# manhtuando97/two-stage-gnn

Measured on AMD Instinct MI355X. Metric: graphs/sec fwd+bwd, DD batch=32 SAGE-3L h=128, higher is better.
Workload: dtype f32; 1 GPU; DD-shaped synthetic graphs (avg 269 nodes / 676 edges, F_in=89), batch=32 per GPU, GcnEncoderGraph (GraphSage 'base') 3 layers h=128, Nmax=1000, slot-BN, CE loss, clip 2.0 + Adam; 1 step(s) per hipGraph launch, seed = rank, 128 untimed settle steps before the warm-up; global_batch=32, parallelism=dp1, launch=hipGraph replay (one graph: forward + backward + bucket + optimiser), rows=8151, edges_directed=40970

## Files before the change

### include/tsgnn.h

```cpp
#ifndef TSGNN_H
#define TSGNN_H
#include <stdint.h>

typedef struct ihipStream_t* tsgnn_stream_t;

#ifdef __cplusplus
extern "C" {
#endif

#define TSGNN_ABI_VERSION 2
int tsgnn_abi_version(void);
const char* tsgnn_strerror(int code);
const char* tsgnn_last_kernel(void);


int tsgnn_scan_workspace_ints(int64_t n, int64_t* ws_ints);
int tsgnn_exclusive_scan_i32(const int* in, int64_t n, int* out, int* ws, tsgnn_stream_t stream);

int tsgnn_row_maps(const int* graph_ptr, int B, int64_t n_rows, int* row_graph, int* row_slot,
                   tsgnn_stream_t stream);

int tsgnn_dense_adj_count(const float* adj, int B, int nmax, const int* graph_ptr, const int* row_graph,
                          int64_t n_rows, int* row_cnt, tsgnn_stream_t stream);
int tsgnn_dense_adj_fill(const float* adj, int B, int nmax, const int* graph_ptr, const int* row_graph,
                         int64_t n_rows, const int* rowptr, int* col, float* val, tsgnn_stream_t stream);

int tsgnn_coo_count(const int64_t* key, int64_t E, int64_t n_rows, int* cnt, int* bad_flag,
                    tsgnn_stream_t stream);
int tsgnn_coo_fill(const int64_t* key, const int64_t* other, int64_t E, int64_t n_rows, const int* rowptr,
                   int* cursor, int* col, int* eid, tsgnn_stream_t stream);


int tsgnn_ingest_layout(int B, int nmax, int64_t row_cap, int ell_w, int64_t tail_cap, int64_t* off);
int tsgnn_host_collate_tu(const int64_t* ds_graph_ptr, const int64_t* ds_rowptr, const int64_t* ds_col, const int64_t* ds_node_label,
                          const int64_t* ds_graph_label, const int64_t* ids, int B, int nmax, int64_t row_cap, int ell_w,
                          int64_t tail_cap, int32_t* staging, int64_t* out);
int tsgnn_onehot_rows_f32(const int* label, int64_t n_rows, int64_t total_rows, int F, float* x, int64_t ldx, tsgnn_stream_t stream);

int tsgnn_ingest_upload_f32(int32_t* dev, const int32_t* host, int64_t words, const int* node_label_dev, int64_t n_rows, int64_t total_rows,
                            int F, float* x, int64_t ldx, tsgnn_stream_t stream);
int tsgnn_ingest_compact_layout(int B, int nmax, int64_t row_cap, int64_t edge_cap, int64_t tail_cap, int64_t* off);
int tsgnn_host_collate_compact(const int64_t* ds_graph_ptr, const int64_t* ds_rowptr, const int64_t* ds_col, const int64_t* ds_node_label,
                               const int64_t* ds_graph_label, const int64_t* ids, int B, int nmax, int64_t row_cap, int64_t edge_cap,
                               int ell_w, int64_t tail_cap, int32_t* staging, int64_t* out);
int tsgnn_ingest_pull_expand_f32(const int32_t* host, int32_t* mirror, int B, int nmax, int64_t row_cap, int64_t edge_cap, int ell_w,
                                 int64_t tail_cap, int32_t* row_graph, int32_t* row_slot, int32_t* ell, int32_t* tail_ptr, int32_t* ell_slots, int32_t* tail_slots, int F, float* x,
                                 int64_t ldx, tsgnn_stream_t stream);
int tsgnn_ingest_pull_expand_ack_f32(const int32_t* host, int32_t* mirror, int B, int nmax, int64_t row_cap, int64_t edge_cap, int ell_w,
                                     int64_t tail_cap, int32_t* row_graph, int32_t* row_slot, int32_t* ell, int32_t* tail_ptr, int32_t* ell_slots, int32_t* tail_slots, int F,
                                     float* x, int64_t ldx, int64_t* host_ack, tsgnn_stream_t stream);
int tsgnn_ingest_pull_f32(const int32_t* host, int32_t* mirror, int B, int nmax, int64_t row_cap, int64_t edge_cap, int64_t tail_cap,
                          tsgnn_stream_t stream);
int tsgnn_ingest_expand_ack_f32(int32_t* mirror, int B, int nmax, int64_t row_cap, int64_t edge_cap, int ell_w, int64_t tail_cap,
                                int32_t* row_graph, int32_t* row_slot, int32_t* ell, int32_t* tail_ptr, int32_t* ell_slots, int32_t* tail_slots, int F, float* x, int64_t ldx,
                                int64_t* host_ack, tsgnn_stream_t stream);
int tsgnn_ingest_arm_pull_rider(const int32_t* host, int32_t* mirror, int B, int nmax, int64_t row_cap, int64_t edge_cap, int64_t tail_cap);
int tsgnn_ingest_arm_pull_rider_parts(const int32_t* host, int32_t* mirror, int B, int nmax, int64_t row_cap, int64_t edge_cap, int64_t tail_cap,
                                      int parts, int skip);
int tsgnn_ingest_arm_expand_rider(int32_t* mirror, int B, int nmax, int64_t row_cap, int64_t edge_cap, int ell_w, int64_t tail_cap,
                                  int32_t* row_graph, int32_t* row_slot, int32_t* ell, int32_t* tail_ptr, int32_t* ell_slots, int32_t* tail_slots, int F, float* x, int64_t ldx,
                                  int64_t* host_ack);
int tsgnn_ingest_flush_pull_rider(tsgnn_stream_t stream);
int tsgnn_ingest_disarm_riders(void);
typedef struct tsgnn_collate_pool tsgnn_collate_pool;
int tsgnn_collate_pool_create(int nthreads, tsgnn_collate_pool** pool);
int tsgnn_collate_pool_submit(tsgnn_collate_pool* pool, const int64_t* ds_graph_ptr, const int64_t* ds_rowptr, const int64_t* ds_col,
                              const int64_t* ds_node_label, const int64_t* ds_graph_label, const int64_t* ids, int B, int nmax,
                              int64_t row_cap, int64_t edge_cap, int ell_w, int64_t tail_cap, int32_t* staging, int64_t* out,
                              void* after_event, int64_t* ticket);
int tsgnn_collate_pool_submit_ack(tsgnn_collate_pool* pool, const int64_t* ds_graph_ptr, const int64_t* ds_rowptr, const int64_t* ds_col,
                                  const int64_t* ds_node_label, const int64_t* ds_graph_label, const int64_t* ids, int B, int nmax,
                                  int64_t row_cap, int64_t edge_cap, int ell_w, int64_t tail_cap, int32_t* staging, int64_t* out,
                                  const int64_t* host_ack, int64_t ack_target, int seq, int64_t* ticket);
int tsgnn_collate_pool_wait(tsgnn_collate_pool* pool, int64_t ticket);
int tsgnn_collate_pool_destroy(tsgnn_collate_pool* pool);

int tsgnn_csr_transpose(const int* rowptr, const int* col, const float* val, int64_t n_rows, int64_t n_cols,
                        int64_t nnz, int* rowptr_t, int* col_t, float* val_t, int* src_e, int* cnt_ws,
                        int* scan_ws, tsgnn_stream_t stream);


int tsgnn_csr_spmm_f32(const int* rowptr, const int* col, const float* val, const float* self_w,
                       const float* x, int64_t ldx, float* y, int64_t ldy, int64_t n_rows, int feat,
                       float self_scalar, int relu_in, int accumulate, tsgnn_stream_t stream);

int tsgnn_csr_to_ell(const int* rowptr, const int* col, int64_t n_rows, int W, int* ell, int* tail_cnt, tsgnn_stream_t stream);
int tsgnn_csr_tail_fill(const int* rowptr, const int* col, const int* tail_ptr, int64_t n_rows, int W, int* tail_col,
                        tsgnn_stream_t stream);
int tsgnn_ell_spmm_f32(const int* ell, int W, const float* x, int64_t ldx, float* y, int64_t ldy, int64_t n_rows, int feat,
                       float self_scalar, tsgnn_stream_t stream);

int tsgnn_gcn_norm_f32(const int* rowptr, const int* col, const float* val, int64_t n_rows, float self_fill,
                       float* dinv, float* val_out, float* self_w, tsgnn_stream_t stream);

int tsgnn_sddmm_rows_f32(const int* rowptr, const int* col, const float* dy, int64_t lddy, const float* x, int64_t ldx,
                         int64_t n_rows, int feat, float* dval, float* dself, tsgnn_stream_t stream);


int tsgnn_gemm_f32(const float* A, int64_t sam, int64_t sak, const float* B, int64_t sbk, int64_t sbn, float* C,
                   int64_t scm, int64_t scn, int M, int N, int K, int batch, int64_t stride_a, int64_t stride_b,
                   int64_t stride_c, const int* seg_ptr, int ragged, int max_seg, float alpha, int accumulate,
                   tsgnn_stream_t stream);
int tsgnn_gemm_splitk_plan(int M, int N, int K, int* ksplit, int64_t* ws_floats);
int tsgnn_gemm_splitk_f32(const float* A, int64_t sam, int64_t sak, const float* B, int64_t sbk, int64_t sbn,
                          float* C, int M, int N, int K, int ksplit, float* ws, int accumulate,
                          tsgnn_stream_t stream);
int tsgnn_linear_wgrad_plan(int64_t rows, int K_in, int N, int64_t ldz, int64_t lddu, int* nslab, int64_t* rows_per_slab,
                            int64_t* ws_floats);
int tsgnn_linear_wgrad_f32(const float* z, int64_t ldz, const float* du, int64_t lddu, int64_t rows, int K_in, int N, int nslab,
                           int64_t rows_per_slab, int64_t bias_only_rows, float* ws, float* dw, float* db, tsgnn_stream_t stream);
int tsgnn_wgrad_reduce_sets_blocks(const int64_t* desc);
int tsgnn_wgrad_reduce_sets_f32(const int64_t* desc, float* normparts, float* step_state, tsgnn_stream_t stream);
int tsgnn_wgrad_reduce_multi_f32(const float* ws0, int nslab0, int K0, int N0, float* dw0, float* db0, const float* ws1, int nslab1,
                                 int K1, int N1, float* dw1, float* db1, const float* ws2, int nslab2, int K2, int N2, float* dw2,
                                 float* db2, const float* ws3, int nslab3, int K3, int N3, float* dw3, float* db3,
                                 float* normparts, float* step_state, tsgnn_stream_t stream);
int tsgnn_wgrad_blocks_plan(int64_t rows, int K_in, int N, int64_t ldz, int64_t lddu, int* nslab, int64_t* rows_per_slab,
                            int64_t* ws_floats);
int tsgnn_wgrad_blocks_f32(const float* z, int64_t ldz, const float* du, int64_t lddu, int64_t rows, int K_in, int N, int nslab,
                           int64_t rows_per_slab, float* ws, float* dw, int64_t lddw, tsgnn_stream_t stream);
int tsgnn_wgrad_blocks_oi_f32(const float* z, int64_t ldz, const float* du, int64_t lddu, int64_t rows, int K_in, int N, int nslab,
                              int64_t rows_per_slab, float* ws, float* dw_oi, int64_t lddw, float* db, tsgnn_stream_t stream);
int tsgnn_ragged_tn_f32(const float* s_mat, int64_t lds_, const float* x, int64_t ldx, int K, int N, const int* slab_row_ptr,
                        int nslab, const int* seg_slab_ptr, int nseg, float* ws, float* out, tsgnn_stream_t stream);
int tsgnn_ragged_tn_direct_supported(int K, int64_t max_rows);
int tsgnn_ragged_tn_direct_f32(const float* s_mat, int64_t lds_, int K, const int* graph_ptr, int B, const float* x0, int64_t ldx0,
                               int N0, float* out0, const float* x1, int64_t ldx1, int N1, float* out1, tsgnn_stream_t stream);
int tsgnn_ragged_tn_direct_ro_f32(const float* s_mat, int64_t lds_, int K, const int* graph_ptr, int B, const float* x0, int64_t ldx0,
                                  int N0, float* out0, const float* x1, int64_t ldx1, int N1, float* out1, float* ro_out,
                                  int64_t ro_ldo, int* ro_arg, int nmax, int64_t n_real, int ghost_zero, tsgnn_stream_t stream);
int tsgnn_wgrad_narrow_plan(int64_t rows, int K_in, int N, int64_t* ws_floats);
int tsgnn_wgrad_narrow_f32(const float* z, int64_t ldz, const float* du, int64_t lddu, int64_t rows, int K_in, int N, float* ws,
                           float* dwb, tsgnn_stream_t stream);
int tsgnn_colsum_f32(const float* x, int64_t ld, int64_t rows, int F, float* out, float* ws, int accumulate,
                     tsgnn_stream_t stream);

int tsgnn_linear_l2norm_f32(const float* z, int64_t ldz, const float* w, int64_t ldw, const float* bias, float* v,
                            int64_t ldv, float* rinv, int64_t rows, int K, int N, int normalize,
                            tsgnn_stream_t stream);
int tsgnn_rowgemm_supported(const float* a, int64_t lda, const float* b, int64_t ldb, const float* c, int64_t ldc, int K, int N,
                            int trans_b);
int tsgnn_rowgemm_f32(const float* a, int64_t lda, const float* b, int64_t ldb, int trans_b, const float* bias, float* c,
                      int64_t ldc, float* rinv, int64_t rows, int K, int N, int normalize, int64_t fill_rows,
                      tsgnn_stream_t stream);
int tsgnn_panel_blocks(int64_t rows, int panel_units);
int tsgnn_gather_rowgemm_f32(const int* ell, int ell_w, const int* tail_ptr, const int* tail_col, const float* x, int64_t ldx, const float* b, int64_t ldb, int trans_b,
                             const float* bias, float* c, int64_t ldc, float* rinv, float* zout, int64_t ldz, int64_t rows, int K,
                             int N, int normalize, int64_t fill_rows, tsgnn_stream_t stream);
int tsgnn_gather_rowgemm_st_f32(const int* ell, int ell_w, const int* tail_ptr, const int* tail_col, const float* x, int64_t ldx, const float* b, int64_t ldb, const float* bias,
                                float* c, int64_t ldc, float* rinv, float* zout, int64_t ldz, int64_t rows, int K, int N,
                                int64_t fill_rows, const int* row_slot, unsigned long long* sums, float* ghost, int panel_units,
                                const int64_t* pack_desc, tsgnn_stream_t stream);
int tsgnn_sage_layer_fwd_bn_f32(const int* ell, int ell_w, const int* tail_ptr, const int* tail_col, const float* x, int64_t ldx, const float* w, int64_t ldw, const float* bias,
                                float* v, int64_t ldv, float* rinv, float* zout, int64_t ldz, int64_t rows, int K, int64_t fill_rows,
                                const int* graph_ptr, const int* slot_count, int B, int nslots, int n_ghost, unsigned long long* packed,
                                unsigned long long* packed_out, const int* row_graph, const unsigned long long* sums_in,
                                const float* ghost_in, float* mean_out, float* rstd_out, const int* row_slot,
                                unsigned long long* sums_out, float* ghost_out, const int* ro_map, int ro_map_ch, int panel_units,
                                const float* w_img, tsgnn_stream_t stream);
int tsgnn_sage_layer_fwd_bn_plan(int64_t rows, int64_t fill_rows, int B, int nslots, int panel_units, int* ro_ch, int* n_gemm,
                                 int* n_full);
int tsgnn_sage_layer_fwd_f32(const int* ell, int ell_w, const int* tail_ptr, const int* tail_col, const float* x, int64_t ldx, const float* w, int64_t ldw, const float* bias,
                             float* v, int64_t ldv, float* rinv, float* zout, int64_t ldz, int64_t rows, int K, int64_t fill_rows,
                             const int* graph_ptr, int B, int nslots, int n_ghost, unsigned long long* packed, tsgnn_stream_t stream);
int tsgnn_sage_layer_fwd_ro_f32(const int* ell, int ell_w, const int* tail_ptr, const int* tail_col, const float* x, int64_t ldx, const float* w, int64_t ldw, const float* bias,
                                float* v, int64_t ldv, float* rinv, float* zout, int64_t ldz, int64_t rows, int K, int64_t fill_rows,
                                const int* graph_ptr, int B, int nslots, int n_ghost, unsigned long long* packed,
                                unsigned long long* packed_out, const int* row_graph, tsgnn_stream_t stream);
int tsgnn_sage_layer_bwd_f32(const int* ell, int ell_w, const int* tail_ptr, const int* tail_col, const float* du, int64_t lddu, const float* w, int64_t ldw, float* dxs,
                             int64_t lddxs, const float* z, int64_t ldz, int64_t rows, int nslab, int64_t rows_per_slab,
                             int64_t bias_only_rows, float* ws, int panel_units, const float* w_img, tsgnn_stream_t stream);
int tsgnn_l2norm_bwd_f32(const float* v, int64_t ldv, const float* dv, int64_t lddv, const float* rinv, float* du,
                         int64_t lddu, int64_t rows, int F, tsgnn_stream_t stream);


int tsgnn_bn_slots_fwd_f32(const int* graph_ptr, const int* slot_count, const int* row_slot, int B, int nmax,
                           int64_t n_real, int n_ghost, const float* v, int64_t ldv, int F, int relu, int bn,
                           float* mean, float* rstd, float* y, int64_t ldy, tsgnn_stream_t stream);
int tsgnn_bn_slots_bwd_f32(const int* graph_ptr, const int* slot_count, const int* row_slot, int B, int nmax,
                           int64_t n_real, int n_ghost, const float* v, int64_t ldv, const float* dy, int64_t lddy, int F,
                           int relu, int bn, const float* mean, const float* rstd, float* m1, float* m2, float* dv,
                           int64_t lddv, tsgnn_stream_t stream);

int tsgnn_row_ln_fwd_f32(const float* v, int64_t ldv, int64_t rows, int F, int relu, float* mean, float* rstd, float* y, int64_t ldy,
                         tsgnn_stream_t stream);
int tsgnn_row_ln_bwd_f32(const float* v, int64_t ldv, const float* dy, int64_t lddy, int64_t rows, int F, int relu, const float* mean,
                         const float* rstd, float* dv, int64_t lddv, tsgnn_stream_t stream);

int tsgnn_row_post_bwd_f32(const int* row_graph, int B, int64_t n_real, int64_t rows, const float* v, int64_t ldv, const float* dxs,
                           int64_t lddxs, const float* dout, int64_t ldo, const int* arg, int F, int relu, int ln, const float* mean,
                           const float* rstd, const float* rinv, float* du, int64_t lddu, tsgnn_stream_t stream);

int tsgnn_row_post_nodes_bwd_f32(int64_t n_real, int64_t rows, const float* v, int64_t ldv, const float* dxs, int64_t lddxs,
                                 const float* dnode, int64_t lddn, int ghost_zero, int F, int relu, int ln, const float* mean,
                                 const float* rstd, const float* rinv, float* du, int64_t lddu, tsgnn_stream_t stream);

int tsgnn_readout_max_ws_words(int B, int nmax, int F);
int tsgnn_readout_max_fwd_f32(const int* graph_ptr, const int* slot_count, int B, int nmax, int64_t n_real, int n_ghost,
                              const float* x, int64_t ldx, int F, int relu, unsigned long long* packed_ws, float* out,
                              int64_t ldo, int* arg, tsgnn_stream_t stream);
int tsgnn_readout_max_bwd_f32(const float* dout, int64_t ldo, const int* arg, int B, int F, const float* x, int64_t ldx_in,
                              int relu, int64_t n_real, float* dx, int64_t ldx, tsgnn_stream_t stream);
int tsgnn_readout_max_bwd_rows_f32(const float* dout, int64_t ldo, const int* arg, const int* row_graph, int F, int64_t rows,
                                   int64_t rows_total, const float* add, int64_t ldadd, float* dx, int64_t ldx, tsgnn_stream_t stream);

int tsgnn_pack_rows_f32(const float* src, int nmax, int F, const int* row_graph, const int* row_slot, int64_t n_real,
                        float* dst, int64_t ld, tsgnn_stream_t stream);
int tsgnn_unpack_rows_f32(const int* graph_ptr, int B, int nmax, int64_t n_real, int n_ghost, const float* src, int64_t ld,
                          int F, float fill, float* dst, tsgnn_stream_t stream);
int tsgnn_unpack_rows_bwd_ghost_f32(const int* graph_ptr, int B, int nmax, int64_t n_real, const float* ddst, int F,
                                    float* dsrc, int64_t ld, tsgnn_stream_t stream);


int tsgnn_softmax_ce_f32(const float* logits, int64_t ld, const int64_t* label, int B, int C, float* loss, float* dlogits,
                         tsgnn_stream_t stream);
int tsgnn_adam_from_partials_f32(float* param, const float* grad, float* m, float* v, int64_t n, float lr, float beta1, float beta2,
                                 float eps, float weight_decay, float max_norm, float* state, const float* parts, int nparts,
                                 const float* poison, tsgnn_stream_t stream);
int tsgnn_clip_adam_step_f32(float* param, const float* grad, float* m, float* v, int64_t n, float lr, float beta1,
                             float beta2, float eps, float weight_decay, float max_norm, float grad_scale, float* state,
                             float* ws, const float* poison, tsgnn_stream_t stream);


int tsgnn_dense_stack_supported(int B, int K, int nstack, int L, int fin0, int hidden, int last0, int last1);
int tsgnn_dense_stack_fwd_f32(const int64_t* desc, tsgnn_stream_t stream);
int tsgnn_dense_stack_bwd_f32(const int64_t* desc, tsgnn_stream_t stream);
int tsgnn_dense_stack_max_resident(void);
int tsgnn_dense_stack_barrier_selftest(unsigned* sync, float* err, int expect, tsgnn_stream_t stream);


int tsgnn_node_scores_f32(const float* x, int64_t ldx, int64_t rows, int H, int Fh, const float* a, int64_t lda, float* s,
                          tsgnn_stream_t stream);
int tsgnn_node_scores2_f32(const float* x, int64_t ldx, int64_t rows, int H, int Fh, const float* a1, int64_t lda1, float* s1,
                           const float* a2, int64_t lda2, float* s2, tsgnn_stream_t stream);
int tsgnn_edge_softmax_fwd_f32(const int* rowptr, const int* col, int64_t rows, int H, const float* s_grp, const float* s_oth,
                               int mod, float slope, float* alpha, tsgnn_stream_t stream);
int tsgnn_edge_softmax_bwd_f32(const int* rowptr, const int* col, int64_t rows, int H, const float* s_grp, const float* s_oth,
                               int mod, float slope, const float* alpha, const float* dalpha, float* dt, float* ds_grp,
                               tsgnn_stream_t stream);
int tsgnn_edge_permute_f32(const float* src, const int* perm, int64_t n, int H, int scatter, float* dst, tsgnn_stream_t stream);
int tsgnn_csr_row_sum_f32(const int* rowptr, const float* val, int64_t rows, int H, float* out, tsgnn_stream_t stream);
int tsgnn_csr_row_sum_perm_f32(const int* rowptr, const float* val, const int* eperm, int64_t rows, int H, float* out,
                               tsgnn_stream_t stream);
int tsgnn_csr_spmm_heads_f32(const int* rowptr, const int* col, const float* alpha, int H, int Fh, const float* x, int64_t ldx,
                             int mod, float* y, int64_t ldy, int64_t rows, tsgnn_stream_t stream);
int tsgnn_csr_spmm_heads_epi_f32(const int* rowptr, const int* col, const float* alpha, int H, int Fh, const float* x, int64_t ldx,
                                 int mod, float* y, int64_t ldy, int64_t rows, const float* w1, const float* a1, int64_t lda1,
                                 const float* w2, const float* a2, int64_t lda2, const float* u, int64_t ldu, const float* uw,
                                 int rows_per_seg, const int* row_seg, float uscale, const int* eperm, tsgnn_stream_t stream);
int tsgnn_csr_sddmm_heads_f32(const int* rowptr, const int* col, int H, int Fh, const float* dy, int64_t lddy, const float* x,
                              int64_t ldx, int mod, float* dalpha, int64_t rows, tsgnn_stream_t stream);
int tsgnn_segment_wsum_f32(const float* x, int64_t ldx, const float* w, int H, int Fh, const int* seg_ptr, int nseg, int64_t rows,
                           int64_t max_seg, float scale, int mean, float* ws, float* out, int64_t ldo, tsgnn_stream_t stream);
int tsgnn_segment_wsum2_f32(const float* x, int64_t ldx, const float* w1, const float* w2, int H, int Fh, const int* seg_ptr, int nseg,
                            int64_t rows, int64_t max_seg, float scale, float* ws, float* out1, float* out2, int64_t ldo,
                            tsgnn_stream_t stream);
int tsgnn_gather_wsum_f32(const float* x, int64_t ldx, const int* idx, const float* w, const int* seg_ptr, int nseg, int C, float scale,
                          float* out, int64_t ldo, tsgnn_stream_t stream);
int tsgnn_broadcast_add_f32(float* y, int64_t ldy, int64_t rows, int H, int Fh, const float* w, const float* a, int64_t lda,
                            const float* u, int64_t ldu, int rows_per_seg, float scale, tsgnn_stream_t stream);
int tsgnn_pack_heads_max(void);
int tsgnn_pack_heads_f32(const float* w0, const float* w1, const float* w2, const float* w3, const float* w4, const float* w5,
                         const float* w6, const float* w7, const float* a0, const float* a1, const float* a2, const float* a3,
                         const float* a4, const float* a5, const float* a6, const float* a7, int H, int Fin, int Fo, float* W, float* A,
                         tsgnn_stream_t stream);
int tsgnn_unpack_heads_f32(const float* dW, const float* dA0, const float* dA1, int H, int Fin, int Fo, float* gw, float* ga,
                           tsgnn_stream_t stream);

int tsgnn_gat_fused_supported(int H, int Fh);
int tsgnn_gat_attn_fwd_f32(const float* hp, int64_t ldh, const int* rowptr, const int* col, const int* rp_t, const int* col_t,
                           int64_t rows, int H, int Fh, float slope, const int* row_graph, int nmax, const int* iso_idx,
                           const float* iso_w, const int* iso_ptr, float uscale, int mean_heads, int apply_elu, float drop_p,
                           uint64_t seed, const unsigned long long* drop_ctr, float* stat, float* y, int64_t ldy, tsgnn_stream_t stream);
int tsgnn_gat_bwd_parts(int B);
int tsgnn_gat_attn_bwd_f32(const float* hp, int64_t ldh, const float* y, int64_t ldy, const float* dy, int64_t lddy, const int* rp_t,
                           const int* col_t, int64_t rows, int H, int Fh, float slope, int mean_heads, int apply_elu,
                           const int* graph_ptr, int B, const int* iso_idx, const float* iso_w, const int* iso_ptr,
                           const float* iso_row, int iso_row_ld, float uscale, float drop_p, uint64_t seed,
                           const unsigned long long* drop_ctr, const float* stat, float* dhp, int Ns, float* t1, float* t2, float* S,
                           float* dupart, tsgnn_stream_t stream);
int tsgnn_gat_attn_bwd_ro_f32(const float* hp, int64_t ldh, const float* y, int64_t ldy, const float* dy, int64_t lddy, const int* rp_t,
                              const int* col_t, int64_t rows, int H, int Fh, float slope, int mean_heads, int apply_elu,
                              const int* graph_ptr, int B, const int* iso_idx, const float* iso_w, const int* iso_ptr,
                              const float* iso_row, int iso_row_ld, float uscale, float drop_p, uint64_t seed,
                              const unsigned long long* drop_ctr, const float* stat, float* dhp, int Ns, float* t1, float* t2, float* S,
                              float* dupart, const float* ro_dout, int64_t ro_ldo, const int* ro_arg, const int* row_graph,
                              tsgnn_stream_t stream);
int tsgnn_gat_dropout_mult_f32(float drop_p, uint64_t seed, const unsigned long long* drop_ctr, int64_t i0, int64_t ni, int64_t j0,
                               int64_t nj, int H, float* out, tsgnn_stream_t stream);
int tsgnn_gat_score_rowsum_f32(const int* rowptr, const int* col, const int* eperm, const float* t1, const float* t2, const float* S,
                               int64_t rows, int H, float* dhp, int64_t ldh, int C, const float* dupart, int B, const int* iso_idx,
                               const float* iso_w, const int* iso_ptr, float uscale, tsgnn_stream_t stream);
int tsgnn_gat_pack_desc_words(void);
int tsgnn_gat_pack_f32(const int64_t* desc, tsgnn_stream_t stream);
int tsgnn_gat_unpack_f32(const int64_t* desc, tsgnn_stream_t stream);
int tsgnn_elu_heads_fwd_f32(const float* x, int64_t rows, int H, int Fh, int mean_heads, int apply_elu, float* y, tsgnn_stream_t stream);
int tsgnn_elu_heads_bwd_f32(const float* x, const float* dy, int64_t rows, int H, int Fh, int mean_heads, int apply_elu, float* dx,
                            tsgnn_stream_t stream);


int tsgnn_mlp3_supported(int B, int D0, int D1, int D2, int C);
int tsgnn_mlp3_fwd_f32(const float* x, int64_t ldx, const float* w1, const float* b1, const float* keep, float keep_scale, const float* w2,
                       const float* b2, const float* w3, const float* b3, int B, int D0, int D1, int D2, int C, float* a1, float* a2,
                       float* logp, tsgnn_stream_t stream);
int tsgnn_mlp3_fwd_drop_f32(const float* x, int64_t ldx, const float* w1, const float* b1, float p, uint64_t seed,
                            unsigned long long* state, unsigned long long* used, const float* w2, const float* b2, const float* w3,
                            const float* b3, int B, int D0, int D1, int D2, int C, float* a1, float* a2, float* logp,
                            tsgnn_stream_t stream);
int tsgnn_mlp3_dropout_mask_f32(float p, uint64_t seed, uint64_t counter, int B, int D1, float* out, tsgnn_stream_t stream);
int tsgnn_mlp3_bwd_f32(const float* x, int64_t ldx, const float* w1, const float* w2, const float* w3, const float* a1,
                       const float* a2, const float* logp, const float* dlogp, float keep_scale, int B, int D0, int D1, int D2, int C,
                       float* dw1, float* db1, float* dw2, float* db2, float* dw3, float* db3, float* dx, int64_t lddx,
                       tsgnn_stream_t stream);
int tsgnn_mlp3_bwd2_f32(const float* x, int64_t ldx, const float* w1, const float* w2, const float* w3, const float* a1,
                        const float* a2, const float* logp, const float* dlogp, float keep_scale, int B, int D0, int D1, int D2, int C,
                        float* dw1, float* db1, float* dw2, float* db2, float* dw3, float* db3, float* dx, int64_t lddx, float* ws,
                        tsgnn_stream_t stream);
int tsgnn_mlp3_bwd2_nll_f32(const float* x, int64_t ldx, const float* w1, const float* w2, const float* w3, const float* a1,
                            const float* a2, const float* logp, const int64_t* label, float* loss, float keep_scale, int B, int D0,
                            int D1, int D2, int C, float* dw1, float* db1, float* dw2, float* db2, float* dw3, float* db3, float* dx,
                            int64_t lddx, float* ws, tsgnn_stream_t stream);

int tsgnn_mlp3_bwd2_norm_blocks(int D1, int D2);
int tsgnn_mlp3_bwd2_np_f32(const float* x, int64_t ldx, const float* w1, const float* w2, const float* w3, const float* a1,
                           const float* a2, const float* logp, const float* dlogp, const int64_t* label, float* loss, float keep_scale, int B,
                           int D0, int D1, int D2, int C, float* dw1, float* db1, float* dw2, float* db2, float* dw3, float* db3, float* dx,
                           int64_t lddx, float* ws, float* normparts, tsgnn_stream_t stream);

int tsgnn_mlp3_triplet_supported(int D0, int D1, int D2, int C);
int tsgnn_mlp3_triplet_fwd_f32(const float* x, int64_t ldx, const float* w1, const float* b1, float p, uint64_t seed,
                               unsigned long long* state, unsigned long long* used, const float* w2, const float* b2, const float* w3,
                               const float* b3, int D0, int D1, int D2, int C, float eps, float* a1, float* a2, float* embed, float* dist,
                               tsgnn_stream_t stream);
int tsgnn_mlp3_triplet_bwd_f32(const float* x, int64_t ldx, const float* w1, const float* w2, const float* w3, const float* a1,
                               const float* a2, const float* embed, const float* dist, float eps, float keep_scale, const float* g_dp,
                               const float* g_dn, const float* g_ea, const float* g_ep, const float* g_en, int D0, int D1, int D2, int C,
                               float* dw1, float* db1, float* dw2, float* db2, float* dw3, float* db3, float* dx, int64_t lddx,
                               tsgnn_stream_t stream);


int tsgnn_linkpred_tile_rows(void);
int tsgnn_linkpred_chunks(void);
int tsgnn_linkpred_loss_f32(const float* S, int64_t lds, int K, int64_t rows, const int* slab_row_ptr, const int* slab_graph,
                            int nslab, const int* graph_ptr, const int* rowptr, const int* col, const float* val,
                            const int* rowptr_t, const int* col_t, const float* val_t, float clamp, float inv_entries, float* dS,
                            int64_t ldd, float* ws, float* part, float* loss, tsgnn_stream_t stream);
int tsgnn_linkpred_loss_xy_f32(const float* X, int64_t ldx, const float* Y, int64_t ldy, int K, int64_t rows, const int* slab_row_ptr,
                               const int* slab_graph, int nslab, const int* graph_ptr, const int* rowptr, const int* col,
                               const float* val, float clamp, float inv_entries, int count_loss, float* dX, int64_t ldd, float* ws,
                               float* part, float* loss, tsgnn_stream_t stream);


int tsgnn_topk_max_segment(void);
int tsgnn_topk_segments_f32(const float* score, const int* graph_ptr, const int* k_ptr, int B, int max_seg, int* perm,
                            int* new_id, tsgnn_stream_t stream);
int tsgnn_gather_gate_fwd_f32(const float* x, int64_t ldx, const float* score, const int* perm, int64_t K, int F, int use_tanh,
                              float* out, int64_t ldo, tsgnn_stream_t stream);
int tsgnn_gather_gate_bwd_f32(const float* x, int64_t ldx, const float* score, const int* perm, int64_t K, int F, int use_tanh,
                              const float* dout, int64_t ldo, float* dx, int64_t lddx, float* dscore, tsgnn_stream_t stream);
int tsgnn_filter_edges_mark(const int* perm, int64_t K, int64_t N, const int64_t* src, const int64_t* dst, int64_t E,
                            int* new_id, int* flag, tsgnn_stream_t stream);
int tsgnn_filter_edges_compact(const int64_t* src, const int64_t* dst, int64_t E, const int* new_id, const int* flag,
                               const int* pos, int64_t* out_src, int64_t* out_dst, int64_t* kept_eid, tsgnn_stream_t stream);
int tsgnn_gcn_coef_f32(const int* rowptr, const int* col, int64_t n_rows, float* dinv, float* self_w, tsgnn_stream_t stream);
int tsgnn_gcn_propagate_f32(const int* rowptr, const int* col, const float* dinv, const float* self_w, const float* x,
                            int64_t ldx, int relu_in, const float* bias, const float* w_dot, const float* dot_bias, float* y,
                            int64_t ldy, float* t, int64_t n_rows, int feat, tsgnn_stream_t stream);
int tsgnn_gcn_propagate_re_f32(const int* rowptr, const int* rowend, const int* col, const float* dinv, const float* self_w,
                               const float* x, int64_t ldx, int relu_in, const float* bias, const float* w_dot, const float* dot_bias,
                               float* y, int64_t ldy, float* t, int64_t n_rows, int feat, tsgnn_stream_t stream);
int tsgnn_gcn_propagate_affine_f32(const int* rowptr, const int* rowend, const int* col, const float* dinv, const float* self_w,
                                   const float* x, int64_t ldx, float* agg, int64_t ldagg, int64_t n_rows, int feat, const float* w,
                                   int64_t ldw, const float* bias, float* y, int64_t ldy, int n_out, tsgnn_stream_t stream);
int tsgnn_propagate_mean_f32(const int* rowptr, const int* rowend, const int* col, int transpose, const float* x, int64_t ldx,
                             const float* xself, int64_t ldxs, float* y, int64_t ldy, int64_t n_rows, int feat, tsgnn_stream_t stream);
int tsgnn_sag_supported(int F);
int tsgnn_sag_pool_gather_f32(const float* y, int64_t ldy, const float* score, const int* perm, const int* new_id,
                              const int* rowptr, const int* col, int64_t K, int F, int relu_in, float* xp, int64_t ldo, int* cnt,
                              tsgnn_stream_t stream);
int tsgnn_sag_pool_graph_max_nodes(void);
int tsgnn_sag_pool_graph_f32(const float* y, int64_t ldy, const int* rowptr, const int* rowend, const int* col, const float* dinv,
                             const float* self_w, const float* w_s, const float* b_s, const int* graph_ptr, const int* graph_ptr_new,
                             int B, int max_seg, int F, float* score, int* perm, int* new_id, float* xp, int64_t ldo, int* cnt,
                             float* out, int64_t ldout, int* arg, int accumulate, int* rowptr_new, int* rowend_new, int* col_new,
                             float* dinv_new, float* self_w_new, float* agg_next, int64_t ldagg, tsgnn_stream_t stream);
int tsgnn_sag_readout_f32(const float* xp, int64_t ld, const int* graph_ptr, int B, int F, int accumulate, float* out, int64_t ldo,
                          int* arg, tsgnn_stream_t stream);
int tsgnn_csr_filter_fill(const int* rowptr, const int* col, const int* perm, const int* new_id, int64_t K, const int* rowptr_new,
                          int* col_new, float* dinv_new, float* self_w_new, tsgnn_stream_t stream);
int tsgnn_scan_short_i32(const int* in, int64_t n, int* out, tsgnn_stream_t stream);
int tsgnn_sag_pool_bwd_f32(const float* y, int64_t ldy, const float* score, const int* new_id, const int* row_graph_new,
                           const int* graph_ptr_new, const int* arg, const float* dxp, int64_t lddxp, const float* dread,
                           int64_t lddr, int64_t N, int F, int relu_in, float* dyb, int64_t lddy, float* dscore,
                           tsgnn_stream_t stream);
int tsgnn_sag_pool_graph_bwd_f32(const float* y, int64_t ldy, const float* score, const int* new_id, const int* graph_ptr,
                                 const int* graph_ptr_new, const int* arg, const float* dxp, int64_t lddxp, const float* dread,
                                 int64_t lddr, const int* rowptr, const int* rowend, const int* col, const float* dinv,
                                 const float* self_w, const float* w_s, int B, int max_seg, int F, float* du, int64_t lddu, float* part,
                                 float* dws, float* dbs, const float* dagg_next, int64_t lddagg, const int* rowptr_n,
                                 const int* rowend_n, const int* col_n, const float* dinv_n, const float* self_w_n,
                                 tsgnn_stream_t stream);
int tsgnn_sag_pool_graph_gc_f32(const float* y, int64_t ldy, const int* rowptr, const int* rowend, const int* col, const float* w_rel,
                                const float* w_root, const float* b, const int* graph_ptr, const int* graph_ptr_new, int B, int max_seg,
                                int F, float* score, int* perm, int* new_id, float* xp, int64_t ldo, int* cnt, float* out,
                                int64_t ldout, int* arg, int accumulate, int* rowptr_new, int* rowend_new, int* col_new,
                                tsgnn_stream_t stream);
int tsgnn_sag_pool_graph_gc_bwd_f32(const float* y, int64_t ldy, const float* score, const int* new_id, const int* graph_ptr,
                                    const int* graph_ptr_new, const int* arg, const float* dxp, int64_t lddxp, const float* dread,
                                    int64_t lddr, const int* rowptr, const int* rowend, const int* col, const float* w_rel,
                                    const float* w_root, int B, int max_seg, int F, float* du, int64_t lddu, float* part,
                                    tsgnn_stream_t stream);
int tsgnn_sag_du_reduce_f32(float* part, int nb, int F, float* dws, float* dbs, tsgnn_stream_t stream);
int tsgnn_linear_wgrad_du_f32(const float* z, int64_t ldz, const float* du, int64_t lddu, int64_t rows, int K_in, int N, int nslab,
                              int64_t rows_per_slab, float* ws, float* dw, float* db, float* part, int nb, int F_du, float* dws,
                              float* dbs, tsgnn_stream_t stream);
int tsgnn_sag_du_blocks(int64_t N, int F);
int tsgnn_sag_du_f32(const int* rowptr, const int* rowend, const int* col, const float* dinv, const float* self_w, const float* dscore, const float* y,
                     int64_t ldy, const float* w_s, float* dyb, int64_t lddy, int64_t N, int F, float* part, float* dws, float* dbs,
                     tsgnn_stream_t stream);
int tsgnn_relu_fwd_f32(const float* x, int64_t n, float* y, tsgnn_stream_t stream);
int tsgnn_relu_bwd_f32(const float* y, const float* dy, int64_t n, float* dx, tsgnn_stream_t stream);
int tsgnn_row_softmax_fwd_f32(const float* x, int64_t ldx, int64_t rows, int C, float* y, int64_t ldy, tsgnn_stream_t stream);
int tsgnn_row_softmax_bwd_f32(const float* y, int64_t ldy, const float* dy, int64_t lddy, int64_t rows, int C, float* dx,
                              int64_t lddx, tsgnn_stream_t stream);
int tsgnn_row_softmax_masked_fwd_f32(const float* x, int64_t ldx, int64_t rows, int C, float* y, int64_t ldy, int64_t zero_from,
                                     tsgnn_stream_t stream);
int tsgnn_row_softmax_masked_bwd_f32(const float* y, int64_t ldy, const float* dy, int64_t lddy, int64_t rows, int C, float* dx,
                                     int64_t lddx, int64_t zero_from, tsgnn_stream_t stream);
int tsgnn_row_softmax_ent_fwd_f32(const float* x, int64_t ldx, int64_t rows, int C, const float* mask, float eps, float* y, int64_t ldy,
                                  float* hpart, tsgnn_stream_t stream);
int tsgnn_row_softmax_ent_bwd_f32(const float* y, int64_t ldy, const float* ds, int64_t ldds, const float* mask, const float* g_ent,
                                  float g_scale, float eps, int64_t rows, int C, float* dx, int64_t lddx, tsgnn_stream_t stream);
int tsgnn_diffpool_link_fwd_f32(const float* adj, int64_t n_adj, const float* ao, const float* G, int B, int K, double* part, int nblk,
                                float* link, double* coef, tsgnn_stream_t stream);
int tsgnn_diffpool_link_bwd_f32(const float* g_link, const double* coef, const float* G, int B, int K, const float* adj, int64_t n_adj,
                                float* dG, float* dao, float* dadj, tsgnn_stream_t stream);


int tsgnn_slot_fused_supported(int B, int F);
int tsgnn_slot_bn_fwd_f32(const int* graph_ptr, const int* slot_count, int B, int nmax, int64_t n_real, int n_ghost,
                          const float* v, int64_t ldv, int F, int relu, float* mean, float* rstd, float* y, int64_t ldy,
                          unsigned long long* zero_ptr, int64_t zero_n, tsgnn_stream_t stream);
int tsgnn_slot_post_bwd_f32(const int* graph_ptr, const int* slot_count, int B, int nmax, int64_t n_real, int n_ghost,
                            const float* v, int64_t ldv, const float* dxs, int64_t lddxs, const float* dxs2, int64_t lddxs2,
                            const float* dout, int64_t ldo, const int* arg, int F, int relu, int bn, const float* mean,
                            const float* rstd, const float* rinv, float* du, int64_t lddu, tsgnn_stream_t stream);
int tsgnn_slot_post_wgrad_f32(const int* graph_ptr, const int* slot_count, int B, int nmax, int64_t n_real, int n_ghost,
                              const float* v, int64_t ldv, const float* dxs, int64_t lddxs, const float* dout, int64_t ldo,
                              const int* arg, int F, int relu, int bn, const float* mean, const float* rstd, const float* rinv,
                              const float* z, int64_t ldz, int K_in, float* ws, int nblocks, tsgnn_stream_t stream);
int tsgnn_readout_l2_bwd_f32(const int* graph_ptr, const int* row_graph, int B, int64_t n_real, int n_ghost_rows, const float* v,
                             int64_t ldv, const float* dout, int64_t ldo, const int* arg, int F, const float* rinv, float* du,
                             int64_t lddu, tsgnn_stream_t stream);
int tsgnn_readout_partial_f32(const int* graph_ptr, int B, int nmax, int64_t n_real, int n_ghost, const float* x, int64_t ldx, int F,
                              unsigned long long* packed, tsgnn_stream_t stream);
int tsgnn_readout_decode_layers_f32(const unsigned long long* packed, int B, int L, int Fh, int Fl, float* out, int64_t ldo, int* arg,
                                    tsgnn_stream_t stream);


int tsgnn_head2_fwd_f32(const float* out, int64_t ldo, const float* w1, const float* b1, const float* w2, const float* b2, int B, int P,
                        int E, int C, float* vec, float* y, tsgnn_stream_t stream);
int tsgnn_readout_head_fwd_f32(const unsigned long long* packed, int B, int L, int Fh, int Fl, const float* v_last, int64_t ldv,
                               const int* graph_ptr, int64_t n_real, int nslots, int n_ghost, float* out, int64_t ldo, int* arg,
                               const float* w1, const float* b1, const float* w2, const float* b2, int E, int C, float* vec, float* y,
                               tsgnn_stream_t stream);
int tsgnn_packed_head_fwd_f32(const unsigned long long* packed, int B, int L, int Fh, int Fl, float* out, int64_t ldo, int* arg,
                              const float* w1, const float* b1, const float* w2, const float* b2, int E, int C, float* vec, float* y,
                              tsgnn_stream_t stream);
int tsgnn_packed_head_fwd_z_f32(unsigned long long* packed, int B, int L, int Fh, int Fl, float* out, int64_t ldo, int* arg,
                                const float* w1, const float* b1, const float* w2, const float* b2, int E, int C, float* vec, float* y,
                                unsigned long long* clear, int64_t clear_n, tsgnn_stream_t stream);
int tsgnn_head2_bwd_f32(const float* out, int64_t ldo, const float* vec, const float* dy, const float* dvec, const float* w1,
                        const float* w2, int B, int P, int E, int C, float* dout, int64_t lddo, float* dw1, float* db1,
                        float* dw2, float* db2, float* normparts, tsgnn_stream_t stream);
int tsgnn_head2_fwd_ro_f32(float* out, int64_t ldo, const float* w1, const float* b1, const float* w2, const float* b2, int B, int P,
                           int E, int C, float* vec, float* y, const float* z, int64_t ldz, int N, int c0, int F, int* arg,
                           tsgnn_stream_t stream);
int tsgnn_head2_bwd_ro_f32(const float* out, int64_t ldo, const float* vec, const float* dy, const float* dvec, const float* w1,
                           const float* w2, int B, int P, int E, int C, float* dout, int64_t lddo, float* dw1, float* db1,
                           float* dw2, float* db2, float* normparts, const int* arg, int c0, int F, int N, float* dz, int64_t lddz,
                           const float* ce_y, const int64_t* ce_label, float* ce_loss, tsgnn_stream_t stream);
int tsgnn_head2_bwd_ce_f32(const float* out, int64_t ldo, const float* vec, const float* y, const int64_t* label, float* loss,
                           const float* dvec, const float* w1, const float* w2, int B, int P, int E, int C, float* dout, int64_t lddo,
                           float* dw1, float* db1, float* dw2, float* db2, float* normparts, tsgnn_stream_t stream);

int tsgnn_head2_bwd_du_f32(const float* out, int64_t ldo, const float* vec, const float* y, const int64_t* label, float* loss,
                           const float* dy, const float* dvec, const float* w1, const float* w2, int B, int P, int E, int C, float* dout,
                           int64_t lddo, float* dw1, float* db1, float* dw2, float* db2, float* normparts, const int* graph_ptr,
                           int64_t n_real, int n_ghost_rows, int max_nodes, const float* v, int64_t ldv, const float* rinv, const int* arg,
                           int seg_off, int F, float* du, int64_t lddu, tsgnn_stream_t stream);
int tsgnn_head2_bwd_du_map_f32(const float* out, int64_t ldo, const float* vec, const float* y, const int64_t* label, float* loss,
                               const float* dy, const float* dvec, const float* w1, const float* w2, int B, int P, int E, int C,
                               float* dout, int64_t lddo, float* dw1, float* db1, float* dw2, float* db2, float* normparts,
                               const int* graph_ptr, int64_t n_real, int n_ghost_rows, int max_nodes, const float* v, int64_t ldv,
                               const float* rinv, const int* arg, int seg_off, int F, float* du, int64_t lddu, const int* du_map,
                               int n_map, int du_chunk, tsgnn_stream_t stream);

int tsgnn_contract_dense_supported(int N, int K, int F);
int tsgnn_contract_dense_fwd_f32(const float* s, const float* z, const float* adj, int B, int N, int K, int F, float* xo, float* ao,
                                 float* t, tsgnn_stream_t stream);
int tsgnn_contract_dense_fwd_ro_f32(const float* s, const float* z, const float* adj, int B, int N, int K, int F, float* xo, float* ao,
                                    float* t, float* ro_out, int64_t ro_ldo, int* ro_arg, float* s_out, tsgnn_stream_t stream);
int tsgnn_contract_dense_bwd_f32(const float* s, const float* z, const float* adj, const float* t, const float* dxo, const float* dao,
                                 int B, int N, int K, int F, float* ds, float* dz, float* dadj, tsgnn_stream_t stream);
int tsgnn_contract_dense_bwd_ro_f32(const float* s, const float* z, const float* adj, const float* t, const float* dxo, const float* dao,
                                    int B, int N, int K, int F, float* ds, float* dz, float* dadj, const float* ro_dout, int64_t ro_ldo,
                                    const int* ro_arg, int softmax, tsgnn_stream_t stream);

int tsgnn_contract_rows_bwd_supported(int K, int F);
int tsgnn_contract_rows_bwd_f32(const float* S, int64_t ldS, const float* Z, int64_t ldZ, const float* AS, int64_t ldAS,
                                const float* dxo, const float* dao, const int* slab_row_ptr, const int* slab_graph, int nslab, int K,
                                int F, float* dZ, int64_t lddZ, float* dS, int64_t lddS, float* dAS, int64_t lddAS,
                                int64_t zero_from, int64_t zero_to, tsgnn_stream_t stream);
int tsgnn_contract_rows_bwd_ro_f32(const float* S, int64_t ldS, const float* Z, int64_t ldZ, const float* AS, int64_t ldAS,
                                   const float* dxo, const float* dao, const int* slab_row_ptr, const int* slab_graph, int nslab, int K,
                                   int F, float* dZ, int64_t lddZ, float* dS, int64_t lddS, float* dAS, int64_t lddAS,
                                   int64_t zero_from, int64_t zero_to, const float* ro_dout, int64_t ro_ldo, const int* ro_arg,
                                   tsgnn_stream_t stream);

int tsgnn_slot_bn_fwd_pair_f32(const int* graph_ptr, const int* slot_count, int B, int nmax, int64_t n_real, int n_ghost,
                               const float* v0, const float* v1, int64_t ldv, int F, int relu, float* mean0, float* mean1, float* rstd0,
                               float* rstd1, float* y0, float* y1, int64_t ldy, tsgnn_stream_t stream);
int tsgnn_slot_post_bwd_pair_f32(const int* graph_ptr, const int* slot_count, int B, int nmax, int64_t n_real, int n_ghost,
                                 const float* v0, const float* v1, int64_t ldv, const float* dxs0, const float* dxs1, int64_t lddxs,
                                 const float* dxs2_0, const float* dxs2_1, int64_t lddxs2, int F, int relu, int bn, const float* mean0,
                                 const float* mean1, const float* rstd0, const float* rstd1, const float* rinv0, const float* rinv1,
                                 float* du0, float* du1, int64_t lddu, tsgnn_stream_t stream);

int tsgnn_sage_multi_tn_words(void);
int tsgnn_sage_multi_g_words(void);
int tsgnn_sage_multi_f32(const int64_t* desc, tsgnn_stream_t stream);
int tsgnn_sage_multi_zero_f32(const int64_t* desc, float* zero0, int64_t n0, float* zero1, int64_t n1, tsgnn_stream_t stream);

int tsgnn_gat_bwd_products_f32(const float* x, int64_t ldx, const float* du, int64_t lddu, int64_t rows, int K_in, int N, const float* wp,
                               int64_t ldwp, float* dx, int64_t lddx, int nslab, int64_t rows_per_slab, float* ws, tsgnn_stream_t stream);
int tsgnn_linear_bwd_products_f32(const float* x, int64_t ldx, const float* dy, int64_t lddy, int64_t rows, int K_in, int N, const float* w,
                                  int64_t ldw, float* dx, int64_t lddx, int nslab, int64_t rows_per_slab, float* ws, tsgnn_stream_t stream);
int tsgnn_wgrad_blocks_slabs_f32(const float* z, int64_t ldz, const float* du, int64_t lddu, int64_t rows, int K_in, int N, int nslab,
                                 int64_t rows_per_slab, float* ws, tsgnn_stream_t stream);

int tsgnn_triplet_embed_fwd_f32(const float* r, int64_t ldr, const float* w, int64_t ldw, const float* b, int D, int E, float eps,
                                float* embed, float* dist, tsgnn_stream_t stream);
int tsgnn_triplet_embed_bwd_f32(const float* r, int64_t ldr, const float* w, int64_t ldw, int D, int E, float eps, const float* embed,
                                const float* dist, const float* d_dp, const float* d_dn, const float* d_ea, const float* d_ep,
                                const float* d_en, float* d_r, int64_t lddr, float* dw, int64_t lddw, float* db, tsgnn_stream_t stream);

int tsgnn_mlp2_triplet_supported(int D, int H, int E);
int tsgnn_mlp2_triplet_fwd_f32(const float* r, int64_t ldr, const float* w1, const float* b1, const float* w2, const float* b2, int D,
                               int H, int E, float eps, float* h, float* embed, float* dist, tsgnn_stream_t stream);
int tsgnn_mlp2_triplet_bwd_f32(const float* r, int64_t ldr, const float* w1, const float* w2, const float* h, const float* embed,
                               const float* dist, float eps, const float* g_dp, const float* g_dn, const float* g_ea, const float* g_ep,
                               const float* g_en, int D, int H, int E, float* dr, int64_t lddr, float* dw1, float* db1, float* dw2,
                               float* db2, tsgnn_stream_t stream);

int tsgnn_margin_rank_fwd_f32(const float* x1, const float* x2, const float* target, int64_t n, float margin, int mean, float* loss,
                              float* coef, tsgnn_stream_t stream);
int tsgnn_margin_rank_bwd_f32(const float* g, const float* coef, int64_t n, float* dx1, float* dx2, tsgnn_stream_t stream);

int tsgnn_sage_conv_supported(int K, int N);
int tsgnn_sage_conv_pack_f32(const int64_t* desc, tsgnn_stream_t stream);
int tsgnn_sage_conv_f32(const int* ell, int ell_w, const int* tail_ptr, const int* tail_col, const float* xg, int64_t ldxg, const float* xs,
                        int64_t ldxs, const float* dst_scale, const float* wl_pk, const float* wr_pk,
                        const float* bias, float* out, int64_t ldo, float* zout, int64_t ldz, float* rinv,
                        int64_t rows, int K, int N, int relu_out, int normalize, unsigned long long* ro_packed,
                        unsigned long long* ro_sums, const int* ro_row_graph, const int* ro_graph_ptr, const float* post_h, int64_t post_ldh,
                        const float* post_dread, int64_t post_lddr, const int* post_arg, const float* post_row_scale, float* out2,
                        int64_t ldo2, tsgnn_stream_t stream);
int tsgnn_sage_wgrad_pair_f32(const float* z, int64_t ldz, const float* x, int64_t ldx, const float* du, int64_t lddu, int64_t rows, int K,
                              int N, int nslab, int64_t rows_per_slab, float* ws_l, float* ws_r, tsgnn_stream_t stream);
int tsgnn_sage_relu_readout_bwd_f32(const float* h, int64_t ldh, const float* dxs, int64_t lddxs, const float* dread, int64_t lddr,
                                    const int* arg, const int* row_graph, const int* graph_ptr, int64_t rows, int F, int relu, float* du,
                                    int64_t lddu, const float* row_scale, float* dus, int64_t lddus, tsgnn_stream_t stream);
int tsgnn_sage_readout_decode_f32(unsigned long long* packed, unsigned long long* sums, const int* graph_ptr, int B, int L, int F, float* read,
                                  int64_t ldr, int* arg, tsgnn_stream_t stream);
int tsgnn_copy2d_multi_f32(const int64_t* desc, tsgnn_stream_t stream);

int tsgnn_gatconv_supported(int H, int Co);
int tsgnn_gatconv_fwd_f32(const float* hp, int64_t ldh, const int* rowptr, const int* col, int64_t rows, int H, int Co, float slope,
                          int mean_heads, int apply_elu, const float* bias, float* stat, float* y, int64_t ldy, tsgnn_stream_t stream);
int tsgnn_gatconv_bwd_rows_f32(const float* hp, int64_t ldh, const float* y, int64_t ldy, const float* dy, int64_t lddy, const int* rowptr,
                               const int* col, int64_t rows, int H, int Co, float slope, int mean_heads, int apply_elu, const float* stat,
                               float* dpre, int64_t lddp, float* dhp, int Ns, float* alpha, float* t1, float* t2, float* S,
                               tsgnn_stream_t stream);
int tsgnn_gatconv_pack_desc_words(void);
int tsgnn_gatconv_pack_f32(const int64_t* desc, tsgnn_stream_t stream);
int tsgnn_gatconv_unpack_f32(const int64_t* desc, tsgnn_stream_t stream);

int tsgnn_eigen_pool_fwd_f32(const float* z, int64_t ldz, int C, const int* graph_ptr0, int B, int nmax, int64_t n_rows0,
                             int ghost_mode, const int* graph_ptr1, const int* bptr, const int* members, const float* coef, int J,
                             int final_level, float* out, int64_t ldo, int64_t n_rows1, int n_ghost1, float* fsum, float* ro,
                             int64_t ldro, int* arg, tsgnn_stream_t stream);
int tsgnn_eigen_pool_bwd_f32(const float* dxp, int64_t lddxp, const float* fsum, const int* cluster_of, const int* row_graph,
                             const float* coef, int J, int C, const float* dro, int64_t lddro, const int* arg, int B, int nmax,
                             int64_t n_rows0, int ghost_mode, int final_level, float* dz, int64_t lddz, int64_t rows_total,
                             tsgnn_stream_t stream);
int tsgnn_eigen_pool_from_dense_f32(const float* P, int J, int B, int nmax, const int* row_graph, const int* row_slot,
                                    const int* graph_ptr1, int64_t n_rows, int final_level, int* cluster_of, float* coef, int64_t* key,
                                    int* bad, tsgnn_stream_t stream);

int tsgnn_knn_supported(int64_t dim, int k, int n_classes);
int tsgnn_knn_classify_f32(const float* train, int64_t ld_train, const int* train_class, int64_t n_train, const float* query,
                           int64_t ld_query, int64_t n_query, int64_t dim, int k, int n_classes, const int* query_class, int* confusion,
                           int* pred, int* nbr_index, float* nbr_dist, tsgnn_stream_t stream);

#ifdef __cplusplus
}
#endif
#endif
```

### two-stage-gnn_amd/csrc/layer_bwd.hip

```cpp
#include "common.h"
#include "../../include/tsgnn.h"
#include "rowgemm_body.h"
#include "tn_rows_body.h"
#include <cstdlib>

namespace {

template <bool PANELS_FIRST, bool UNITS = false, bool BIMG = false>
__global__ __launch_bounds__(256) void sage_layer_bwd_kernel(RowGemmArgs ga, TnArgs gt, unsigned n_tn, unsigned nslab, unsigned n_pan, int slab_delay) {
  extern __shared__ __attribute__((aligned(16))) float smem[];
  if (PANELS_FIRST) {
    if (blockIdx.x < n_pan) rowgemm_body<4, true, true, 1, false, false, false, UNITS, BIMG>(ga, smem, blockIdx.x);
    else {
      for (int i = 0; i < slab_delay; ++i) __builtin_amdgcn_s_sleep(16);
      const unsigned b = blockIdx.x - n_pan, by = b / nslab, sp = b % nslab;
      unsigned sl = sp;
      if ((nslab & 7u) == 0) sl = ((blockIdx.x & 7u) * (nslab >> 3)) + (sp >> 3);
      tn_rows_body<4, 4, 2>(gt, smem, sl, by, nslab);
    }
  } else {
    if (blockIdx.x < n_tn) tn_rows_body<4, 4, 2>(gt, smem, blockIdx.x % nslab, blockIdx.x / nslab, nslab);
    else rowgemm_body<4, true, true, 1, false, false, false, UNITS, BIMG>(ga, smem, blockIdx.x - n_tn);
  }
}

}

extern "C" {

int tsgnn_sage_layer_bwd_f32(const int* ell, int ell_w, const int* tail_ptr, const int* tail_col, const float* du, int64_t lddu, const float* w, int64_t ldw, float* dxs,
                             int64_t lddxs, const float* z, int64_t ldz, int64_t rows, int nslab, int64_t rows_per_slab,
                             int64_t bias_only_rows, float* ws, int panel_units, const float* w_img, tsgnn_stream_t stream) {
  if (!ell || !du || !w || !dxs || !z || !ws || rows <= 0 || nslab <= 0 || rows_per_slab <= 0 || bias_only_rows < 0) return TSGNN_EINVAL;
  if (ell_w != 4 && ell_w != 8 && ell_w != 16) return TSGNN_EUNSUPPORTED;
  const uintptr_t al = reinterpret_cast<uintptr_t>(ell) | reinterpret_cast<uintptr_t>(du) | reinterpret_cast<uintptr_t>(w) |
                       reinterpret_cast<uintptr_t>(dxs) | reinterpret_cast<uintptr_t>(z) | reinterpret_cast<uintptr_t>(w_img);
  if ((al & 15) || (lddu % 4) || (ldw % 4) || (lddxs % 4) || (ldz % 4) || lddu < 128 || ldw < 128 || lddxs < 128 || ldz < 128)
    return TSGNN_EUNSUPPORTED;
  if ((tail_ptr == nullptr) != (tail_col == nullptr)) return TSGNN_EINVAL;
  RowGemmArgs ga{du, lddu, w, ldw, nullptr, dxs, lddxs, nullptr, rows, 128, 128, 0, 0, ell, ell_w, nullptr, 0, tail_ptr, tail_col};
  ga.b_img = reinterpret_cast<const float4*>(w_img);
  TnArgs gt{z, ldz, du, lddu, rows, rows_per_slab, 128, 128, ws, nullptr, bias_only_rows};
  const int ncu = device_cu_count();
  const unsigned n_tn = 2u * (unsigned)nslab, n_pan = panel_split(rows, ncu, panel_units, &ga.n_full, &ga.unit);
  constexpr size_t lt = tn_rows_lds_bytes<4, 4>();
  const size_t la = w_img ? rowgemm_lds_bytes<4, true, true, 1, false, true>() : rowgemm_lds_bytes<4, true, true>();
  const size_t lds = la > lt ? la : lt;
  static const int panels_first = [] { const char* e = getenv("TSGNN_BWD_PANELS_FIRST"); return e ? atoi(e) : 1; }();
  static const int slab_delay_env = [] { const char* e = getenv("TSGNN_SLAB_DELAY"); return e ? atoi(e) : -1; }();
  const int slab_delay = slab_delay_env >= 0 ? slab_delay_env : ((int64_t)n_pan <= (int64_t)ncu ? 2 : 0);
  const bool units = ga.unit == 8 || ga.unit == 16;
  TSGNN_KNAME("sage_layer_bwd_kernel<%s,%s>", panels_first ? "true" : "false", units ? "true" : "false");
#define TSGNN_BWD_(PF_, UN_) \
  do {                       \
    if (w_img) sage_layer_bwd_kernel<PF_, UN_, true><<<n_tn + n_pan, 256, lds, stream>>>(ga, gt, n_tn, (unsigned)nslab, n_pan, slab_delay); \
    else sage_layer_bwd_kernel<PF_, UN_><<<n_tn + n_pan, 256, lds, stream>>>(ga, gt, n_tn, (unsigned)nslab, n_pan, slab_delay);            \
  } while (0)
  if (panels_first && units) TSGNN_BWD_(true, true);
  else if (panels_first) TSGNN_BWD_(true, false);
  else if (units) TSGNN_BWD_(false, true);
  else TSGNN_BWD_(false, false);
#undef TSGNN_BWD_
  TSGNN_CHECK_LAUNCH();
  return TSGNN_OK;
}

}
```

### two-stage-gnn_amd/csrc/layer_fwd.hip

```cpp
#include "common.h"
#include "../../include/tsgnn.h"
#include "rowgemm_body.h"
#include "readout_body.h"
#include "ingest_rider.h"

namespace {

template <bool RO>
__global__ __launch_bounds__(256) void sage_layer_fwd_kernel(RowGemmArgs ga, SlotArgs sa, unsigned n_gemm, unsigned ro_gx, int F4,
                                                             unsigned long long* __restrict__ packed, unsigned n_main, PullRider pr) {
  extern __shared__ __attribute__((aligned(16))) float smem[];
  if (blockIdx.x < n_gemm) {
    rowgemm_body<4, false, true, 1, RO>(ga, smem, blockIdx.x);
  } else if (blockIdx.x < n_main) {
    const unsigned r = blockIdx.x - n_gemm;
    readout_partial_body<32>(sa, ga.a, ga.lda, F4, packed, r % ro_gx, r / ro_gx, reinterpret_cast<unsigned long long*>(smem));
  } else {
    pull_rider_body(pr, blockIdx.x - n_main);
  }
}

template <bool RO, bool ST, bool UNITS = false, bool BIMG = false>
__global__ __launch_bounds__(256, 2) void sage_layer_fwd_bn_kernel(RowGemmArgs ga, SlotArgs sa, BnReadArgs bn, unsigned n_gemm, unsigned ro_gx,
                                                                int ro_ch, int F4, unsigned long long* __restrict__ packed, unsigned n_main,
                                                                PullRider pr, const int* __restrict__ ro_map) {
  extern __shared__ __attribute__((aligned(16))) float smem[];
  if (blockIdx.x < n_gemm) {
    rowgemm_body<4, false, true, 1, RO, true, ST, UNITS, BIMG>(ga, smem, blockIdx.x);
  } else if (blockIdx.x < n_main) {
    unsigned r = blockIdx.x - n_gemm;
    if (ro_map) r = (unsigned)ro_map[r];
    readout_partial_bn_body<32>(sa, bn, ga.a, ga.lda, F4, packed, r % ro_gx, r / ro_gx, ro_ch, reinterpret_cast<unsigned long long*>(smem));
  } else {
    pull_rider_body(pr, blockIdx.x - n_main);
  }
}

}

extern "C" {

int tsgnn_sage_layer_fwd_bn_plan(int64_t rows, int64_t fill_rows, int B, int nslots, int panel_units, int* ro_ch, int* n_gemm, int* n_full) {
  if (!ro_ch || !n_gemm || !n_full || rows <= 0 || B <= 0 || nslots <= 0) return TSGNN_EINVAL;
  const int ncu = device_cu_count();
  int unit_ = 16;
  const unsigned ng = panel_split(rows, ncu, panel_units, n_full, &unit_) + (fill_rows > 0 ? 1u : 0u);
  int ch = 64;
  while (ch < 256 && ng + (unsigned)((nslots + ch - 1) / ch) * (unsigned)B > 2u * (unsigned)ncu) ch *= 2;
  *ro_ch = ch; *n_gemm = (int)ng;
  return TSGNN_OK;
}

int tsgnn_sage_layer_fwd_bn_f32(const int* ell, int ell_w, const int* tail_ptr, const int* tail_col, const float* x, int64_t ldx, const float* w, int64_t ldw, const float* bias,
                                float* v, int64_t ldv, float* rinv, float* zout, int64_t ldz, int64_t rows, int K, int64_t fill_rows,
                                const int* graph_ptr, const int* slot_count, int B, int nslots, int n_ghost, unsigned long long* packed,
                                unsigned long long* packed_out, const int* row_graph, const unsigned long long* sums_in,
                                const float* ghost_in, float* mean_out, float* rstd_out, const int* row_slot,
                                unsigned long long* sums_out, float* ghost_out, const int* ro_map, int ro_map_ch, int panel_units,
                                const float* w_img, tsgnn_stream_t stream) {
  if (!ell || !x || !w || !v || !rinv || !graph_ptr || !slot_count || !packed || !sums_in || !ghost_in || !mean_out || !rstd_out ||
      rows <= 0 || fill_rows < 0 || K <= 0 || B <= 0 || nslots <= 0 || (n_ghost != 0 && n_ghost != nslots) || (packed_out && !row_graph) ||
      (row_slot && (!sums_out || !ghost_out)))
    return TSGNN_EINVAL;
  if (ell_w != 4 && ell_w != 8 && ell_w != 16) return TSGNN_EUNSUPPORTED;
  const uintptr_t al = reinterpret_cast<uintptr_t>(ell) | reinterpret_cast<uintptr_t>(x) | reinterpret_cast<uintptr_t>(w) |
                       reinterpret_cast<uintptr_t>(v) | reinterpret_cast<uintptr_t>(zout) | reinterpret_cast<uintptr_t>(bias) |
                       reinterpret_cast<uintptr_t>(sums_in) | reinterpret_cast<uintptr_t>(sums_out) | reinterpret_cast<uintptr_t>(w_img);
  if ((al & 15) || K != 128 || (ldx % 4) || (ldw % 4) || (ldv % 4) || (zout && (ldz % 4 || ldz < K)) || ldx < K || ldw < 128 || ldv < 128 ||
      nslots > BN_TAB || rows >= (1 << 20) || n_ghost == 0 || (packed_out && row_slot))
    return TSGNN_EUNSUPPORTED;
  if (packed_out && fill_rows <= 0) return TSGNN_EUNSUPPORTED;
  if ((tail_ptr == nullptr) != (tail_col == nullptr)) return TSGNN_EINVAL;
  RowGemmArgs ga{x, ldx, w, ldw, bias, v, ldv, rinv, rows, K, 128, 1, fill_rows, ell, ell_w, zout, ldz, tail_ptr, tail_col,
                 packed_out, graph_ptr, row_graph, B, nslots, n_ghost};
  ga.st_row_slot = row_slot; ga.st_sums = sums_out; ga.st_ghost = ghost_out;
  ga.b_img = reinterpret_cast<const float4*>(w_img);
  ga.bn_sums = sums_in; ga.bn_ghost = ghost_in; ga.bn_slot_count = slot_count; ga.bn_B = B; ga.bn_nslots = nslots; ga.bn_F = K;
  SlotArgs sa{graph_ptr, slot_count, B, nslots, rows, n_ghost};
  BnReadArgs bn{sums_in, ghost_in, K, mean_out, rstd_out};
  const int ncu = device_cu_count();
  const unsigned n_gemm = panel_split(rows, ncu, panel_units, &ga.n_full, &ga.unit) + (fill_rows > 0 ? 1u : 0u);
  int ro_ch = 64;
  while (ro_ch < 256 && n_gemm + (unsigned)((nslots + ro_ch - 1) / ro_ch) * (unsigned)B > 2u * (unsigned)ncu) ro_ch *= 2;
  const unsigned ro_gx = (unsigned)((nslots + ro_ch - 1) / ro_ch);
  if (ro_map && ro_map_ch != ro_ch) ro_map = nullptr;
  size_t lds = w_img ? rowgemm_lds_bytes<4, false, true, 1, true, true>() : rowgemm_lds_bytes<4, false, true, 1, true>();
  const size_t lro = 8 * 128 * sizeof(unsigned long long) + 256 * sizeof(float2);
  if (lds < lro) lds = lro;
  const unsigned n_main = n_gemm + ro_gx * (unsigned)B;
  const PullRider pr = take_pull_rider();
  const bool units = ga.unit == 8 || ga.unit == 16;
#define TSGNN_FWD_BN_(RO_, ST_, UN_, IM_) \
  sage_layer_fwd_bn_kernel<RO_, ST_, UN_, IM_><<<n_main + pr.blocks, 256, lds, stream>>>(ga, sa, bn, n_gemm, ro_gx, ro_ch, K / 4, packed, n_main, pr, ro_map)
#define TSGNN_FWD_BN(RO_, ST_)                                                                  \
  do {                                                                                          \
    if (units) { if (w_img) TSGNN_FWD_BN_(RO_, ST_, true, true); else TSGNN_FWD_BN_(RO_, ST_, true, false); }   \
    else { if (w_img) TSGNN_FWD_BN_(RO_, ST_, false, true); else TSGNN_FWD_BN_(RO_, ST_, false, false); }       \
  } while (0)
  if (packed_out) {
    TSGNN_KNAME("sage_layer_fwd_bn_kernel<true,false,%s>", units ? "true" : "false");
    TSGNN_FWD_BN(true, false);
  } else if (row_slot) {
    TSGNN_KNAME("sage_layer_fwd_bn_kernel<false,true,%s>", units ? "true" : "false");
    TSGNN_FWD_BN(false, true);
  } else {
    TSGNN_KNAME("sage_layer_fwd_bn_kernel<false,false,%s>", units ? "true" : "false");
    TSGNN_FWD_BN(false, false);
  }
#undef TSGNN_FWD_BN
#undef TSGNN_FWD_BN_
  TSGNN_CHECK_LAUNCH();
  return TSGNN_OK;
}

int tsgnn_sage_layer_fwd_ro_f32(const int* ell, int ell_w, const int* tail_ptr, const int* tail_col, const float* x, int64_t ldx, const float* w, int64_t ldw, const float* bias,
                                float* v, int64_t ldv, float* rinv, float* zout, int64_t ldz, int64_t rows, int K, int64_t fill_rows,
                                const int* graph_ptr, int B, int nslots, int n_ghost, unsigned long long* packed,
                                unsigned long long* packed_out, const int* row_graph, tsgnn_stream_t stream) {
  if (!ell || !x || !w || !v || !rinv || !graph_ptr || !packed || rows <= 0 || fill_rows < 0 || K <= 0 || B <= 0 || nslots <= 0 ||
      (n_ghost != 0 && n_ghost != nslots) || (packed_out && !row_graph))
    return TSGNN_EINVAL;
  if (ell_w != 4 && ell_w != 8 && ell_w != 16) return TSGNN_EUNSUPPORTED;
  const uintptr_t al = reinterpret_cast<uintptr_t>(ell) | reinterpret_cast<uintptr_t>(x) | reinterpret_cast<uintptr_t>(w) |
                       reinterpret_cast<uintptr_t>(v) | reinterpret_cast<uintptr_t>(zout) | reinterpret_cast<uintptr_t>(bias);
  if ((al & 15) || K != 128 || (ldx % 4) || (ldw % 4) || (ldv % 4) || (zout && (ldz % 4 || ldz < K)) || ldx < K || ldw < 128 || ldv < 128)
    return TSGNN_EUNSUPPORTED;
  if ((tail_ptr == nullptr) != (tail_col == nullptr)) return TSGNN_EINVAL;
  if (packed_out && n_ghost && fill_rows <= 0) return TSGNN_EUNSUPPORTED;
  RowGemmArgs ga{x, ldx, w, ldw, bias, v, ldv, rinv, rows, K, 128, 1, fill_rows, ell, ell_w, zout, ldz, tail_ptr, tail_col,
                 packed_out, graph_ptr, row_graph, B, nslots, n_ghost};
  SlotArgs sa{graph_ptr, nullptr, B, nslots, rows, n_ghost};
  const unsigned n_gemm = (unsigned)ceil_div64(rows, 32) + (fill_rows > 0 ? 1u : 0u);
  const unsigned ro_gx = (unsigned)((nslots + 63) / 64);
  size_t lds = rowgemm_lds_bytes<4, false, true>();
  if (lds < 8 * 128 * sizeof(unsigned long long)) lds = 8 * 128 * sizeof(unsigned long long);
  const unsigned n_main = n_gemm + ro_gx * (unsigned)B;
  const PullRider pr = take_pull_rider();
  if (packed_out) {
    TSGNN_KNAME("sage_layer_fwd_kernel<true>");
    sage_layer_fwd_kernel<true><<<n_main + pr.blocks, 256, lds, stream>>>(ga, sa, n_gemm, ro_gx, K / 4, packed, n_main, pr);
  } else {
    TSGNN_KNAME("sage_layer_fwd_kernel<false>");
    sage_layer_fwd_kernel<false><<<n_main + pr.blocks, 256, lds, stream>>>(ga, sa, n_gemm, ro_gx, K / 4, packed, n_main, pr);
  }
  TSGNN_CHECK_LAUNCH();
  return TSGNN_OK;
}

int tsgnn_sage_layer_fwd_f32(const int* ell, int ell_w, const int* tail_ptr, const int* tail_col, const float* x, int64_t ldx, const float* w, int64_t ldw, const float* bias,
                             float* v, int64_t ldv, float* rinv, float* zout, int64_t ldz, int64_t rows, int K, int64_t fill_rows,
                             const int* graph_ptr, int B, int nslots, int n_ghost, unsigned long long* packed, tsgnn_stream_t stream) {
  return tsgnn_sage_layer_fwd_ro_f32(ell, ell_w, tail_ptr, tail_col, x, ldx, w, ldw, bias, v, ldv, rinv, zout, ldz, rows, K, fill_rows,
                                     graph_ptr, B, nslots, n_ghost, packed, nullptr, nullptr, stream);
}

}
```

### two-stage-gnn_amd/csrc/rowgemm.hip

```cpp
#include "common.h"
#include "../../include/tsgnn.h"

#include <cstdlib>
#include "rowgemm_body.h"
#include "ingest_rider.h"
#include "pack_body.h"
#include "rowgemm_big_body.h"

namespace {

inline unsigned ks2_max_blocks() {
  static const unsigned n = [] { const char* e = getenv("TSGNN_KS2_MAX_BLOCKS"); return e ? (unsigned)atoi(e) : (unsigned)device_cu_count(); }();
  return n;
}
inline bool rowgemm_ks2_enabled() {
  static const bool on = [] { const char* e = getenv("TSGNN_ROWGEMM_KS2"); return !(e && e[0] == '0'); }();
  return on;
}

template <int NT, bool TRANS_B, bool GATHER>
__global__ __launch_bounds__(256) void rowgemm_kernel(RowGemmArgs g) {
  extern __shared__ __attribute__((aligned(16))) float smem[];
  rowgemm_body<NT, TRANS_B, GATHER>(g, smem, blockIdx.x);
}

template <int NT, bool TRANS_B>
__global__ __launch_bounds__(512) void rowgemm_gather_ks2_kernel(RowGemmArgs g) {
  extern __shared__ __attribute__((aligned(16))) float smem[];
  rowgemm_body<NT, TRANS_B, true, 2>(g, smem, blockIdx.x);
}

__device__ __forceinline__ void st_passengers(const PackRider& pk, const PullRider& pr, unsigned b) {
  if (b < pk.blocks) pack_rider_body(pk, b);
  else pull_rider_body(pr, b - pk.blocks);
}
template <bool UNITS>
__global__ __launch_bounds__(256) void rowgemm_gather_st_kernel(RowGemmArgs g, PullRider pr, unsigned nblk, PackRider pk) {
  extern __shared__ __attribute__((aligned(16))) float smem[];
  if (blockIdx.x >= nblk) { st_passengers(pk, pr, blockIdx.x - nblk); return; }
  rowgemm_body<4, false, true, 1, false, false, true, UNITS>(g, smem, blockIdx.x);
}
__global__ __launch_bounds__(512) void rowgemm_gather_ks2_st_kernel(RowGemmArgs g, PullRider pr, unsigned nblk, PackRider pk) {
  extern __shared__ __attribute__((aligned(16))) float smem[];
  if (blockIdx.x >= nblk) { st_passengers(pk, pr, blockIdx.x - nblk); return; }
  rowgemm_body<4, false, true, 2, false, false, true>(g, smem, blockIdx.x);
}

template <int NT, bool TRANS_B>
__global__ __launch_bounds__(256) void rowgemm_colsplit_kernel(RowGemmArgs g) {
  extern __shared__ __attribute__((aligned(16))) float smem[];
  const int n0 = (int)blockIdx.y * 32 * NT;
  g.N = min(32 * NT, g.N - n0);
  g.c += n0;
  if (g.bias) g.bias += n0;
  g.b += TRANS_B ? (int64_t)n0 * g.ldb : (int64_t)n0;
  g.rinv = nullptr;
  if (!TRANS_B && g.N <= 32) rowgemm_body<1, TRANS_B, false>(g, smem, blockIdx.x);
  else rowgemm_body<NT, TRANS_B, false>(g, smem, blockIdx.x);
}

inline bool rowgemm_colsplit_enabled() {
  static const bool on = [] { const char* e = getenv("TSGNN_ROWGEMM_COLSPLIT"); return !(e && e[0] == '0'); }();
  return on;
}

inline unsigned colsplit_max_panels() {
  static const unsigned n = [] {
    const char* e = getenv("TSGNN_ROWGEMM_COLSPLIT_PANELS");
    return e ? (unsigned)atoi(e) : 0xFFFFFFFFu;
  }();
  return n;
}

inline int64_t rowgemm_big_min_rows() {
  static const int64_t n = [] {
    const char* e = getenv("TSGNN_ROWGEMM_BIG_ROWS");
    return e ? (int64_t)atoll(e) : (int64_t)49152;
  }();
  return n;
}

inline int64_t rowgemm_big_wide_min_rows() {
  static const int64_t n = [] {
    const char* e = getenv("TSGNN_ROWGEMM_BIG_WIDE_ROWS");
    return e ? (int64_t)atoll(e) : (int64_t)2048;
  }();
  return n;
}

template <int U, bool TRANS_B>
void launch_big(const RowGemmArgs& g, hipStream_t s) {
  constexpr size_t lds = rowgemm_big_lds_bytes<U, TRANS_B>();
  static const int bpc = [] {
    if (lds > 64 * 1024)
      (void)hipFuncSetAttribute(reinterpret_cast<const void*>(rowgemm_big_kernel<U, TRANS_B>), hipFuncAttributeMaxDynamicSharedMemorySize, (int)lds);
    int n = 0;
    if (hipOccupancyMaxActiveBlocksPerMultiprocessor(&n, reinterpret_cast<const void*>(rowgemm_big_kernel<U, TRANS_B>), 256, lds) != hipSuccess || n < 1) n = 1;
    return n;
  }();
  const unsigned npanels = (unsigned)ceil_div64(g.rows, 32);
  const unsigned ny = (unsigned)((g.N + 127) / 128);
  const unsigned heavy = (unsigned)(g.N / 128 + ((g.N % 128) > 32 ? 1 : 0));
  unsigned grid = (unsigned)device_cu_count() * (unsigned)bpc / (heavy ? heavy : 1u);
  if (grid > npanels) grid = npanels;
  if (grid == 0) grid = 1;
  if (ny > 1) {
    const unsigned per = (npanels + grid - 1) / grid;
    grid = (npanels + per - 1) / per;
  }
  TSGNN_KNAME("rowgemm_big_kernel<%d,%s>", U, TRANS_B ? "true" : "false");
  rowgemm_big_kernel<U, TRANS_B><<<dim3(grid, ny), 256, lds, s>>>(g, npanels);
}

template <bool TRANS_B>
bool try_big(const RowGemmArgs& g, hipStream_t s) {
  const bool wide = g.N > 128;
  const int64_t mn = wide ? rowgemm_big_wide_min_rows() : rowgemm_big_min_rows();
  if (mn <= 0 || g.rows < mn || g.N > 384 || g.K > 128 || (TRANS_B && (g.K % 4)) || (g.N % 4)) return false;
  if (g.N > 128 && (g.normalize || g.fill_rows > 0 || g.rinv)) return false;
  if (g.K <= 96) launch_big<12, TRANS_B>(g, s);
  else launch_big<16, TRANS_B>(g, s);
  return true;
}

template <bool TRANS_B>
bool try_colsplit(const RowGemmArgs& g, hipStream_t s) {
  const unsigned nblk = (unsigned)ceil_div64(g.rows, 32);
  if (g.normalize || g.fill_rows > 0 || g.N <= 128 || (g.N % 4) || nblk == 0 || nblk > colsplit_max_panels() ||
      !rowgemm_colsplit_enabled())
    return false;
  const size_t lds = rowgemm_lds_bytes<4, TRANS_B, false>();
  TSGNN_KNAME("rowgemm_colsplit_kernel<4,%s>", TRANS_B ? "true" : "false");
  rowgemm_colsplit_kernel<4, TRANS_B><<<dim3(nblk, (unsigned)((g.N + 127) / 128)), 256, lds, s>>>(g);
  return true;
}

template <int NT, bool TRANS_B, bool GATHER>
void launch_rowgemm(const RowGemmArgs& g, hipStream_t s) {
  const unsigned nblk = (unsigned)(ceil_div64(g.rows, 32) + (g.fill_rows > 0 ? 1 : 0));
  if constexpr (GATHER && NT <= 4) {
    if (g.K > KC && nblk <= ks2_max_blocks() && rowgemm_ks2_enabled()) {
      constexpr size_t lds2 = rowgemm_lds_bytes<NT, TRANS_B, true, 2>();
      static bool attr = false;
      if (!attr && lds2 > 64 * 1024) {
        (void)hipFuncSetAttribute(reinterpret_cast<const void*>(rowgemm_gather_ks2_kernel<NT, TRANS_B>),
                                  hipFuncAttributeMaxDynamicSharedMemorySize, (int)lds2);
        attr = true;
      }
      TSGNN_KNAME("rowgemm_gather_ks2_kernel<%d,%s>", NT, TRANS_B ? "true" : "false");
      rowgemm_gather_ks2_kernel<NT, TRANS_B><<<nblk, 512, lds2, s>>>(g);
      return;
    }
  }
  const size_t lds = rowgemm_lds_bytes<NT, TRANS_B, GATHER>();
  TSGNN_KNAME("rowgemm_kernel<%d,%s,%s>", NT, TRANS_B ? "true" : "false", GATHER ? "true" : "false");
  rowgemm_kernel<NT, TRANS_B, GATHER><<<nblk, 256, lds, s>>>(g);
}

template <bool TRANS_B, bool GATHER>
void dispatch_rowgemm(const RowGemmArgs& g, hipStream_t s) {
  switch ((g.N + 31) / 32) {
    case 1: launch_rowgemm<1, TRANS_B, GATHER>(g, s); break;
    case 2: launch_rowgemm<2, TRANS_B, GATHER>(g, s); break;
    case 3: launch_rowgemm<3, TRANS_B, GATHER>(g, s); break;
    case 4: launch_rowgemm<4, TRANS_B, GATHER>(g, s); break;
    default:
      if constexpr (!GATHER) {
        switch ((g.N + 31) / 32) {
          case 5: launch_rowgemm<5, TRANS_B, false>(g, s); break;
          case 6: launch_rowgemm<6, TRANS_B, false>(g, s); break;
          case 7: launch_rowgemm<7, TRANS_B, false>(g, s); break;
          default: launch_rowgemm<8, TRANS_B, false>(g, s); break;
        }
      }
      break;
  }
}

}

extern "C" {

int tsgnn_rowgemm_supported(const float* a, int64_t lda, const float* b, int64_t ldb, const float* c, int64_t ldc, int K, int N,
                            int trans_b) {
  const bool al = ((reinterpret_cast<uintptr_t>(a) | reinterpret_cast<uintptr_t>(b)) & 15) == 0;
  if (!al || (lda % 4) || (ldb % 4) || N > 384 || N <= 0 || K <= 0) return 0;
  if (lda < ((K + 3) / 4) * 4) return 0;
  if (!trans_b && (N % 4)) return 0;
  if (trans_b && (K % 4)) return 0;
  (void)c; (void)ldc;
  return 1;
}

int tsgnn_rowgemm_f32(const float* a, int64_t lda, const float* b, int64_t ldb, int trans_b, const float* bias, float* c,
                      int64_t ldc, float* rinv, int64_t rows, int K, int N, int normalize, int64_t fill_rows,
                      tsgnn_stream_t stream) {
  if (!a || !b || !c || rows < 0 || fill_rows < 0 || K <= 0 || N <= 0 || lda < K || ldc < N) return TSGNN_EINVAL;
  if (!tsgnn_rowgemm_supported(a, lda, b, ldb, c, ldc, K, N, trans_b)) return TSGNN_EUNSUPPORTED;
  if (fill_rows > 0 && ((N % 4) || (ldc % 4) || (reinterpret_cast<uintptr_t>(c) & 15) ||
                        (bias && (reinterpret_cast<uintptr_t>(bias) & 15))))
    return TSGNN_EUNSUPPORTED;
  if (rows == 0 && fill_rows == 0) return TSGNN_OK;
  RowGemmArgs g{a, lda, b, ldb, bias, c, ldc, rinv, rows, K, N, normalize, fill_rows, nullptr, 0, nullptr, 0};
  if (trans_b) {
    if (!try_big<true>(g, stream) && !try_colsplit<true>(g, stream)) {
      if (N > 256) return TSGNN_EUNSUPPORTED;
      dispatch_rowgemm<true, false>(g, stream);
    }
  } else {
    if (!try_big<false>(g, stream) && !try_colsplit<false>(g, stream)) {
      if (N > 256) return TSGNN_EUNSUPPORTED;
      dispatch_rowgemm<false, false>(g, stream);
    }
  }
  TSGNN_CHECK_LAUNCH();
  return TSGNN_OK;
}

int tsgnn_gather_rowgemm_st_f32(const int* ell, int ell_w, const int* tail_ptr, const int* tail_col, const float* x, int64_t ldx, const float* b, int64_t ldb, const float* bias,
                                float* c, int64_t ldc, float* rinv, float* zout, int64_t ldz, int64_t rows, int K, int N,
                                int64_t fill_rows, const int* row_slot, unsigned long long* sums, float* ghost, int panel_units,
                                const int64_t* pack_desc, tsgnn_stream_t stream) {
  if (!ell || !x || !b || !c || !row_slot || !sums || !ghost || rows <= 0 || fill_rows < 0 || K <= 0 || N <= 0 || ldx < K || ldc < N)
    return TSGNN_EINVAL;
  if (ell_w != 4 && ell_w != 8 && ell_w != 16) return TSGNN_EUNSUPPORTED;
  if (!tsgnn_rowgemm_supported(x, ldx, b, ldb, c, ldc, K, N, 0) || N > 128 || N <= 96 || K > 128 || (reinterpret_cast<uintptr_t>(ell) & 15) ||
      (reinterpret_cast<uintptr_t>(sums) & 15))
    return TSGNN_EUNSUPPORTED;
  if (zout && ((ldz % 4) || ldz < K || (reinterpret_cast<uintptr_t>(zout) & 15))) return TSGNN_EUNSUPPORTED;
  if ((N % 4) || (ldc % 4) || (reinterpret_cast<uintptr_t>(c) & 15) || (bias && (reinterpret_cast<uintptr_t>(bias) & 15))) return TSGNN_EUNSUPPORTED;
  PackRider pk{};
  if (pack_desc) {
    if (reinterpret_cast<uintptr_t>(pack_desc) & 7) return TSGNN_EINVAL;
    const int nsets = (int)pack_desc[0];
    if (nsets <= 0 || nsets > PACK_RIDER_SETS) return TSGNN_EINVAL;
    for (int t = 0; t < nsets; ++t) {
      const int rc = pack_set_from_desc(pack_desc + 1 + 6 * t, pk.s[t]);
      if (rc != TSGNN_OK) return rc;
    }
    pk.blocks = (unsigned)nsets;
  }
  if ((tail_ptr == nullptr) != (tail_col == nullptr)) return TSGNN_EINVAL;
  RowGemmArgs g{x, ldx, b, ldb, bias, c, ldc, rinv, rows, K, N, 1, fill_rows, ell, ell_w, zout, ldz, tail_ptr, tail_col};
  g.st_row_slot = row_slot; g.st_sums = sums; g.st_ghost = ghost;
  unsigned nblk = (unsigned)(ceil_div64(rows, 32) + (fill_rows > 0 ? 1 : 0));
  const bool ks2 = K > KC && nblk <= ks2_max_blocks() && rowgemm_ks2_enabled();
  if (!ks2)
    nblk = panel_split(rows, device_cu_count(), panel_units, &g.n_full, &g.unit) + (fill_rows > 0 ? 1u : 0u);
  if (ks2) {
    constexpr size_t lds2 = rowgemm_lds_bytes<4, false, true, 2>();
    static bool attr = false;
    if (!attr && lds2 > 64 * 1024) {
      (void)hipFuncSetAttribute(reinterpret_cast<const void*>(rowgemm_gather_ks2_st_kernel), hipFuncAttributeMaxDynamicSharedMemorySize, (int)lds2);
      attr = true;
    }
    const PullRider pr = take_pull_rider(512);
    pk.blocks *= PACK_SET_ENTRIES / 512;
    TSGNN_KNAME("rowgemm_gather_ks2_st_kernel");
    rowgemm_gather_ks2_st_kernel<<<nblk + pk.blocks + pr.blocks, 512, lds2, stream>>>(g, pr, nblk, pk);
  } else {
    const PullRider pr = take_pull_rider(256);
    pk.blocks *= PACK_SET_ENTRIES / 256;
    TSGNN_KNAME("rowgemm_gather_st_kernel<%s>", (g.unit == 8 || g.unit == 16) ? "true" : "false");
    if (g.unit == 8 || g.unit == 16) rowgemm_gather_st_kernel<true><<<nblk + pk.blocks + pr.blocks, 256, rowgemm_lds_bytes<4, false, true>(), stream>>>(g, pr, nblk, pk);
    else rowgemm_gather_st_kernel<false><<<nblk + pk.blocks + pr.blocks, 256, rowgemm_lds_bytes<4, false, true>(), stream>>>(g, pr, nblk, pk);
  }
  TSGNN_CHECK_LAUNCH();
  return TSGNN_OK;
}

int tsgnn_panel_blocks(int64_t rows, int panel_units) {
  if (rows <= 0) return 0;
  int nf = 0, un = 16;
  return (int)panel_split(rows, device_cu_count(), panel_units, &nf, &un);
}

int tsgnn_gather_rowgemm_f32(const int* ell, int ell_w, const int* tail_ptr, const int* tail_col, const float* x, int64_t ldx, const float* b, int64_t ldb, int trans_b,
                             const float* bias, float* c, int64_t ldc, float* rinv, float* zout, int64_t ldz, int64_t rows, int K,
                             int N, int normalize, int64_t fill_rows, tsgnn_stream_t stream) {
  if (!ell || !x || !b || !c || rows < 0 || fill_rows < 0 || K <= 0 || N <= 0 || ldx < K || ldc < N) return TSGNN_EINVAL;
  if (ell_w != 4 && ell_w != 8 && ell_w != 16) return TSGNN_EUNSUPPORTED;
  if (!tsgnn_rowgemm_supported(x, ldx, b, ldb, c, ldc, K, N, trans_b) || N > 128 || K > 128 || (reinterpret_cast<uintptr_t>(ell) & 15))
    return TSGNN_EUNSUPPORTED;
  if (zout && ((ldz % 4) || ldz < K || (reinterpret_cast<uintptr_t>(zout) & 15))) return TSGNN_EUNSUPPORTED;
  if (fill_rows > 0 && ((N % 4) || (ldc % 4) || (reinterpret_cast<uintptr_t>(c) & 15) ||
                        (bias && (reinterpret_cast<uintptr_t>(bias) & 15))))
    return TSGNN_EUNSUPPORTED;
  if (rows == 0 && fill_rows == 0) return TSGNN_OK;
  if ((tail_ptr == nullptr) != (tail_col == nullptr)) return TSGNN_EINVAL;
  RowGemmArgs g{x, ldx, b, ldb, bias, c, ldc, rinv, rows, K, N, normalize, fill_rows, ell, ell_w, zout, ldz, tail_ptr, tail_col};
  if (trans_b) dispatch_rowgemm<true, true>(g, stream);
  else dispatch_rowgemm<false, true>(g, stream);
  TSGNN_CHECK_LAUNCH();
  return TSGNN_OK;
}

}
```

### two-stage-gnn_amd/csrc/rowgemm_body.h

```cpp
#pragma once
#include "common.h"
#include <type_traits>
#include <cstdlib>

namespace {


typedef float f32x16 __attribute__((ext_vector_type(16)));
constexpr int KC = 32;
constexpr int LDA_S = KC + 4;
constexpr float NORM_EPS = 1e-12f;

struct RowGemmArgs {
  const float* a; int64_t lda;
  const float* b; int64_t ldb;
  const float* bias;
  float* c; int64_t ldc;
  float* rinv;
  int64_t rows; int K; int N;
  int normalize;
  int64_t fill_rows;
  const int* ell; int ell_w;
  float* zout; int64_t ldz;
  const int* tail_ptr; const int* tail_col;
  unsigned long long* ro_packed;
  const int* ro_graph_ptr; const int* ro_row_graph;
  int ro_B, ro_nslots, ro_nghost;
  const int* st_row_slot; unsigned long long* st_sums; float* st_ghost;
  const unsigned long long* bn_sums; const float* bn_ghost; const int* bn_slot_count; int bn_B, bn_nslots, bn_F;
  int n_full;
  int unit;
  const float4* b_img;
};

inline int panel_unit_rows(int64_t rows, int ncu) {
  static const int forced = [] { const char* e = getenv("TSGNN_PANEL_UNIT"); const int v = e ? atoi(e) : 0; return (v == 8 || v == 16) ? v : 0; }();
  if (forced) return forced;
  return ((rows + 31) / 32 - ncu) <= ncu / 16 ? 8 : 16;
}
inline unsigned panel_split(int64_t rows, int ncu, int panel_units, int* n_full, int* unit) {
  const int64_t P = (rows + 31) / 32;
  *n_full = 0; *unit = 32;
  if (!panel_units || ncu < 8) return (unsigned)P;
  if (P <= ncu || P - ncu > ncu / 2) return (unsigned)P;
  const int nf = ncu & ~7;
  *n_full = nf;
  const int u = *unit = panel_unit_rows(rows, ncu);
  return (unsigned)nf + (unsigned)((rows - 32 * (int64_t)nf + u - 1) / u);
}

constexpr int BN_TAB = 1024;
constexpr float BN_FWD_EPS = 1e-5f;
constexpr double BN_FIX = 1099511627776.0;

__device__ __forceinline__ unsigned long long rg_pack_max(float val, unsigned r) {
  return ((unsigned long long)f32_ordered(val) << 32) | (unsigned long long)(0xFFFFFFFFu - r);
}

__device__ __forceinline__ float4 ldg4(const float* p) { return *reinterpret_cast<const float4*>(p); }

constexpr int GN = 8;
constexpr int LDA_F = 128;

template <int NT, bool TRANS_B, bool GATHER, int KS = 1, bool READOUT = false, bool BNIN = false, bool STATS = false, bool UNITS = false,
          bool BIMG = false>
__device__ __forceinline__ void rowgemm_body(const RowGemmArgs& g, float* smem_all, unsigned bid) {
  static_assert(KS == 1 || (KS == 2 && GATHER && NT <= 4), "the split-K variant is built for the gather kernel, widths <= 128");
  static_assert(!READOUT || (NT <= 4 && KS == 1), "the readout epilogue is built for one column tile per wave");
  static_assert(!BNIN || (GATHER && KS == 1), "batch-norm on the fly lives in the gather prologue of the one-group kernel");
  static_assert(!STATS || NT <= 4, "the statistics epilogue is built for one column tile per wave");
  static_assert(!BIMG || (GATHER && KS == 1 && NT == 4), "the image variant is built for the one-group gather kernel at K = N = 128");
  constexpr int NP = 32 * NT;
  constexpr int TPW = (NT + 3) / 4;
  constexpr int BV = NT;
  constexpr int A_FLOATS = GATHER ? 0 : 32 * LDA_S;
  constexpr int B_FLOATS = TRANS_B ? NP * LDA_S : KC * NP;
  constexpr int STAGE = A_FLOATS + B_FLOATS;
  const int tid_all = threadIdx.x;
  const int grp = KS == 2 ? (tid_all >> 8) : 0;
  const int tid = KS == 2 ? (tid_all & 255) : tid_all, lane = tid & 63, wid = tid >> 6;
  const int i = lane & 31, h = lane >> 5;
  const int Kc = KS == 1 ? g.K : ((g.K + 2 * KC - 1) / (2 * KC)) * KC;
  const int kb = grp * Kc;
  const int Kv = KS == 1 ? g.K : min(g.K - kb, Kc);
  constexpr int GRP = BIMG ? 256 : (KS == 2 && 2 * STAGE < 4096 + 256) ? 4096 + 256 : 2 * STAGE;
  float* smem = smem_all + grp * GRP;
  float* Apanel = smem_all + KS * GRP + (KS == 2 ? 0 : 256);
  float* scratch = KS == 2 ? smem_all + GRP + 4096 : smem_all + GRP;
  const unsigned npanels = (unsigned)((g.rows + 31) / 32);
  int64_t m0, rows_hi;
  if constexpr (UNITS) {
    const int un = g.unit == 8 ? 8 : 16;
    const unsigned nfull = (unsigned)g.n_full, nhalf = (unsigned)((g.rows - 32 * (int64_t)nfull + un - 1) / un);
    if (bid < nfull) { m0 = (int64_t)xcd_remap(bid, nfull) * 32; rows_hi = m0 + 32; }
    else if (bid < nfull + nhalf) { m0 = 32 * (int64_t)nfull + un * (int64_t)xcd_remap(bid - nfull, nhalf); rows_hi = min(m0 + un, g.rows); }
    else { m0 = (int64_t)npanels * 32; rows_hi = m0; }
  } else {
    m0 = (bid < npanels ? (int64_t)xcd_remap(bid, npanels) : (int64_t)bid) * 32;
    rows_hi = g.rows;
  }
  TR(0);
  if (m0 >= g.rows) {
    if (KS == 2 && grp == 1) return;
    float* fred = smem_all;
    const int N4 = g.N / 4, rpp = 256 / N4;
    const int c4 = tid % N4, rsub = tid / N4;
    float4 bv = make_float4(0.f, 0.f, 0.f, 0.f);
    if (g.bias && rsub < rpp) bv = ldg4(g.bias + 4 * c4);
    float ss = rsub == 0 ? (bv.x * bv.x + bv.y * bv.y) + (bv.z * bv.z + bv.w * bv.w) : 0.f;
    ss = wave_sum(ss);
    if (lane == 0) fred[wid] = ss;
    __syncthreads();
    float sc = 1.f;
    if (g.normalize) sc = fminf(__builtin_amdgcn_rsqf((fred[0] + fred[1]) + (fred[2] + fred[3])), 1.0f / NORM_EPS);
    const float4 out = make_float4(bv.x * sc, bv.y * sc, bv.z * sc, bv.w * sc);
    if constexpr (STATS) {
      if (g.st_ghost && wid == 0) {
        const float a = fmaxf(out.x, 0.f), b = fmaxf(out.y, 0.f), c = fmaxf(out.z, 0.f), d = fmaxf(out.w, 0.f);
        float g1 = rsub == 0 ? (a + b) + (c + d) : 0.f, g2 = rsub == 0 ? (a * a + b * b) + (c * c + d * d) : 0.f;
        g1 = wave_sum(g1); g2 = wave_sum(g2);
        if (lane == 0) { g.st_ghost[0] = g1; g.st_ghost[1] = g2; }
      }
    }
    if (rsub < rpp) {
      for (int64_t r = rsub; r < g.fill_rows; r += rpp) {
        *reinterpret_cast<float4*>(g.c + (g.rows + r) * g.ldc + 4 * c4) = out;
        if (g.rinv && c4 == 0) g.rinv[g.rows + r] = sc;
      }
      if constexpr (READOUT) {
        if (g.ro_packed && g.ro_nghost) {
          for (int b = rsub; b < g.ro_B; b += rpp) {
            const int sz = g.ro_graph_ptr[b + 1] - g.ro_graph_ptr[b];
            if (sz < g.ro_nslots && sz < g.fill_rows) {
              const unsigned row = (unsigned)(g.rows + sz);
              unsigned long long* dst = g.ro_packed + (int64_t)b * g.N + 4 * c4;
              atomicMax(dst + 0, rg_pack_max(out.x, row)); atomicMax(dst + 1, rg_pack_max(out.y, row));
              atomicMax(dst + 2, rg_pack_max(out.z, row)); atomicMax(dst + 3, rg_pack_max(out.w, row));
            }
          }
        }
      }
    }
    return;
  }
  int ro_gf = 0, ro_gl = 0;
  if constexpr (READOUT) {
    if (g.ro_packed) {
      ro_gf = g.ro_row_graph[m0];
      ro_gl = g.ro_row_graph[min(m0 + 31, rows_hi - 1)];
    }
  }

  const int am = tid >> 3, ak4 = tid & 7;
  const bool a_row_ok = (m0 + am) < rows_hi;
  const float* ap = g.a + ((a_row_ok && !GATHER) ? (m0 + am) : 0) * g.lda + 4 * ak4 + (GATHER ? 0 : kb);
  const float* bp[BV];
  int b_k[BV];
  int b_lds[BV];
  bool b_nok[BV];
#pragma unroll
  for (int q = 0; q < BV; ++q) {
    const int idx = q * 256 + tid;
    if (!TRANS_B) {
      const int k = idx / (NP / 4), n4 = idx % (NP / 4);
      b_nok[q] = 4 * n4 < g.N;
      bp[q] = g.b + (int64_t)(k + kb) * g.ldb + (b_nok[q] ? 4 * n4 : 0);
      b_k[q] = k;
      b_lds[q] = k * NP + 4 * n4;
    } else {
      const int n = idx / (KC / 4), k4 = idx % (KC / 4);
      b_nok[q] = n < g.N;
      bp[q] = g.b + (int64_t)(b_nok[q] ? n : 0) * g.ldb + 4 * k4 + kb;
      b_k[q] = 4 * k4;
      b_lds[q] = n * LDA_S + 4 * k4;
    }
  }
  struct Staged {
    float4 ra;
    float4 rb[BV];
    int a_valid;
    unsigned b_valid;
    bool plain;
  };
  const bool panel_full = (m0 + 32) <= rows_hi && g.N == NP;
  auto fetch = [&](Staged& s, int k0) {
    s.plain = panel_full && (k0 + KC) <= Kv;
    s.a_valid = 0;
    s.b_valid = 0;
    if (GATHER) {
#pragma unroll
      for (int q = 0; q < BV; ++q) {
        const bool kok = (k0 + b_k[q]) < Kv;
        if (!TRANS_B) s.rb[q] = ldg4(kok ? bp[q] + (int64_t)k0 * g.ldb : bp[q] - (int64_t)b_k[q] * g.ldb);
        else s.rb[q] = ldg4(kok ? bp[q] + k0 : bp[q] - b_k[q]);
        s.b_valid |= (kok && b_nok[q]) ? (1u << q) : 0u;
      }
      s.plain = false;
      return;
    }
    if (s.plain) {
      s.ra = ldg4(ap + k0);
#pragma unroll
      for (int q = 0; q < BV; ++q) s.rb[q] = ldg4(TRANS_B ? bp[q] + k0 : bp[q] + (int64_t)k0 * g.ldb);
      return;
    }
    const int gk = k0 + 4 * ak4;
    const bool ok = a_row_ok && gk < Kv;
    s.a_valid = ok ? min(4, Kv - gk) : 0;
    s.ra = ldg4(gk < Kv ? ap + k0 : ap - 4 * ak4);
#pragma unroll
    for (int q = 0; q < BV; ++q) {
      const bool kok = (k0 + b_k[q]) < Kv;
      if (!TRANS_B) s.rb[q] = ldg4(kok ? bp[q] + (int64_t)k0 * g.ldb : bp[q] - (int64_t)b_k[q] * g.ldb);
      else s.rb[q] = ldg4(kok ? bp[q] + k0 : bp[q] - b_k[q]);
      s.b_valid |= (kok && b_nok[q]) ? (1u << q) : 0u;
    }
  };
  auto commit = [&](const Staged& s, float* st) {
    if (GATHER) {
#pragma unroll
      for (int q = 0; q < BV; ++q)
        *reinterpret_cast<float4*>(st + A_FLOATS + b_lds[q]) = ((s.b_valid >> q) & 1u) ? s.rb[q] : make_float4(0.f, 0.f, 0.f, 0.f);
      return;
    }
    if (s.plain) {
      *reinterpret_cast<float4*>(st + am * LDA_S + 4 * ak4) = s.ra;
#pragma unroll
      for (int q = 0; q < BV; ++q) *reinterpret_cast<float4*>(st + A_FLOATS + b_lds[q]) = s.rb[q];
      return;
    }
    float4 va = s.ra;
    if (s.a_valid < 4) va.w = 0.f;
    if (s.a_valid < 3) va.z = 0.f;
    if (s.a_valid < 2) va.y = 0.f;
    if (s.a_valid < 1) va.x = 0.f;
    *reinterpret_cast<float4*>(st + am * LDA_S + 4 * ak4) = va;
#pragma unroll
    for (int q = 0; q < BV; ++q)
      *reinterpret_cast<float4*>(st + A_FLOATS + b_lds[q]) = ((s.b_valid >> q) & 1u) ? s.rb[q] : make_float4(0.f, 0.f, 0.f, 0.f);
  };
  auto frags = [&](const float* st, int k0, float (&af)[KC / 2], float (&bf)[TPW][KC / 2]) {
    const float* As = GATHER ? Apanel : st;
    constexpr int lda_s = GATHER ? LDA_F : LDA_S;
    const int kq = GATHER ? (kb + k0) >> 2 : 0;
    const float* Bs = st + A_FLOATS;
#pragma unroll
    for (int u = 0; u < KC / 8; ++u) {
      const float4 v = GATHER ? *reinterpret_cast<const float4*>(As + i * lda_s + 4 * ((kq + 2 * u + h) ^ (i & 7)))
                              : *reinterpret_cast<const float4*>(As + i * lda_s + 8 * u + 4 * h);
      af[4 * u] = v.x; af[4 * u + 1] = v.y; af[4 * u + 2] = v.z; af[4 * u + 3] = v.w;
    }
    if constexpr (BIMG) return;
#pragma unroll
    for (int t = 0; t < TPW; ++t) {
      const int tile = wid + 4 * t;
      if (4 * (t + 1) <= NT || tile < NT) {
#pragma unroll
        for (int u = 0; u < KC / 8; ++u) {
          if (!TRANS_B) {
#pragma unroll
            for (int c = 0; c < 4; ++c) bf[t][4 * u + c] = Bs[(8 * u + 4 * h + c) * NP + tile * 32 + i];
          } else {
            const float4 v = *reinterpret_cast<const float4*>(Bs + (tile * 32 + i) * LDA_S + 8 * u + 4 * h);
            bf[t][4 * u] = v.x; bf[t][4 * u + 1] = v.y; bf[t][4 * u + 2] = v.z; bf[t][4 * u + 3] = v.w;
          }
        }
      } else {
#pragma unroll
        for (int j = 0; j < KC / 2; ++j) bf[t][j] = 0.f;
      }
    }
  };

  f32x16 acc[TPW];
#pragma unroll
  for (int t = 0; t < TPW; ++t)
#pragma unroll
    for (int r = 0; r < 16; ++r) acc[t][r] = 0.f;

  constexpr int NS = (NT <= 4 && !GATHER) ? 4 : 2;
  Staged st[NS];
  constexpr int NPASS = 4 / KS;
  int ids[NPASS][GN];
  if (GATHER) {
    const int rsub = tid_all >> 5;
#pragma unroll
    for (int p = 0; p < NPASS; ++p) {
      const int64_t row = m0 + 8 * KS * p + rsub;
#pragma unroll
      for (int q = 0; q < GN / 4; ++q) {
        int4 v = make_int4(-1, -1, -1, -1);
        if (row < rows_hi && 4 * q < g.ell_w) v = *reinterpret_cast<const int4*>(g.ell + row * g.ell_w + 4 * q);
        ids[p][4 * q] = v.x; ids[p][4 * q + 1] = v.y; ids[p][4 * q + 2] = v.z; ids[p][4 * q + 3] = v.w;
      }
    }
  }
  constexpr int BN_PT = BN_TAB / 256;
  float2* bn_tab = reinterpret_cast<float2*>(Apanel + 32 * LDA_F);
  ulonglong2 bn_s[BNIN ? BN_PT : 1];
  int bn_have[BNIN ? BN_PT : 1];
  float bn_g1 = 0.f, bn_g2 = 0.f;
  if constexpr (BNIN) {
#pragma unroll
    for (int q = 0; q < BN_PT; ++q) {
      const int n = min(tid_all + 256 * q, g.bn_nslots - 1);
      bn_s[q] = *reinterpret_cast<const ulonglong2*>(g.bn_sums + 2 * n);
      bn_have[q] = g.bn_slot_count[n];
    }
    bn_g1 = g.bn_ghost[0]; bn_g2 = g.bn_ghost[1];
  }
  int st_slot = -1;
  if constexpr (STATS) {
    if (g.st_sums && wid == 0 && grp == 0 && lane < 32 && (m0 + lane) < rows_hi) st_slot = g.st_row_slot[m0 + lane];
  }
  if constexpr (!BIMG) {
#pragma unroll
    for (int c = 0; c < NS; ++c)
      if (c == 0 || c * KC < Kc) fetch(st[c], c * KC);
  }
  float bq[BIMG ? 4 * KC / 2 : 1];
  auto img_fetch = [&](int u0) {
    const float4* img = g.b_img + (wid * 16 + u0) * 64 + lane;
#pragma unroll
    for (int u = 0; u < 8; ++u) {
      const float4 v = img[u * 64];
      bq[4 * (u0 + u)] = v.x; bq[4 * (u0 + u) + 1] = v.y; bq[4 * (u0 + u) + 2] = v.z; bq[4 * (u0 + u) + 3] = v.w;
    }
  };
  if (GATHER) {
    const int c4 = tid_all & 31, rsub = tid_all >> 5;
    const bool colok = 4 * c4 < g.K;
    if constexpr (BNIN) {
      const double inv_cnt = 1.0 / ((double)g.bn_B * (double)g.bn_F);
#pragma unroll
      for (int q = 0; q < BN_PT; ++q) {
        const int n = tid_all + 256 * q;
        if (n < g.bn_nslots) {
          const float2 ms = bn_stats_from_sums(bn_s[q].x, bn_s[q].y, bn_have[q], bn_g1, bn_g2, g.bn_B, inv_cnt, BN_FWD_EPS);
          bn_tab[n] = make_float2(ms.y, ms.x * ms.y);
        }
      }
    }
    float4 nbv[NPASS][GN];
#pragma unroll
    for (int p = 0; p < NPASS; ++p)
#pragma unroll
      for (int k = 0; k < GN; ++k) {
        nbv[p][k] = make_float4(0.f, 0.f, 0.f, 0.f);
        if (colok && ids[p][k] >= 0) nbv[p][k] = ldg4(g.a + (int64_t)(BNIN ? (ids[p][k] & 0xFFFFF) : ids[p][k]) * g.lda + 4 * c4);
      }
    if constexpr (BIMG) {
      __builtin_amdgcn_sched_barrier(0);
      img_fetch(0);
      __builtin_amdgcn_sched_barrier(0);
    }
    if constexpr (BNIN) {
      __syncthreads();
#pragma unroll
      for (int p = 0; p < NPASS; ++p)
#pragma unroll
        for (int k = 0; k < GN; ++k) {
          if (ids[p][k] >= 0) {
            const float2 rm = bn_tab[ids[p][k] >> 20];
            float4& t = nbv[p][k];
            t.x = fmaf(fmaxf(t.x, 0.f), rm.x, -rm.y); t.y = fmaf(fmaxf(t.y, 0.f), rm.x, -rm.y);
            t.z = fmaf(fmaxf(t.z, 0.f), rm.x, -rm.y); t.w = fmaf(fmaxf(t.w, 0.f), rm.x, -rm.y);
          }
        }
    }
#pragma unroll
    for (int p = 0; p < NPASS; ++p) {
      const int64_t row = m0 + 8 * KS * p + rsub;
      float4 va = nbv[p][0];
#pragma unroll
      for (int k = 1; k < GN; ++k) { va.x += nbv[p][k].x; va.y += nbv[p][k].y; va.z += nbv[p][k].z; va.w += nbv[p][k].w; }
      bool table_full = g.ell_w <= GN && ids[p][GN - 1] >= 0;
      if (colok && g.ell_w > GN && ids[p][GN - 1] >= 0) {
        static_assert(GN == 8, "the second half of a 16-wide table");
        const int4 e0 = *reinterpret_cast<const int4*>(g.ell + row * g.ell_w + 8), e1 = *reinterpret_cast<const int4*>(g.ell + row * g.ell_w + 12);
        const int js[8] = {e0.x, e0.y, e0.z, e0.w, e1.x, e1.y, e1.z, e1.w};
        table_full = js[7] >= 0;
        float4 t[8];
#pragma unroll
        for (int k = 0; k < 8; ++k) t[k] = ldg4(g.a + (int64_t)(js[k] >= 0 ? (BNIN ? (js[k] & 0xFFFFF) : js[k]) : 0) * g.lda + 4 * c4);
#pragma unroll
        for (int k = 0; k < 8; ++k) {
          if (js[k] >= 0) {
            if constexpr (BNIN) {
              const float2 rm = bn_tab[js[k] >> 20];
              t[k].x = fmaf(fmaxf(t[k].x, 0.f), rm.x, -rm.y); t[k].y = fmaf(fmaxf(t[k].y, 0.f), rm.x, -rm.y);
              t[k].z = fmaf(fmaxf(t[k].z, 0.f), rm.x, -rm.y); t[k].w = fmaf(fmaxf(t[k].w, 0.f), rm.x, -rm.y);
            }
            va.x += t[k].x; va.y += t[k].y; va.z += t[k].z; va.w += t[k].w;
          }
        }
      }
      if (colok && g.tail_ptr && row < rows_hi && table_full) {
        for (int e = g.tail_ptr[row]; e < g.tail_ptr[row + 1]; ++e) {
          const int j = g.tail_col[e];
          float4 t = ldg4(g.a + (int64_t)(BNIN ? (j & 0xFFFFF) : j) * g.lda + 4 * c4);
          if constexpr (BNIN) {
            const float2 rm = bn_tab[j >> 20];
            t.x = fmaf(fmaxf(t.x, 0.f), rm.x, -rm.y); t.y = fmaf(fmaxf(t.y, 0.f), rm.x, -rm.y);
            t.z = fmaf(fmaxf(t.z, 0.f), rm.x, -rm.y); t.w = fmaf(fmaxf(t.w, 0.f), rm.x, -rm.y);
          }
          va.x += t.x; va.y += t.y; va.z += t.z; va.w += t.w;
        }
      }
      {
        const int pr = 8 * KS * p + rsub;
        *reinterpret_cast<float4*>(Apanel + pr * LDA_F + 4 * (c4 ^ (pr & 7))) = va;
      }
      if (g.zout && colok && row < rows_hi) st_out(reinterpret_cast<float4*>(g.zout + row * g.ldz + 4 * c4), va);
    }
    if constexpr (BIMG) {
      __builtin_amdgcn_sched_barrier(0);
      img_fetch(8);
      __builtin_amdgcn_sched_barrier(0);
    }
  }
  float bias_v[TPW];
#pragma unroll
  for (int t = 0; t < TPW; ++t) {
    const int cn = (wid + 4 * t) * 32 + i;
    bias_v[t] = (g.bias && (wid + 4 * t) < NT && cn < g.N) ? g.bias[cn] : 0.f;
  }
  TR(1);
  if constexpr (!BIMG) {
    commit(st[0], smem);
    if (KC < Kc) commit(st[1], smem + STAGE);
  }
  __syncthreads();
  TR(2);
  float fa[2][KC / 2], fb[2][TPW][KC / 2];
  frags(smem, 0, fa[0], fb[0]);
  if constexpr (BIMG) {
#pragma unroll
    for (int c = 0; c < 4; ++c) {
      if (c < 3) frags(smem, (c + 1) * KC, fa[(c + 1) & 1], fb[0]);
      __builtin_amdgcn_sched_barrier(0);
#pragma unroll
      for (int j = 0; j < KC / 2; ++j) acc[0] = __builtin_amdgcn_mfma_f32_32x32x2f32(fa[c & 1][j], bq[16 * c + j], acc[0], 0, 0, 0);
      __builtin_amdgcn_sched_barrier(0);
      TR(3 + 2 * c);
      TR(4 + 2 * c);
    }
  }
  if (NS == 2 && !BIMG) {
    if (2 * KC < Kc) fetch(st[0], 2 * KC);
    if (3 * KC < Kc) fetch(st[1], 3 * KC);
  }
  auto body = [&](auto ci_, int c) {
    constexpr int CI = decltype(ci_)::value;
    constexpr int P = CI & 1;
    const int k0 = c * KC;
    if (k0 + KC < Kc) frags(smem + (P ^ 1) * STAGE, k0 + KC, fa[P ^ 1], fb[P ^ 1]);
    if (NS == 4 && c >= 0 && k0 + 4 * KC < Kc) fetch(st[CI % NS], k0 + 4 * KC);
    __builtin_amdgcn_sched_barrier(0);
#pragma unroll
    for (int j = 0; j < 8; ++j) acc[0] = __builtin_amdgcn_mfma_f32_32x32x2f32(fa[P][j], fb[P][0][j], acc[0], 0, 0, 0);
    __builtin_amdgcn_sched_barrier(0);
    if (k0 + 2 * KC < Kc) commit(st[(CI + 2) % NS], smem + P * STAGE);
    if (NS == 2 && k0 + 4 * KC < Kc) fetch(st[CI % NS], k0 + 4 * KC);
    __builtin_amdgcn_sched_barrier(0);
#pragma unroll
    for (int j = 8; j < KC / 2; ++j) acc[0] = __builtin_amdgcn_mfma_f32_32x32x2f32(fa[P][j], fb[P][0][j], acc[0], 0, 0, 0);
#pragma unroll
    for (int t = 1; t < TPW; ++t) {
      if (4 * (t + 1) <= NT || (wid + 4 * t) < NT) {
#pragma unroll
        for (int j = 0; j < KC / 2; ++j) acc[t] = __builtin_amdgcn_mfma_f32_32x32x2f32(fa[P][j], fb[P][t][j], acc[t], 0, 0, 0);
      }
    }
    TR(3 + 2 * min(c, 3));
    if (Kc > 2 * KC) __syncthreads();
    TR(4 + 2 * min(c, 3));
  };
  for (int c = 0; !BIMG && c * KC < Kc; c += 4) {
    body(std::integral_constant<int, 0>{}, c);
    if ((c + 1) * KC < Kc) body(std::integral_constant<int, 1>{}, c + 1);
    if ((c + 2) * KC < Kc) body(std::integral_constant<int, 2>{}, c + 2);
    if ((c + 3) * KC < Kc) body(std::integral_constant<int, 3>{}, c + 3);
  }
  if (KS == 2) {
    float* xch = smem_all + GRP;
    if (grp == 1) {
#pragma unroll
      for (int r = 0; r < 16; ++r) xch[(wid * 16 + r) * 64 + lane] = acc[0][r];
    }
    __syncthreads();
    TR(7);
    if (grp == 1) { TR_END(); return; }
#pragma unroll
    for (int r = 0; r < 16; ++r) acc[0][r] += xch[(wid * 16 + r) * 64 + lane];
    TR(8);
  }

  float scale[16];
#pragma unroll
  for (int r = 0; r < 16; ++r) scale[r] = 1.f;
  if (g.bias || g.normalize) {
    float ss[16];
    float q1[STATS ? 16 : 1], q2[STATS ? 16 : 1];
#pragma unroll
    for (int r = 0; r < 16; ++r) ss[r] = 0.f;
#pragma unroll
    for (int t = 0; t < TPW; ++t) {
      const int tile = wid + 4 * t;
      const int cn = tile * 32 + i;
      const bool okc = tile < NT && cn < g.N;
      const float bv = bias_v[t];
#pragma unroll
      for (int r = 0; r < 16; ++r) {
        const float v = okc ? acc[t][r] + bv : 0.f;
        acc[t][r] = v;
        ss[r] = fmaf(v, v, ss[r]);
        if constexpr (STATS) { const float rl = fmaxf(v, 0.f); q1[r] = rl; q2[r] = rl * rl; }
      }
    }
    if (g.normalize) {
      float* red = scratch;
      float* inv = red + 128 + wid * 32;
      float* redq = smem_all;
      if constexpr (STATS) { if (Kc <= 2 * KC) __syncthreads(); }
      float tot = row16_sum_transpose(ss);
      tot += __shfl_xor(tot, 16, 64);
      float t1 = 0.f, t2 = 0.f;
      if constexpr (STATS) {
        t1 = row16_sum_transpose(q1); t2 = row16_sum_transpose(q2);
        t1 += __shfl_xor(t1, 16, 64); t2 += __shfl_xor(t2, 16, 64);
      }
      TR(11);
      if ((lane & 16) == 0) {
        const int r = lane & 15, row = (r & 3) + 8 * (r >> 2) + 4 * h;
        red[row * 4 + wid] = tot;
        if constexpr (STATS) { redq[row * 4 + wid] = t1; redq[128 + row * 4 + wid] = t2; }
      }
      __syncthreads();
      TR(12);
      if (lane < 32) {
        const float4 p = *reinterpret_cast<const float4*>(red + lane * 4);
        const float rs = fminf(__builtin_amdgcn_rsqf((p.x + p.y) + (p.z + p.w)), 1.0f / NORM_EPS);
        inv[lane] = rs;
        if (g.rinv && wid == 0 && (m0 + lane) < rows_hi) g.rinv[m0 + lane] = rs;
        if constexpr (STATS) {
          if (g.st_sums && wid == 0 && st_slot >= 0) {
            const float4 a = *reinterpret_cast<const float4*>(redq + lane * 4), b = *reinterpret_cast<const float4*>(redq + 128 + lane * 4);
            const float s1 = ((a.x + a.y) + (a.z + a.w)) * rs, s2 = ((b.x + b.y) + (b.z + b.w)) * (rs * rs);
            atomicAdd(g.st_sums + 2 * st_slot, (unsigned long long)__double2ll_rn((double)s1 * BN_FIX));
            atomicAdd(g.st_sums + 2 * st_slot + 1, (unsigned long long)__double2ll_rn((double)s2 * BN_FIX));
          }
        }
      }
      __syncthreads();
#pragma unroll
      for (int q = 0; q < 4; ++q) {
        const float4 v = *reinterpret_cast<const float4*>(inv + 8 * q + 4 * h);
        scale[4 * q] = v.x; scale[4 * q + 1] = v.y; scale[4 * q + 2] = v.z; scale[4 * q + 3] = v.w;
      }
    }
  }
  const bool full = panel_full;
#pragma unroll
  for (int t = 0; t < TPW; ++t) {
    const int tile = wid + 4 * t;
    if (tile < NT) {
      const int cn = tile * 32 + i;
      float* cp = g.c + (m0 + 4 * h) * g.ldc + cn;
      if (full) {
#pragma unroll
        for (int r = 0; r < 16; ++r) st_out(cp + (int64_t)((r & 3) + 8 * (r >> 2)) * g.ldc, acc[t][r] * scale[r]);
      } else {
#pragma unroll
        for (int r = 0; r < 16; ++r) {
          const int64_t gm = m0 + (r & 3) + 8 * (r >> 2) + 4 * h;
          if (gm < rows_hi && cn < g.N) cp[(int64_t)((r & 3) + 8 * (r >> 2)) * g.ldc] = acc[t][r] * scale[r];
        }
      }
    }
  }
  if constexpr (READOUT) {
    if (g.ro_packed) {
      const int cn = wid * 32 + i;
      const int64_t last = min(m0 + 31, rows_hi - 1);
      for (int b = ro_gf; b <= ro_gl; ++b) {
        int64_t lo = m0, hi = last + 1;
        if (ro_gf != ro_gl) { lo = max(lo, (int64_t)g.ro_graph_ptr[b]); hi = min(hi, (int64_t)g.ro_graph_ptr[b + 1]); }
        unsigned long long best = 0ull;
#pragma unroll
        for (int r = 0; r < 16; ++r) {
          const int64_t gm = m0 + (r & 3) + 8 * (r >> 2) + 4 * h;
          if (gm >= lo && gm < hi) {
            const unsigned long long p = rg_pack_max(acc[0][r] * scale[r], (unsigned)gm);
            best = p > best ? p : best;
          }
        }
        const unsigned olo = __shfl_xor((unsigned)(best & 0xFFFFFFFFull), 32, 64), ohi = __shfl_xor((unsigned)(best >> 32), 32, 64);
        const unsigned long long other = ((unsigned long long)ohi << 32) | olo;
        best = other > best ? other : best;
        if (h == 0 && best && cn < g.N) atomicMax(&g.ro_packed[(int64_t)b * g.N + cn], best);
      }
    }
  }
  TR(13);
  TR_END();
}


template <int NT, bool TRANS_B, bool GATHER, int KS = 1, bool BNIN = false, bool BIMG = false>
constexpr size_t rowgemm_lds_bytes() {
  constexpr int NP = 32 * NT;
  constexpr int STAGE2 = BIMG ? 256 : 2 * ((GATHER ? 0 : 32 * LDA_S) + (TRANS_B ? NP * LDA_S : KC * NP));
  constexpr int GRP = (KS == 2 && STAGE2 < 4096 + 256) ? 4096 + 256 : STAGE2;
  return sizeof(float) * (KS * GRP + (KS == 2 ? 0 : 128 + 4 * 32) + (GATHER ? 32 * LDA_F : 0) + (BNIN ? 2 * BN_TAB : 0));
}

}
```

### two-stage-gnn_amd/graph.py

```python
import numpy as np
import torch

from . import _native as nat


def _i32(n, device):
    return torch.empty(int(n), dtype=torch.int32, device=device)


def _scan_ws(n, device):
    need = np.zeros(1, dtype=np.int64)
    nat.call_nostream("scan_workspace_ints", int(n), need.ctypes.data)
    return _i32(need[0], device)


def exclusive_scan(counts):
    n = counts.numel()
    out = _i32(n + 1, counts.device)
    nat.call("exclusive_scan_i32", counts, n, out, _scan_ws(n, counts.device))
    return out


class GraphBatch:
    def __init__(self):
        self.B = 0
        self.nmax = 0
        self.n_rows = 0
        self.n_ghost = 0
        self.layout = "packed"
        self.sizes = None
        self.graph_ptr = None
        self.row_graph = None
        self.row_slot = None
        self.slot_count = None
        self.rowptr = None
        self.col = None
        self.val = None
        self.nnz = 0
        self.symmetric = False
        self._t = None
        self.device = None
        self.panel_units = True

    @property
    def total_rows(self):
        return self.n_rows + self.n_ghost

    def _set_sizes(self, sizes, nmax, device, ghosts=True):
        sizes = np.asarray(sizes, dtype=np.int64).reshape(-1)
        if sizes.size == 0 or (sizes < 0).any() or (sizes > nmax).any():
            raise ValueError("graph sizes must lie in [0, nmax]")
        self.B = int(sizes.size)
        self.nmax = int(nmax)
        self.sizes = sizes
        self.n_rows = int(sizes.sum())
        self.n_ghost = self.nmax if ghosts else 0
        gp = np.zeros(self.B + 1, dtype=np.int32)
        np.cumsum(sizes, out=gp[1:])
        hist = np.bincount(sizes, minlength=self.nmax + 1)
        slot_count = (self.B - np.cumsum(hist)[: self.nmax]).astype(np.int32)
        self.device = device
        self.graph_ptr = torch.from_numpy(gp).to(device, non_blocking=True)
        self.slot_count = torch.from_numpy(slot_count).to(device, non_blocking=True)
        self.row_graph = _i32(max(self.n_rows, 1), device)
        self.row_slot = _i32(max(self.n_rows, 1), device)
        nat.call("row_maps", self.graph_ptr, self.B, self.n_rows, self.row_graph, self.row_slot)

    @classmethod
    def from_dense_ghost1(cls, adj, sizes, assume_symmetric=False):
        sizes = np.asarray(sizes, dtype=np.int64).reshape(-1)
        nmax = adj.size(1)
        if (sizes > nmax).any() or (sizes < 0).any():
            raise ValueError("graph sizes must lie in [0, nmax]")
        has_ghost = sizes < nmax
        g = cls.from_dense(adj, sizes + has_ghost, layout="packed", assume_symmetric=assume_symmetric, ghosts=False)
        mult = np.ones(g.n_rows, dtype=np.float32)
        ends = np.cumsum(sizes + has_ghost) - 1
        mult[ends[has_ghost]] = (nmax - sizes[has_ghost]).astype(np.float32)
        g.row_mult = torch.from_numpy(mult).to(adj.device)
        g.real_sizes = sizes
        return g

    @classmethod
    def from_dense(cls, adj, sizes=None, layout="packed", assume_symmetric=False, ghosts=None):
        if adj.dim() != 3 or adj.size(1) != adj.size(2):
            raise ValueError("adj must be [B,N,N]")
        adj = adj.contiguous().float()
        B, nmax = adj.size(0), adj.size(1)
        g = cls()
        g.layout = layout
        if layout == "padded":
            sizes = np.full(B, nmax, dtype=np.int64)
        elif sizes is None:
            raise ValueError("packed layout needs the per-graph node counts")
        g._set_sizes(sizes, nmax, adj.device, ghosts=(layout != "padded") if ghosts is None else bool(ghosts))
        if g.B != B:
            raise ValueError("len(sizes) != batch size of adj")
        R = g.n_rows
        cnt = torch.zeros(g.total_rows, dtype=torch.int32, device=adj.device)
        nat.call("dense_adj_count", adj, B, nmax, g.graph_ptr, g.row_graph, R, cnt)
        g.rowptr = exclusive_scan(cnt)
        g.nnz = int(g.rowptr[-1].item())
        g.col = _i32(max(g.nnz, 1), adj.device)
        g.val = torch.empty(max(g.nnz, 1), dtype=torch.float32, device=adj.device)
        nat.call("dense_adj_fill", adj, B, nmax, g.graph_ptr, g.row_graph, R, g.rowptr, g.col, g.val)
        g.symmetric = bool(assume_symmetric)
        return g

    @classmethod
    def from_edge_index(cls, edge_index, num_nodes, sizes=None, nmax=None, assume_symmetric=False, ghosts=False):
        g = cls()
        g.layout = "packed"
        dev = edge_index.device
        num_nodes = int(num_nodes)
        if sizes is None:
            sizes = np.array([num_nodes], dtype=np.int64)
        sizes = np.asarray(sizes, dtype=np.int64)
        if int(sizes.sum()) != num_nodes:
            raise ValueError("sizes must sum to num_nodes")
        g._set_sizes(sizes, int(nmax) if nmax is not None else int(max(1, sizes.max())), dev, ghosts=ghosts)
        ei = edge_index.contiguous()
        E = int(ei.size(1))
        R = num_nodes
        cnt = torch.zeros(g.total_rows, dtype=torch.int32, device=dev)
        bad = torch.zeros(1, dtype=torch.int32, device=dev)
        key, other = ei[1], ei[0]
        nat.call("coo_count", key, E, R, cnt, bad)
        g.rowptr = exclusive_scan(cnt)
        g.nnz = E
        g.col = _i32(max(E, 1), dev)
        g.eid = _i32(max(E, 1), dev)
        nat.call("coo_fill", key, other, E, R, g.rowptr, _i32(max(R, 1), dev), g.col, g.eid)
        if int(bad.item()) != 0:
            raise IndexError("edge_index contains node ids outside [0, num_nodes)")
        g.val = None
        g.symmetric = bool(assume_symmetric)
        return g

    _uniform_cache = {}

    @classmethod
    def uniform(cls, B, K, device):
        key = (int(B), int(K), str(device))
        g = cls._uniform_cache.get(key)
        if g is None:
            g = cls._uniform_cache[key] = cls.structure_only(np.full(int(B), int(K), dtype=np.int64), int(K), device, ghosts=False)
        return g

    @classmethod
    def structure_only(cls, sizes, nmax, device, ghosts=True):
        g = cls()
        g.layout = "packed" if ghosts else "padded"
        g._set_sizes(sizes, nmax, device, ghosts=ghosts)
        g.rowptr = torch.zeros(g.total_rows + 1, dtype=torch.int32, device=device)
        g.col = _i32(1, device)
        g.symmetric = True
        return g

    @classmethod
    def from_csr(cls, rowptr, col, val, sizes, nmax, assume_symmetric=True):
        g = cls()
        g._set_sizes(sizes, nmax, rowptr.device)
        if rowptr.numel() != g.total_rows + 1:
            raise ValueError("rowptr must have n_rows + nmax + 1 entries (empty ghost rows included)")
        g.rowptr, g.col, g.val = rowptr, col, val
        g.nnz = int(col.numel())
        g.symmetric = bool(assume_symmetric)
        return g

    def row_slabs(self, rows_per_slab=64):
        cache = getattr(self, "_slabs", None)
        if cache is None or cache[3] != rows_per_slab:
            starts, seg = [], [0]
            off = 0
            for n in self.sizes:
                n = int(n)
                starts.extend(range(off, off + n, rows_per_slab))
                seg.append(len(starts))
                off += n
            srp = np.asarray(starts + [off], dtype=np.int32)
            cache = self._slabs = (torch.from_numpy(srp).to(self.device),
                                   torch.from_numpy(np.asarray(seg, dtype=np.int32)).to(self.device), len(starts), rows_per_slab)
        return cache[0], cache[1], cache[2]

    def ell(self):
        if self.val is not None:
            return None
        if getattr(self, "_ell", None) is None:
            R = self.total_rows
            deg = self.rowptr[1:] - self.rowptr[:-1]
            maxdeg = int(deg.max().item()) if R > 0 else 0
            W = 4 if maxdeg <= 4 else (8 if maxdeg <= 8 else 16)
            ell = _i32(max(R * W, 1), self.device)
            tail_cnt = torch.zeros(R, dtype=torch.int32, device=self.device) if maxdeg > W else None
            nat.call("csr_to_ell", self.rowptr, self.col, R, W, ell, tail_cnt)
            tail = None
            if tail_cnt is not None:
                tail_ptr = exclusive_scan(tail_cnt)
                tail_col = _i32(max(int(tail_ptr[-1].item()), 1), self.device)
                nat.call("csr_tail_fill", self.rowptr, self.col, tail_ptr, R, W, tail_col)
                tail = (tail_ptr, tail_col)
            self._ell = (ell, W, tail)
        return self._ell

    def ell_slots(self):
        if getattr(self, "_ell_slots", None) is None:
            e = self.ell()
            if e is None or self.total_rows >= (1 << 20) or self.nmax > 1024 or self.row_slot is None:
                self._ell_slots = False
            else:
                ell, W, tail = e
                slot_of = self.row_slot.to(torch.int64)

                def pack(ids32, n):
                    ids = ids32[:n].to(torch.int64)
                    ok = (ids >= 0) & (ids < self.n_rows)
                    packed = torch.where(ok, (slot_of[ids.clamp(0, max(self.n_rows - 1, 0))] << 20) | ids, torch.full_like(ids, -1))
                    out = _i32(max(ids32.numel(), 1), self.device)
                    out[:n] = packed.to(torch.int32)
                    return out
                table = pack(ell, self.total_rows * W)
                tcol = pack(tail[1], int(tail[0][-1].item())) if tail is not None else None
                self._ell_slots = (table, tcol)
        return self._ell_slots if self._ell_slots is not False else None

    def du_map(self, other_blocks):
        if self.sizes is None or getattr(self, "ghost_slots_fixed", None) is not None:
            return None, (-1 if self.B <= 64 else 0), 64
        cache = self.__dict__.setdefault("_du_maps", {})
        key = int(other_blocks)
        if key not in cache:
            sizes = np.asarray(self.sizes, dtype=np.int64)
            ncu = torch.cuda.get_device_properties(self.device).multi_processor_count
            chunk = 64
            if key + int(np.maximum(1, -(-sizes // 64)).sum()) > ncu:
                chunk = 128
            if int(sizes.max()) > 255 * chunk or self.B >= (1 << 22):
                cache[key] = (None, 0, 64)
            else:
                ent = [(b << 8) | c for b in range(self.B) for c in range(max(1, -(-int(sizes[b]) // chunk)))]
                cache[key] = (torch.from_numpy(np.asarray(ent, dtype=np.int32)).to(self.device), len(ent), chunk)
        return cache[key]

    def readout_map(self, nslots, fill_rows):
        if self.sizes is None:
            return None, 0
        key = (int(nslots), int(fill_rows))
        cache = self.__dict__.setdefault("_ro_maps", {})
        if key not in cache:
            ch = np.zeros(1, dtype=np.int32)
            ng = np.zeros(1, dtype=np.int32)
            nf = np.zeros(1, dtype=np.int32)
            nat.call_nostream("sage_layer_fwd_bn_plan", int(self.n_rows), int(fill_rows), int(self.B), int(nslots), int(self.panel_units),
                              ch.ctypes.data, ng.ctypes.data, nf.ctypes.data)
            ch, ng, nf = int(ch[0]), int(ng[0]), int(nf[0])
            chunks = -(-int(nslots) // ch)
            npan = nf or -(-self.n_rows // 32)
            q, r = divmod(npan, 8)
            start = np.zeros(9, dtype=np.int64)
            for x in range(8):
                start[x + 1] = start[x] + (q + 1 if x < r else q)
            gp = np.concatenate([[0], np.cumsum(np.asarray(self.sizes, dtype=np.int64))])
            mid_panel = ((gp[:-1] + gp[1:]) // 2) // 32
            xcd_of_graph = np.clip(np.searchsorted(start, mid_panel, side="right") - 1, 0, 7)
            want = [[] for _ in range(8)]
            for b in range(self.B):
                for c in range(chunks):
                    want[int(xcd_of_graph[b])].append(b * chunks + c)
            items = self.B * chunks
            slots = [[k for k in range(items) if (ng + k) % 8 == x] for x in range(8)]
            ro = np.full(items, -1, dtype=np.int32)
            left = []
            for x in range(8):
                n = min(len(want[x]), len(slots[x]))
                ro[slots[x][:n]] = want[x][:n]
                left += want[x][n:]
                slots[x] = slots[x][n:]
            free = [k for x in range(8) for k in slots[x]]
            ro[free] = left
            assert (np.sort(ro) == np.arange(items)).all()
            cache[key] = (torch.from_numpy(ro).to(self.device), ch)
        return cache[key]

    def bn_workspace(self, B, L, Fh, Fl, nslots):
        key = (B, L, Fh, Fl, nslots)
        ws = getattr(self, "_bn_ws", None)
        if ws is None or ws["key"] != key:
            words = (L - 1) * 2 * nslots
            from . import message_passing as mp
            ws = {"key": key, "sums": mp.register_clear_on_error(torch.zeros(max(words, 2), dtype=torch.int64, device=self.device)),
                  "ghost": mp.register_clear_on_error(torch.zeros(max(2 * (L - 1), 2), dtype=torch.float32, device=self.device)),
                  "packed": mp.register_clear_on_error(torch.zeros(B * ((L - 1) * Fh + Fl) + Fl, dtype=torch.int64, device=self.device)),
                  "dirty": False}
            self._bn_ws = ws
        return ws

    def _ensure_transpose(self):
        if self._t is None:
            R1 = self.total_rows
            dev = self.device
            rowptr_t = _i32(R1 + 1, dev)
            col_t = _i32(max(self.nnz, 1), dev)
            val_t = torch.empty(max(self.nnz, 1), dtype=torch.float32, device=dev) if self.val is not None else None
            src_e = _i32(max(self.nnz, 1), dev)
            nat.call("csr_transpose", self.rowptr, self.col, self.val, R1, R1, self.nnz, rowptr_t, col_t, val_t,
                     src_e, _i32(max(R1, 1), dev), _scan_ws(R1, dev))
            self._t = (rowptr_t, col_t, val_t)
            self.src_e_t = src_e
        return self._t

    def transpose_map(self):
        rp, col, _ = self._ensure_transpose()
        return rp, col, self.src_e_t

    def transposed(self, val="graph"):
        if isinstance(val, str):
            val = self.val
        if self.symmetric:
            return self.rowptr, self.col, val
        t = self._ensure_transpose()
        if val is self.val:
            return t
        return t[0], t[1], (val[self.src_e_t.long()] if val is not None else None)

    def new_features(self, feat, zero=False):
        f = torch.zeros if zero else torch.empty
        return f(self.total_rows, feat, dtype=torch.float32, device=self.device)
```

### two-stage-gnn_amd/sage_stack.py

```python
import numpy as np
import torch

from . import _native as nat
from . import message_passing as mp


def eligible(g, convs, bn, x):
    if not bn or g.B > 128 or len(convs) < 2:
        return False
    hid = convs[0].output_dim
    for i, c in enumerate(convs):
        if c.add_self or not c.normalize_embedding or c.dropout > 0.001:
            return False
        if c.output_dim % 4 or c.output_dim > 128:
            return False
        if i < len(convs) - 1 and c.output_dim != hid:
            return False
    return x.dim() == 2 and x.size(1) % 4 == 0 and x.is_cuda and x.stride(0) % 4 == 0


def _aggregate_raw(g, x, transposed=False, rows=None):
    n = g.total_rows if rows is None else rows
    if g.val is None and mp.ell_ok(x) and g.total_rows <= mp.ELL_MAX_ROWS and (not transposed or g.symmetric):
        return mp.spmm_ell(g, x, rows=n)
    rp, col, val = g.transposed() if transposed else (g.rowptr, g.col, g.val)
    return mp.spmm_raw(rp, col, val, x, n)


import os

FUSED_TAIL = os.environ.get("TSGNN_FUSED_TAIL", "1") != "0"
MERGED_FWD = os.environ.get("TSGNN_MERGED_FWD", "1") != "0"
MERGED_BWD = os.environ.get("TSGNN_MERGED_BWD", "1") != "0"
GATHER_MAX_ROWS = int(os.environ.get("TSGNN_GATHER_MAX_ROWS", 65536))
GATHER_FUSED = os.environ.get("TSGNN_GATHER_FUSED", "1") != "0"
EPILOGUE_READOUT = os.environ.get("TSGNN_EPILOGUE_READOUT", "1") != "0"
LAST_LAYER_ROWS = os.environ.get("TSGNN_LAST_LAYER_ROWS", "1") != "0"
RO_MAP = os.environ.get("TSGNN_RO_MAP", "1") != "0"
FUSED_BN = os.environ.get("TSGNN_FUSED_BN", "1") != "0"
SLOT_WGRAD = os.environ.get("TSGNN_SLOT_WGRAD", "0") != "0"
HEAD_DU = os.environ.get("TSGNN_HEAD_DU", "1") != "0"


DU_MAP = os.environ.get("TSGNN_DU_MAP", "1") != "0"
SLABS_BESIDE = os.environ.get("TSGNN_SLABS_BESIDE", "1") != "0"
NSLAB_MAX = int(os.environ.get("TSGNN_NSLAB_MAX", "0"))
_ncu = {}


def _cu_count(dev):
    n = _ncu.get(dev)
    if n is None:
        n = _ncu[dev] = torch.cuda.get_device_properties(dev).multi_processor_count
    return n


def _slabs_beside_panels(nslab, rps, need, rows, K, N, dev, panel_units):
    if not SLABS_BESIDE or nslab <= 0:
        return nslab, rps, need
    if NSLAB_MAX and nslab > NSLAB_MAX:
        rps = (-(-rows // NSLAB_MAX) + 7) // 8 * 8
        nslab = -(-rows // rps)
        need = nslab * (K + 1) * N
    ncu = _cu_count(dev)
    npan = int(nat.lib().tsgnn_panel_blocks(int(rows), int(panel_units)))
    if npan <= ncu or 2 * nslab + npan <= 2 * ncu:
        return nslab, rps, need
    cap = max(32, (2 * ncu - npan) // 2)
    rps = -(-rows // cap)
    rps = (rps + 7) // 8 * 8
    nslab = -(-rows // rps)
    return nslab, rps, nslab * (K + 1) * N


def _gather_ok(g, x):
    if not GATHER_FUSED or g.val is not None or not mp.ell_ok(x) or g.total_rows > GATHER_MAX_ROWS:
        return False
    return True


def _flush_readout(g, B, sn, sg, pending):
    if pending is not None:
        y, pk = pending
        nat.call("readout_partial_f32", g.graph_ptr, B, sn, g.n_rows, sg, y, y.stride(0), y.size(1), pk)


_PER_GRAPH = [False]

_IMG_FLOATS = 16384
_IMG_LAYERS = 4


class per_graph_stats:
    def __init__(self, on=True):
        self.on = bool(on)

    def __enter__(self):
        self.prev = _PER_GRAPH[0]
        _PER_GRAPH[0] = self.on

    def __exit__(self, *exc):
        _PER_GRAPH[0] = self.prev
        return False


class _SageStack(torch.autograd.Function):

    @staticmethod
    def forward(ctx, x0, g, has_bias, n_head, nodes, *params):
        head = params[len(params) - n_head:] if n_head else None
        params = params[:len(params) - n_head] if n_head else params
        L = len(params) // 2
        Ws = [params[2 * l].contiguous() for l in range(L)]
        bs = [params[2 * l + 1] if has_bias else None for l in range(L)]
        dev = x0.device
        R, B = g.total_rows, g.B
        Fh, Fl = Ws[0].size(1), Ws[-1].size(1)
        total = B * ((L - 1) * Fh + Fl)
        packed = torch.empty(total + Fl, dtype=torch.int64, device=dev) if not nodes else None
        cat = torch.empty(R, (L - 1) * Fh + Fl, dtype=torch.float32, device=dev) if nodes else None
        x = mp._check(x0, R)
        gs = g.n_ghost
        if g.n_ghost > 0 and x.stride(0) % 4 == 0 and all(
                Ws[l].size(1) % 4 == 0 and Ws[l].data_ptr() % 16 == 0 and (bs[l] is None or bs[l].data_ptr() % 16 == 0)
                for l in range(L)):
            fixed = getattr(g, "ghost_slots_fixed", None)
            gs = min(g.nmax, (int(fixed) if fixed is not None else int(g.sizes.max()) + 1))
        if nodes == 1:
            gs = g.n_ghost
        sn, sg = (gs, gs) if g.n_ghost else (g.nmax, 0)
        saved = []
        off = 0
        pending_ro = None
        keep = []
        last_ro_done = False
        bnf = None
        per_graph = ctx.per_graph = bool(_PER_GRAPH[0])
        if per_graph and head is not None:
            raise NotImplementedError("per-graph statistics: the readout and the node-feature form of the stack only")
        if (FUSED_BN and not per_graph and head is not None and not nodes and L >= 2 and g.n_ghost == g.nmax and sn == sg and sn <= 1024
                and Fh == 128 and Fl == 128 and Ws[0].size(0) <= 128 and x.size(1) % 4 == 0 and MERGED_FWD and EPILOGUE_READOUT
                and _gather_ok(g, x) and all(Ws[l].size(0) == 128 and Ws[l].stride(0) % 4 == 0 for l in range(1, L))
                and all(Ws[l].data_ptr() % 16 == 0 and (bs[l] is None or bs[l].data_ptr() % 16 == 0) for l in range(L))
                and mp.rowgemm_ok(x, x.stride(0), Ws[0], Ws[0].stride(0), Ws[0].size(0), Fh, False)
                and head[0].size(0) <= 128 and (L - 1) * Fh + Fl <= 2048 and g.row_graph is not None):
            ell_s = g.ell_slots()
            if ell_s is not None:
                bnf = g.bn_workspace(B, L, Fh, Fl, sn)
                if bnf["dirty"]:
                    bnf["sums"].zero_(); bnf["ghost"].zero_(); bnf["packed"].zero_()
                bnf["dirty"] = True
                packed = bnf["packed"]
        ctx.w_img = ctx.pack_desc = None
        if bnf is not None:
            ell, ell_w, tail = g.ell()
            tp, tc = tail if tail is not None else (None, None)
            ell_s, tc_s = ell_s
            sums, ghost = bnf["sums"], bnf["ghost"]
            ro_map, ro_ch = g.readout_map(sn, gs) if RO_MAP else (None, 0)
            w_img = pack_desc = None
            if 1 <= L - 1 <= _IMG_LAYERS:
                w_img = torch.empty(2 * (L - 1), _IMG_FLOATS, dtype=torch.float32, device=dev)
                pack_desc = np.empty(1 + 12 * (L - 1), dtype=np.int64)
                pack_desc[0] = 2 * (L - 1)
                for l in range(1, L):
                    for kn in (1, 0):
                        t = 2 * (l - 1) + (1 - kn)
                        pack_desc[1 + 6 * t:7 + 6 * t] = (Ws[l].data_ptr(), Ws[l].stride(0), 128, 128, kn, w_img[t].data_ptr())
                bnf["pack_desc"] = pack_desc
            ctx.w_img, ctx.pack_desc = w_img, pack_desc
            for l in range(L):
                K, N = Ws[l].size(0), Ws[l].size(1)
                v = torch.empty(R, N, dtype=torch.float32, device=dev)
                rinv = torch.empty(R, dtype=torch.float32, device=dev)
                z = torch.empty(R, x.size(1) if l == 0 else Fh, dtype=torch.float32, device=dev)
                s_out = sums[l * 2 * sn:(l + 1) * 2 * sn] if l < L - 1 else None
                g_out = ghost[2 * l:2 * l + 2] if l < L - 1 else None
                if l == 0:
                    nat.call("gather_rowgemm_st_f32", ell, ell_w, tp, tc, x, x.stride(0), Ws[0], Ws[0].stride(0), bs[0], v, v.stride(0), rinv, z,
                             z.stride(0), g.n_rows, K, N, gs, g.row_slot, s_out, g_out, int(g.panel_units),
                             pack_desc.ctypes.data if pack_desc is not None else None)
                    mean = rstd = None
                else:
                    pm, pr_ = saved[l - 1][3], saved[l - 1][4]
                    last = l == L - 1
                    nat.call("sage_layer_fwd_bn_f32", ell_s, ell_w, tp, tc_s, saved[l - 1][1], saved[l - 1][1].stride(0), Ws[l], Ws[l].stride(0), bs[l],
                             v, v.stride(0), rinv, z, z.stride(0), g.n_rows, K, gs, g.graph_ptr, g.slot_count, B, sn, sg,
                             packed[(l - 1) * B * Fh:(l - 1) * B * Fh + B * Fh],
                             packed[l * B * Fh:l * B * Fh + (B + 1) * N] if last else None, g.row_graph,
                             sums[(l - 1) * 2 * sn:l * 2 * sn], ghost[2 * (l - 1):2 * l], pm, pr_,
                             None if last else g.row_slot, s_out, g_out, ro_map, ro_ch, int(g.panel_units),
                             w_img[2 * (l - 1)] if w_img is not None else None)
                if l < L - 1:
                    mean = torch.empty(g.nmax, dtype=torch.float32, device=dev)
                    rstd = torch.empty(g.nmax, dtype=torch.float32, device=dev)
                else:
                    mean = rstd = None
                saved.append((z, v, rinv, mean, rstd, True))
            last_ro_done = True
        for l in (range(L) if bnf is None else ()):
            K, N = Ws[l].size(0), Ws[l].size(1)
            if nodes and l == L - 1:
                v = cat[:, (L - 1) * Fh:]
            else:
                v = torch.empty(R, N, dtype=torch.float32, device=dev)
            rinv = torch.empty(R, dtype=torch.float32, device=dev)
            lean = (g.n_ghost > 0 and x.stride(0) % 4 == 0 and N % 4 == 0 and Ws[l].data_ptr() % 16 == 0
                    and (bs[l] is None or bs[l].data_ptr() % 16 == 0))
            fused = lean and N <= 128 and _gather_ok(g, x) and mp.rowgemm_ok(x, x.stride(0), Ws[l], Ws[l].stride(0), K, N, False)
            if (fused and MERGED_FWD and pending_ro is not None and K == 128 and N == 128 and x.size(1) == 128
                    and Ws[l].stride(0) % 4 == 0):
                ell, ell_w, tail = g.ell()
                tp, tc = tail if tail is not None else (None, None)
                z = torch.empty(R, x.size(1), dtype=torch.float32, device=dev)
                if EPILOGUE_READOUT and l == L - 1 and not nodes and l > 0 and (not g.n_ghost or gs > 0):
                    nat.call("sage_layer_fwd_ro_f32", ell, ell_w, tp, tc, x, x.stride(0), Ws[l], Ws[l].stride(0), bs[l], v, v.stride(0),
                             rinv, z, z.stride(0), g.n_rows, K, gs, g.graph_ptr, B, sn, sg, pending_ro[1],
                             packed[off:off + (B + 1) * N], g.row_graph)
                    last_ro_done = True
                else:
                    nat.call("sage_layer_fwd_f32", ell, ell_w, tp, tc, x, x.stride(0), Ws[l], Ws[l].stride(0), bs[l], v, v.stride(0), rinv,
                             z, z.stride(0), g.n_rows, K, gs, g.graph_ptr, B, sn, sg, pending_ro[1])
                pending_ro = None
            elif fused:
                _flush_readout(g, B, sn, sg, pending_ro)
                pending_ro = None
                ell, ell_w, tail = g.ell()
                tp, tc = tail if tail is not None else (None, None)
                z = torch.empty(R, x.size(1), dtype=torch.float32, device=dev)
                nat.call("gather_rowgemm_f32", ell, ell_w, tp, tc, x, x.stride(0), Ws[l], Ws[l].stride(0), 0, bs[l], v, v.stride(0), rinv,
                         z, z.stride(0), g.n_rows, K, N, 1, gs)
            else:
                _flush_readout(g, B, sn, sg, pending_ro)
                pending_ro = None
                z = _aggregate_raw(g, x, rows=g.n_rows if lean else None)
                if lean and mp.rowgemm_ok(z, z.stride(0), Ws[l], Ws[l].stride(0), K, N, False):
                    nat.call("rowgemm_f32", z, z.stride(0), Ws[l], Ws[l].stride(0), 0, bs[l], v, v.stride(0), rinv, g.n_rows, K, N, 1,
                             gs)
                elif mp.rowgemm_ok(z, z.stride(0), Ws[l], Ws[l].stride(0), K, N, False):
                    if lean:
                        z[g.n_rows:].zero_()
                        lean = False
                    nat.call("rowgemm_f32", z, z.stride(0), Ws[l], Ws[l].stride(0), 0, bs[l], v, v.stride(0), rinv, R, K, N, 1, 0)
                else:
                    if lean:
                        z[g.n_rows:].zero_()
                        lean = False
                    nat.call("linear_l2norm_f32", z, z.stride(0), Ws[l], Ws[l].stride(0), bs[l], v, v.stride(0), rinv, R, K, N, 1)
            pk = packed[off:off + B * N] if not nodes else None
            if l < L - 1 and per_graph:
                mean = torch.empty(R, dtype=torch.float32, device=dev)
                rstd = torch.empty(R, dtype=torch.float32, device=dev)
                y = torch.empty_like(v) if not nodes else cat[:, l * Fh:(l + 1) * Fh]
                if l == 0 and not nodes:
                    packed[:total].zero_()
                nat.call("row_ln_fwd_f32", v, v.stride(0), g.n_rows + sg, N, 1, mean, rstd, y, y.stride(0))
                if not nodes:
                    pending_ro = (y, pk)
                keep.append(y)
                x = y
            elif l < L - 1:
                mean = torch.empty(g.nmax, dtype=torch.float32, device=dev)
                rstd = torch.empty(g.nmax, dtype=torch.float32, device=dev)
                y = torch.empty_like(v) if not nodes else cat[:, l * Fh:(l + 1) * Fh]
                nat.call("slot_bn_fwd_f32", g.graph_ptr, g.slot_count, B, sn, g.n_rows, sg, v, v.stride(0), N, 1,
                         mean, rstd, y, y.stride(0), packed if (l == 0 and not nodes) else None, total)
                if not nodes:
                    pending_ro = (y, pk)
                keep.append(y)
                x = y
            else:
                mean = rstd = None
                if head is None and not nodes and not last_ro_done:
                    nat.call("readout_partial_f32", g.graph_ptr, B, sn, g.n_rows, sg, v, v.stride(0), N, pk)
            saved.append((z, v, rinv, mean, rstd, lean))
            off += B * N
        ctx.nodes = nodes
        if nodes:
            if nodes == 2 and g.n_ghost:
                nat.defer_zero(cat[g.n_rows:])
            ctx.g, ctx.L, ctx.has_bias, ctx.dims = g, L, has_bias, (Fh, Fl)
            ctx.slots = (sn, sg)
            ctx.Ws, ctx.saved, ctx.arg = Ws, saved, None
            ctx.params = params
            ctx.head = None
            return cat
        out = torch.empty(B, (L - 1) * Fh + Fl, dtype=torch.float32, device=dev)
        arg = torch.empty(total, dtype=torch.int32, device=dev)
        ctx.g, ctx.L, ctx.has_bias, ctx.dims = g, L, has_bias, (Fh, Fl)
        ctx.slots = (sn, sg)
        ctx.Ws, ctx.saved, ctx.arg = Ws, saved, arg
        ctx.params = params
        ctx.x0_ld = x.size(1) if L == 0 else x0.size(1)
        ctx.head = None
        if head is None:
            nat.call("readout_decode_layers_f32", packed, B, L, Fh, Fl, out, out.stride(0), arg)
            return out
        w1, b1, w2, b2 = head
        w1c, w2c = w1.contiguous(), w2.contiguous()
        E, C = w1c.size(0), w2c.size(0)
        vec = torch.empty(B, E, dtype=torch.float32, device=dev)
        y = torch.empty(B, C, dtype=torch.float32, device=dev)
        v_last = saved[-1][1]
        if bnf is not None:
            nat.call("packed_head_fwd_z_f32", packed, B, L, Fh, Fl, out, out.stride(0), arg, w1c, b1, w2c, b2, E, C, vec, y,
                     bnf["sums"], (L - 1) * 2 * sn)
            bnf["dirty"] = False
        elif last_ro_done and E <= 128 and out.size(1) <= 2048:
            nat.call("packed_head_fwd_f32", packed, B, L, Fh, Fl, out, out.stride(0), arg, w1c, b1, w2c, b2, E, C, vec, y)
        else:
            nat.call("readout_head_fwd_f32", packed, B, L, Fh, Fl, v_last, v_last.stride(0), g.graph_ptr, g.n_rows, sn, sg, out,
                     out.stride(0), arg, w1c, b1, w2c, b2, E, C, vec, y)
        ctx.head = (out, vec, w1c, w2c, head)
        ctx.set_materialize_grads(False)
        return vec, y

    @staticmethod
    def backward(ctx, *gouts):
        g, L = ctx.g, ctx.L
        Fh, Fl = ctx.dims
        R, B = g.total_rows, g.B
        w_img = ctx.w_img
        head_grads = ()
        du_last = None
        if ctx.head is None:
            dout = gouts[0].contiguous()
            dev = dout.device
        else:
            out, vec, w1c, w2c, (pw1, pb1, pw2, pb2) = ctx.head
            dvec, dy = gouts
            dev = out.device
            P, E, C = out.size(1), w1c.size(0), w2c.size(0)
            if dy is None and dvec is None:
                return (None,) * (5 + 2 * L + 4)
            ce = mp.take_deferred_ce(dy) if dy is not None else None
            if ce is None:
                dy = dy.contiguous() if dy is not None else torch.zeros(B, C, device=dev)
            dvec = dvec.contiguous() if dvec is not None else None
            dout = torch.empty(B, P, dtype=torch.float32, device=dev)
            dw1, s1 = mp._sink_or_new(pw1, (E, P), dev)
            dw2, s2 = mp._sink_or_new(pw2, (C, E), dev)
            db1, s3 = mp._sink_or_new(pb1, (E,), dev) if pb1 is not None else (None, False)
            db2, s4 = mp._sink_or_new(pb2, (C,), dev) if pb2 is not None else (None, False)
            parts = mp.head_norm_slots((s1, s2, s3, s4), (pb1 is not None, pb2 is not None), (pw1, pb1, pw2, pb2), E)
            sn_, sg_ = ctx.slots
            v_l, rinv_l, lean_l = ctx.saved[L - 1][1], ctx.saved[L - 1][2], ctx.saved[L - 1][5]
            if (HEAD_DU and LAST_LAYER_ROWS and not ctx.nodes and L > 1 and lean_l and Fl % 4 == 0 and Fl <= 128 and g.n_ghost == g.nmax
                    and sn_ == sg_ and g.n_ghost >= B and ctx.needs_input_grad[5 + 2 * (L - 1)] and v_l.stride(0) % 4 == 0):
                du_l = torch.empty(R, Fl, dtype=torch.float32, device=dev)
                argl = ctx.arg[(L - 1) * B * Fh:(L - 1) * B * Fh + B * Fl]
                dmap, ndmap, dchunk = g.du_map(B + (E + 3) // 4 + 1) if DU_MAP else (None, 0, 64)
                if nat.try_call("head2_bwd_du_map_f32", out, out.stride(0), vec, ce[0] if ce is not None else None,
                                ce[1] if ce is not None else None, ce[2] if ce is not None else None, None if ce is not None else dy, dvec,
                                w1c, w2c, B, P, E, C, dout, dout.stride(0), dw1, db1, dw2, db2, parts, g.graph_ptr, g.n_rows, sg_,
                                sn_, v_l, v_l.stride(0), rinv_l, argl, (L - 1) * Fh, Fl, du_l, du_l.stride(0), dmap, ndmap, dchunk):
                    du_last = du_l
            if du_last is not None:
                pass
            elif ce is not None:
                nat.call("head2_bwd_ce_f32", out, out.stride(0), vec, ce[0], ce[1], ce[2], dvec, w1c, w2c, B, P, E, C, dout,
                         dout.stride(0), dw1, db1, dw2, db2, parts)
            else:
                nat.call("head2_bwd_f32", out, out.stride(0), vec, dy, dvec, w1c, w2c, B, P, E, C, dout, dout.stride(0), dw1, db1, dw2,
                         db2, parts)
            head_grads = (None if s1 else dw1, None if s3 else db1, None if s2 else dw2, None if s4 else db2)
            if mp.GRAD_SINK is not None and s1 and s2 and (s3 or pb1 is None) and (s4 or pb2 is None):
                mp.GRAD_SINK.ready((pw1, pb1, pw2, pb2))
        sn, sg = ctx.slots
        grads = [None] * (2 * L)
        dxs = None
        dx0 = None
        keep = []
        red = mp.WgradSets(mp.wgrad_reduce_multi, max_sets_with_shares=4)
        for l in range(L - 1, -1, -1):
            z, v, rinv, mean, rstd, lean = ctx.saved[l]
            W = ctx.Ws[l]
            K, N = W.size(0), W.size(1)
            last = l == L - 1
            du = du_last if (last and du_last is not None) else torch.empty(R, N, dtype=torch.float32, device=dev)
            bo = sg
            if ctx.nodes:
                dsl = argl = None
                dnode = dout[:, l * Fh:l * Fh + N]
            else:
                dsl = dout[:, l * Fh:l * Fh + N]
                argl = ctx.arg[l * B * Fh:l * B * Fh + B * N]
                dnode = None
            if last and du_last is not None:
                bo = B
            elif (LAST_LAYER_ROWS and last and not ctx.nodes and dxs is None and N % 4 == 0 and N <= 128 and g.n_ghost == g.nmax
                    and sn == sg and dout.stride(0) % 4 == 0 and dsl.data_ptr() % 16 == 0 and g.row_graph is not None):
                nat.call("readout_l2_bwd_f32", g.graph_ptr, g.row_graph, B, g.n_rows, sg, v, v.stride(0), dsl, dout.stride(0), argl, N, rinv,
                         du, du.stride(0))
            elif (SLOT_WGRAD and l == 0 and L > 1 and not ctx.nodes and not ctx.needs_input_grad[0] and lean and B <= 32 and N == 128
                  and K <= 128 and sn == sg and g.n_ghost == g.nmax and ctx.needs_input_grad[5] and z.stride(0) % 4 == 0
                  and z.data_ptr() % 16 == 0 and v.data_ptr() % 16 == 0 and (not ctx.has_bias or ctx.needs_input_grad[6])):
                per = int(os.environ.get("TSGNN_SLOT_WGRAD_PER", "2"))
                nblk = max(1, -(-sn // per))
                ws0 = torch.empty(nblk * (K + 1) * N, dtype=torch.float32, device=dev)
                nat.call("slot_post_wgrad_f32", g.graph_ptr, g.slot_count, B, sn, g.n_rows, sg, v, v.stride(0), dxs,
                         dxs.stride(0) if dxs is not None else 0, dsl, dout.stride(0) if dsl is not None else 0, argl, N, 1, 1, mean, rstd,
                         rinv, z, z.stride(0), K, ws0, nblk)
                dw = red.grad(ctx.params[0], (K, N))
                db = red.grad(ctx.params[1] if ctx.has_bias else None, (N,))
                red.add((ws0, nblk, K, N, dw, db))
                grads[0], grads[1] = red.autograd_grad(dw), red.autograd_grad(db)
                continue
            elif ctx.per_graph and ctx.nodes:
                nat.call("row_post_nodes_bwd_f32", g.n_rows, g.n_rows + sg, v, v.stride(0), dxs, dxs.stride(0) if dxs is not None else 0,
                         dnode, dnode.stride(0), 1 if ctx.nodes == 2 else 0, N, 0 if last else 1, 0 if last else 1, mean, rstd, rinv, du,
                         du.stride(0))
            elif ctx.per_graph:
                nat.call("row_post_bwd_f32", g.row_graph, B, g.n_rows, g.n_rows + sg, v, v.stride(0), dxs,
                         dxs.stride(0) if dxs is not None else 0, dsl, dout.stride(0), argl, N, 0 if last else 1, 0 if last else 1, mean,
                         rstd, rinv, du, du.stride(0))
            else:
                nat.call("slot_post_bwd_f32", g.graph_ptr, g.slot_count, B, sn, g.n_rows, sg, v, v.stride(0), dxs,
                         dxs.stride(0) if dxs is not None else 0, dnode, dnode.stride(0) if dnode is not None else 0, dsl,
                         dout.stride(0) if dsl is not None else 0, argl, N, 0 if last else 1, 0 if last else 1, mean, rstd, rinv, du,
                         du.stride(0))
            want_w = ctx.needs_input_grad[5 + 2 * l]
            want_b = ctx.has_bias and ctx.needs_input_grad[6 + 2 * l]
            merged = False
            if (MERGED_BWD and want_w and lean and l > 0 and K == 128 and N == 128 and g.symmetric and z.size(1) == K
                    and _gather_ok(g, du) and z.data_ptr() % 16 == 0 and du.data_ptr() % 16 == 0 and W.data_ptr() % 16 == 0
                    and W.stride(0) % 4 == 0):
                nslab, rps, need = mp.wgrad_plan(g.n_rows, K, N, z.stride(0), du.stride(0))
                nslab, rps, need = _slabs_beside_panels(nslab, rps, need, g.n_rows, K, N, dev, g.panel_units)
                if 0 < nslab < 512:
                    ell, ell_w, tail = g.ell()
                    tp, tc = tail if tail is not None else (None, None)
                    ws = torch.empty(need, dtype=torch.float32, device=dev)
                    dxs = torch.empty(R, K, dtype=torch.float32, device=dev)
                    nat.call("sage_layer_bwd_f32", ell, ell_w, tp, tc, du, du.stride(0), W, W.stride(0), dxs, dxs.stride(0), z, z.stride(0),
                             g.n_rows, nslab, rps, bo, ws, int(g.panel_units),
                             w_img[2 * (l - 1) + 1] if w_img is not None else None)
                    dw = red.grad(ctx.params[2 * l], (K, N))
                    db = red.grad(ctx.params[2 * l + 1] if want_b else None, (N,))
                    red.add((ws, nslab, K, N, dw, db))
                    grads[2 * l], grads[2 * l + 1] = red.autograd_grad(dw), red.autograd_grad(db)
                    keep.append(du)
                    merged = True
            if merged:
                continue
            if want_w:
                if not lean and sg < g.n_ghost:
                    du[g.n_rows + sg:].zero_()
                sl = mp.linear_wgrad_slabs(z, K, du[:g.n_rows + bo] if lean else du, bias_only_rows=bo if lean else 0)
                if sl is not None:
                    dw = red.grad(ctx.params[2 * l], (K, N))
                    db = red.grad(ctx.params[2 * l + 1] if want_b else None, (N,))
                    red.add((sl[0], sl[1], K, N, dw, db))
                    dw, db = red.autograd_grad(dw), red.autograd_grad(db)
                else:
                    if lean:
                        z[g.n_rows:].zero_()
                        du[g.n_rows + sg:].zero_()
                    dw, db = mp.linear_wgrad(z, K, du, want_b)
                grads[2 * l], grads[2 * l + 1] = dw, db
            elif want_b:
                if sg < g.n_ghost:
                    du[g.n_rows + sg:].zero_()
                grads[2 * l + 1] = mp.colsum(du)
            keep.append(du)
            need_dx = l > 0 or ctx.needs_input_grad[0]
            if need_dx:
                ldz = z.size(1)
                if (l > 0 and g.n_ghost > 0 and g.symmetric and ldz == K and K <= 128 and _gather_ok(g, du)
                        and mp.rowgemm_ok(du, du.stride(0), W, W.stride(0), N, K, True)):
                    ell, ell_w, tail = g.ell()
                    tp, tc = tail if tail is not None else (None, None)
                    dxs = torch.empty(R, ldz, dtype=torch.float32, device=dev)
                    nat.call("gather_rowgemm_f32", ell, ell_w, tp, tc, du, du.stride(0), W, W.stride(0), 1, None, dxs, dxs.stride(0), None,
                             None, 0, g.n_rows, N, K, 0, 0)
                else:
                    dz = torch.zeros(R, ldz, dtype=torch.float32, device=dev) if ldz > K else torch.empty(R, ldz, dtype=torch.float32, device=dev)
                    if mp.rowgemm_ok(du, du.stride(0), W, W.stride(0), N, K, True):
                        nat.call("rowgemm_f32", du, du.stride(0), W, W.stride(0), 1, None, dz, dz.stride(0), None, g.n_rows, N, K, 0, 0)
                    else:
                        mp.gemm(du, du.stride(0), 1, W, 1, W.stride(0), dz, dz.stride(0), 1, R, K, N)
                    dxs = _aggregate_raw(g, dz, transposed=True, rows=g.n_rows if (l > 0 and g.n_ghost) else None)
                if l == 0:
                    dx0 = dxs
        red.close()
        del keep
        return (dx0, None, None, None, None) + tuple(grads) + head_grads


def sage_stack_readouts(x, g, convs):
    has_bias = convs[0].bias is not None
    params = []
    for c in convs:
        params.append(c.weight)
        params.append(c.bias if has_bias else c.weight.new_zeros(1))
    return _SageStack.apply(x, g, has_bias, 0, 0, *params)


def sage_stack_nodes(x, g, convs, mask_ghost):
    has_bias = convs[0].bias is not None
    params = []
    for c in convs:
        params.append(c.weight)
        params.append(c.bias if has_bias else c.weight.new_zeros(1))
    return _SageStack.apply(x, g, has_bias, 0, 2 if (mask_ghost and g.n_ghost) else 1, *params)


PAIR_LAUNCHES = os.environ.get("TSGNN_STACK_PAIRS", "1") != "0"
ZERO_RIDER = os.environ.get("TSGNN_ZERO_RIDER", "1") != "0"


def _multi(tn, gs, zero=None):
    import numpy as np
    words = [len(tn), len(gs)]
    for a in tn:
        words += [nat._arg(v) or 0 for v in a[:11]]
    for a in gs:
        words += [(nat._arg(v) or 0) if not isinstance(v, bool) else int(v) for v in a[:20]]
    d = np.asarray(words, dtype=np.int64)
    if zero is not None:
        za, zb = zero
        if not (za.is_contiguous() and zb.is_contiguous()):
            return False
        return nat.try_call("sage_multi_zero_f32", d.ctypes.data, za, za.numel(), zb, zb.numel())
    return nat.try_call("sage_multi_f32", d.ctypes.data)


def _zero_after(q, i):
    return q[i + 1][1][0] if i + 1 < len(q) and q[i + 1][0] == "_zero" else None


def _slab_form(rec):
    return rec[0] == "linear_wgrad_f32" and len(rec[1]) >= 13 and rec[1][11] is None and rec[1][12] is None


def run_paired(qa, qb):
    i = j = 0
    while i < len(qa) and j < len(qb):
        a, b = qa[i], qb[j]
        if a[0] == b[0] == "gather_rowgemm_f32":
            za, zb = _zero_after(qa, i), _zero_after(qb, j)
            if ZERO_RIDER and za is not None and zb is not None and _multi([], [a[1], b[1]], zero=(za, zb)):
                i += 2; j += 2
                continue
            if _multi([], [a[1], b[1]]):
                i += 1; j += 1
                continue
        if _slab_form(a) and _slab_form(b):
            na = qa[i + 1] if i + 1 < len(qa) else (None,)
            nb = qb[j + 1] if j + 1 < len(qb) else (None,)
            if na[0] == nb[0] == "gather_rowgemm_f32" and _multi([a[1], b[1]], [na[1], nb[1]]):
                i += 2; j += 2
                continue
            if _multi([a[1], b[1]], []):
                i += 1; j += 1
                continue
        if a[0] == b[0] == "_zero":
            torch._foreach_zero_([a[1][0], b[1][0]])
            i += 1; j += 1
            continue
        if a[0] == b[0] and a[0] in _PAIRED and _PAIRED[a[0]](a[1], b[1]):
            i += 1; j += 1
            continue
        nat.run([a]); nat.run([b])
        i += 1; j += 1
    nat.run(qa[i:]); nat.run(qb[j:])


def _same(x, y):
    if torch.is_tensor(x) or torch.is_tensor(y):
        return torch.is_tensor(x) and torch.is_tensor(y) and x.data_ptr() == y.data_ptr()
    return x == y


def _pair_slot_bn(a, b):
    if a[14] is not None or b[14] is not None or not all(_same(a[k], b[k]) for k in (0, 1, 2, 3, 4, 5, 7, 8, 9, 13)):
        return False
    return nat.try_call("slot_bn_fwd_pair_f32", a[0], a[1], a[2], a[3], a[4], a[5], a[6], b[6], a[7], a[8], a[9], a[10], b[10], a[11], b[11],
                        a[12], b[12], a[13])


def _pair_slot_post_bwd(a, b):
    if any(t[12] is not None or t[14] is not None for t in (a, b)):
        return False
    if (a[8] is None) != (b[8] is None) or (a[10] is None) != (b[10] is None):
        return False
    if not all(_same(a[k], b[k]) for k in (0, 1, 2, 3, 4, 5, 7, 9, 11, 15, 16, 17, 22)):
        return False
    return nat.try_call("slot_post_bwd_pair_f32", a[0], a[1], a[2], a[3], a[4], a[5], a[6], b[6], a[7], a[8], b[8], a[9], a[10], b[10], a[11],
                        a[15], a[16], a[17], a[18], b[18], a[19], b[19], a[20], b[20], a[21], b[21], a[22])


def _pair_reduce(a, b):
    if a[24] is not None or a[25] is not None or b[24] is not None or b[25] is not None:
        return False
    sets = [mp.wgrad_set(*t[6 * k:6 * k + 6], kn=1, lddw=t[6 * k + 3]) for t in (a, b) for k in range(4) if t[6 * k] is not None]
    if not sets:
        return False
    d = mp._desc(sets)
    return nat.try_call("wgrad_reduce_sets_f32", d.ctypes.data, None, None)


_PAIRED = {"slot_bn_fwd_f32": _pair_slot_bn, "slot_post_bwd_f32": _pair_slot_post_bwd, "wgrad_reduce_multi_f32": _pair_reduce}


class _StackCtx:
    needs_input_grad = ()

    def set_materialize_grads(self, v):
        pass


class _SageStackPair(torch.autograd.Function):

    @staticmethod
    def forward(ctx, xa, xb, g, has_bias, nodes_a, nodes_b, n_a, *params):
        ca, cb = _StackCtx(), _StackCtx()
        with nat.deferred() as qa:
            oa = _SageStack.forward(ca, xa, g, has_bias, 0, nodes_a, *params[:n_a])
        with nat.deferred() as qb:
            ob = _SageStack.forward(cb, xb, g, has_bias, 0, nodes_b, *params[n_a:])
        run_paired(qa, qb)
        ctx.ca, ctx.cb, ctx.n_a = ca, cb, n_a
        return oa, ob

    @staticmethod
    def backward(ctx, da, db):
        n, n_a = ctx.needs_input_grad, ctx.n_a
        ctx.ca.needs_input_grad = (n[0], False, False, False, False) + tuple(n[7:7 + n_a])
        ctx.cb.needs_input_grad = (n[1], False, False, False, False) + tuple(n[7 + n_a:])
        with nat.deferred() as qa:
            ga = _SageStack.backward(ctx.ca, da)
        with nat.deferred() as qb:
            gb = _SageStack.backward(ctx.cb, db)
        run_paired(qa, qb)
        return (ga[0], gb[0], None, None, None, None, None) + tuple(ga[5:]) + tuple(gb[5:])


def sage_stack_nodes_pair(xa, xb, g, convs_a, convs_b, mask_ghost):
    has_bias = convs_a[0].bias is not None
    if (convs_b[0].bias is not None) != has_bias:
        return sage_stack_nodes(xa, g, convs_a, mask_ghost), sage_stack_nodes(xb, g, convs_b, mask_ghost)
    params = []
    for c in list(convs_a) + list(convs_b):
        params.append(c.weight)
        params.append(c.bias if has_bias else c.weight.new_zeros(1))
    nodes = 2 if (mask_ghost and g.n_ghost) else 1
    if mp.ell_ok(xa) and g.val is None:
        g.ell()
        if not g.symmetric:
            g.transposed()
    return _SageStackPair.apply(xa, xb, g, has_bias, nodes, nodes, 2 * len(convs_a), *params)


def head_ok(g, convs, lin1, lin2):
    P = sum(c.output_dim for c in convs)
    Fl = convs[-1].output_dim
    return (FUSED_TAIL and isinstance(lin1, torch.nn.Linear) and isinstance(lin2, torch.nn.Linear) and P % 4 == 0 and P <= 2048
            and Fl % 4 == 0 and Fl <= 128 and lin1.out_features <= 4096 and g.B <= 1024 and lin1.in_features == P
            and lin1.weight.data_ptr() % 16 == 0)


def sage_stack_head(x, g, convs, lin1, lin2):
    has_bias = convs[0].bias is not None
    params = []
    for c in convs:
        params.append(c.weight)
        params.append(c.bias if has_bias else c.weight.new_zeros(1))
    vec, y = _SageStack.apply(x, g, has_bias, 4, 0, *params, lin1.weight, lin1.bias, lin2.weight, lin2.bias)
    y._tsgnn_defer_ce = True
    return vec, y
```

Before: 257,000 graphs/s.

## Add packed per-panel gather schedules that balance neighbour loads across row groups

Adds a host-built gather schedule that packs the neighbour ids of each 32-row panel into fixed-size per-wave records (8 groups of 32 slots, or 16 of 24 for the split-K layer-0 kernel). Each record carries start/end bitmasks, and rows are distributed to balance degree across waves. The fused gather-GEMM kernels (layer-0 forward, BN forward and merged backward) gain a SCHED template path that loads all slot ids up front and issues the row loads at once, replacing the padded ELL width plus tail walk. This is meant to cut wasted padded loads and load imbalance from varied degrees, at the cost of a CPU-side packing pass (cached per graph) and extra kernel instantiations, and it only applies when no unit-cut panels or tails exist.

```diff
diff --git a/include/tsgnn.h b/include/tsgnn.h
--- a/include/tsgnn.h
+++ b/include/tsgnn.h
@@ -144,6 +144,9 @@
                       int64_t ldc, float* rinv, int64_t rows, int K, int N, int normalize, int64_t fill_rows,
                       tsgnn_stream_t stream);
 int tsgnn_panel_blocks(int64_t rows, int panel_units);
+#define TSGNN_SCHED_8x32 32
+#define TSGNN_SCHED_16x24 24
+int tsgnn_gather_sched_slots(int64_t rows, int64_t fill_rows, int K, int panel_units, int layer0);
 int tsgnn_gather_rowgemm_f32(const int* ell, int ell_w, const int* tail_ptr, const int* tail_col, const float* x, int64_t ldx, const float* b, int64_t ldb, int trans_b,
                              const float* bias, float* c, int64_t ldc, float* rinv, float* zout, int64_t ldz, int64_t rows, int K,
                              int N, int normalize, int64_t fill_rows, tsgnn_stream_t stream);
diff --git a/two-stage-gnn_amd/csrc/layer_bwd.hip b/two-stage-gnn_amd/csrc/layer_bwd.hip
--- a/two-stage-gnn_amd/csrc/layer_bwd.hip
+++ b/two-stage-gnn_amd/csrc/layer_bwd.hip
@@ -6,11 +6,11 @@
 
 namespace {
 
-template <bool PANELS_FIRST, bool UNITS = false, bool BIMG = false>
+template <bool PANELS_FIRST, bool UNITS = false, bool BIMG = false, int SCHED = 0>
 __global__ __launch_bounds__(256) void sage_layer_bwd_kernel(RowGemmArgs ga, TnArgs gt, unsigned n_tn, unsigned nslab, unsigned n_pan, int slab_delay) {
   extern __shared__ __attribute__((aligned(16))) float smem[];
   if (PANELS_FIRST) {
-    if (blockIdx.x < n_pan) rowgemm_body<4, true, true, 1, false, false, false, UNITS, BIMG>(ga, smem, blockIdx.x);
+    if (blockIdx.x < n_pan) rowgemm_body<4, true, true, 1, false, false, false, UNITS, BIMG, SCHED>(ga, smem, blockIdx.x);
     else {
       for (int i = 0; i < slab_delay; ++i) __builtin_amdgcn_s_sleep(16);
       const unsigned b = blockIdx.x - n_pan, by = b / nslab, sp = b % nslab;
@@ -20,7 +20,7 @@
     }
   } else {
     if (blockIdx.x < n_tn) tn_rows_body<4, 4, 2>(gt, smem, blockIdx.x % nslab, blockIdx.x / nslab, nslab);
-    else rowgemm_body<4, true, true, 1, false, false, false, UNITS, BIMG>(ga, smem, blockIdx.x - n_tn);
+    else rowgemm_body<4, true, true, 1, false, false, false, UNITS, BIMG, SCHED>(ga, smem, blockIdx.x - n_tn);
   }
 }
 
@@ -32,7 +32,9 @@
                              int64_t lddxs, const float* z, int64_t ldz, int64_t rows, int nslab, int64_t rows_per_slab,
                              int64_t bias_only_rows, float* ws, int panel_units, const float* w_img, tsgnn_stream_t stream) {
   if (!ell || !du || !w || !dxs || !z || !ws || rows <= 0 || nslab <= 0 || rows_per_slab <= 0 || bias_only_rows < 0) return TSGNN_EINVAL;
-  if (ell_w != 4 && ell_w != 8 && ell_w != 16) return TSGNN_EUNSUPPORTED;
+  const bool sched = ell_w == TSGNN_SCHED_8x32;
+  if (sched && (tail_ptr || tail_col)) return TSGNN_EINVAL;
+  if (!sched && ell_w != 4 && ell_w != 8 && ell_w != 16) return TSGNN_EUNSUPPORTED;
   const uintptr_t al = reinterpret_cast<uintptr_t>(ell) | reinterpret_cast<uintptr_t>(du) | reinterpret_cast<uintptr_t>(w) |
                        reinterpret_cast<uintptr_t>(dxs) | reinterpret_cast<uintptr_t>(z) | reinterpret_cast<uintptr_t>(w_img);
   if ((al & 15) || (lddu % 4) || (ldw % 4) || (lddxs % 4) || (ldz % 4) || lddu < 128 || ldw < 128 || lddxs < 128 || ldz < 128)
@@ -50,16 +52,19 @@
   static const int slab_delay_env = [] { const char* e = getenv("TSGNN_SLAB_DELAY"); return e ? atoi(e) : -1; }();
   const int slab_delay = slab_delay_env >= 0 ? slab_delay_env : ((int64_t)n_pan <= (int64_t)ncu ? 2 : 0);
   const bool units = ga.unit == 8 || ga.unit == 16;
+  if (sched && units) return TSGNN_EUNSUPPORTED;
   TSGNN_KNAME("sage_layer_bwd_kernel<%s,%s>", panels_first ? "true" : "false", units ? "true" : "false");
-#define TSGNN_BWD_(PF_, UN_) \
+#define TSGNN_BWD_(PF_, UN_, SC_) \
   do {                       \
-    if (w_img) sage_layer_bwd_kernel<PF_, UN_, true><<<n_tn + n_pan, 256, lds, stream>>>(ga, gt, n_tn, (unsigned)nslab, n_pan, slab_delay); \
-    else sage_layer_bwd_kernel<PF_, UN_><<<n_tn + n_pan, 256, lds, stream>>>(ga, gt, n_tn, (unsigned)nslab, n_pan, slab_delay);            \
+    if (w_img) sage_layer_bwd_kernel<PF_, UN_, true, SC_><<<n_tn + n_pan, 256, lds, stream>>>(ga, gt, n_tn, (unsigned)nslab, n_pan, slab_delay); \
+    else sage_layer_bwd_kernel<PF_, UN_, false, SC_><<<n_tn + n_pan, 256, lds, stream>>>(ga, gt, n_tn, (unsigned)nslab, n_pan, slab_delay);       \
   } while (0)
-  if (panels_first && units) TSGNN_BWD_(true, true);
-  else if (panels_first) TSGNN_BWD_(true, false);
-  else if (units) TSGNN_BWD_(false, true);
-  else TSGNN_BWD_(false, false);
+  if (panels_first && units) TSGNN_BWD_(true, true, 0);
+  else if (panels_first && sched) TSGNN_BWD_(true, false, TSGNN_SCHED_8x32);
+  else if (panels_first) TSGNN_BWD_(true, false, 0);
+  else if (units) TSGNN_BWD_(false, true, 0);
+  else if (sched) TSGNN_BWD_(false, false, TSGNN_SCHED_8x32);
+  else TSGNN_BWD_(false, false, 0);
 #undef TSGNN_BWD_
   TSGNN_CHECK_LAUNCH();
   return TSGNN_OK;
diff --git a/two-stage-gnn_amd/csrc/layer_fwd.hip b/two-stage-gnn_amd/csrc/layer_fwd.hip
--- a/two-stage-gnn_amd/csrc/layer_fwd.hip
+++ b/two-stage-gnn_amd/csrc/layer_fwd.hip
@@ -20,13 +20,13 @@
   }
 }
 
-template <bool RO, bool ST, bool UNITS = false, bool BIMG = false>
+template <bool RO, bool ST, bool UNITS = false, bool BIMG = false, int SCHED = 0>
 __global__ __launch_bounds__(256, 2) void sage_layer_fwd_bn_kernel(RowGemmArgs ga, SlotArgs sa, BnReadArgs bn, unsigned n_gemm, unsigned ro_gx,
                                                                 int ro_ch, int F4, unsigned long long* __restrict__ packed, unsigned n_main,
                                                                 PullRider pr, const int* __restrict__ ro_map) {
   extern __shared__ __attribute__((aligned(16))) float smem[];
   if (blockIdx.x < n_gemm) {
-    rowgemm_body<4, false, true, 1, RO, true, ST, UNITS, BIMG>(ga, smem, blockIdx.x);
+    rowgemm_body<4, false, true, 1, RO, true, ST, UNITS, BIMG, SCHED>(ga, smem, blockIdx.x);
   } else if (blockIdx.x < n_main) {
     unsigned r = blockIdx.x - n_gemm;
     if (ro_map) r = (unsigned)ro_map[r];
@@ -62,7 +62,9 @@
       rows <= 0 || fill_rows < 0 || K <= 0 || B <= 0 || nslots <= 0 || (n_ghost != 0 && n_ghost != nslots) || (packed_out && !row_graph) ||
       (row_slot && (!sums_out || !ghost_out)))
     return TSGNN_EINVAL;
-  if (ell_w != 4 && ell_w != 8 && ell_w != 16) return TSGNN_EUNSUPPORTED;
+  const bool sched = ell_w == TSGNN_SCHED_8x32;
+  if (sched && (tail_ptr || tail_col)) return TSGNN_EINVAL;
+  if (!sched && ell_w != 4 && ell_w != 8 && ell_w != 16) return TSGNN_EUNSUPPORTED;
   const uintptr_t al = reinterpret_cast<uintptr_t>(ell) | reinterpret_cast<uintptr_t>(x) | reinterpret_cast<uintptr_t>(w) |
                        reinterpret_cast<uintptr_t>(v) | reinterpret_cast<uintptr_t>(zout) | reinterpret_cast<uintptr_t>(bias) |
                        reinterpret_cast<uintptr_t>(sums_in) | reinterpret_cast<uintptr_t>(sums_out) | reinterpret_cast<uintptr_t>(w_img);
@@ -88,14 +90,16 @@
   const size_t lro = 8 * 128 * sizeof(unsigned long long) + 256 * sizeof(float2);
   if (lds < lro) lds = lro;
   const unsigned n_main = n_gemm + ro_gx * (unsigned)B;
+  if (sched && ga.n_full > 0) return TSGNN_EUNSUPPORTED;
   const PullRider pr = take_pull_rider();
   const bool units = ga.unit == 8 || ga.unit == 16;
-#define TSGNN_FWD_BN_(RO_, ST_, UN_, IM_) \
-  sage_layer_fwd_bn_kernel<RO_, ST_, UN_, IM_><<<n_main + pr.blocks, 256, lds, stream>>>(ga, sa, bn, n_gemm, ro_gx, ro_ch, K / 4, packed, n_main, pr, ro_map)
+#define TSGNN_FWD_BN_(RO_, ST_, UN_, IM_, SC_) \
+  sage_layer_fwd_bn_kernel<RO_, ST_, UN_, IM_, SC_><<<n_main + pr.blocks, 256, lds, stream>>>(ga, sa, bn, n_gemm, ro_gx, ro_ch, K / 4, packed, n_main, pr, ro_map)
 #define TSGNN_FWD_BN(RO_, ST_)                                                                  \
   do {                                                                                          \
-    if (units) { if (w_img) TSGNN_FWD_BN_(RO_, ST_, true, true); else TSGNN_FWD_BN_(RO_, ST_, true, false); }   \
-    else { if (w_img) TSGNN_FWD_BN_(RO_, ST_, false, true); else TSGNN_FWD_BN_(RO_, ST_, false, false); }       \
+    if (units) { if (w_img) TSGNN_FWD_BN_(RO_, ST_, true, true, 0); else TSGNN_FWD_BN_(RO_, ST_, true, false, 0); }   \
+    else if (sched) { if (w_img) TSGNN_FWD_BN_(RO_, ST_, false, true, TSGNN_SCHED_8x32); else TSGNN_FWD_BN_(RO_, ST_, false, false, TSGNN_SCHED_8x32); } \
+    else { if (w_img) TSGNN_FWD_BN_(RO_, ST_, false, true, 0); else TSGNN_FWD_BN_(RO_, ST_, false, false, 0); }       \
   } while (0)
   if (packed_out) {
     TSGNN_KNAME("sage_layer_fwd_bn_kernel<true,false,%s>", units ? "true" : "false");
diff --git a/two-stage-gnn_amd/csrc/rowgemm.hip b/two-stage-gnn_amd/csrc/rowgemm.hip
--- a/two-stage-gnn_amd/csrc/rowgemm.hip
+++ b/two-stage-gnn_amd/csrc/rowgemm.hip
@@ -34,16 +34,17 @@
   if (b < pk.blocks) pack_rider_body(pk, b);
   else pull_rider_body(pr, b - pk.blocks);
 }
-template <bool UNITS>
+template <bool UNITS, int SCHED = 0>
 __global__ __launch_bounds__(256) void rowgemm_gather_st_kernel(RowGemmArgs g, PullRider pr, unsigned nblk, PackRider pk) {
   extern __shared__ __attribute__((aligned(16))) float smem[];
   if (blockIdx.x >= nblk) { st_passengers(pk, pr, blockIdx.x - nblk); return; }
-  rowgemm_body<4, false, true, 1, false, false, true, UNITS>(g, smem, blockIdx.x);
-}
+  rowgemm_body<4, false, true, 1, false, false, true, UNITS, false, SCHED>(g, smem, blockIdx.x);
+}
+template <int SCHED = 0>
 __global__ __launch_bounds__(512) void rowgemm_gather_ks2_st_kernel(RowGemmArgs g, PullRider pr, unsigned nblk, PackRider pk) {
   extern __shared__ __attribute__((aligned(16))) float smem[];
   if (blockIdx.x >= nblk) { st_passengers(pk, pr, blockIdx.x - nblk); return; }
-  rowgemm_body<4, false, true, 2, false, false, true>(g, smem, blockIdx.x);
+  rowgemm_body<4, false, true, 2, false, false, true, false, false, SCHED>(g, smem, blockIdx.x);
 }
 
 template <int NT, bool TRANS_B>
@@ -223,7 +224,9 @@
                                 const int64_t* pack_desc, tsgnn_stream_t stream) {
   if (!ell || !x || !b || !c || !row_slot || !sums || !ghost || rows <= 0 || fill_rows < 0 || K <= 0 || N <= 0 || ldx < K || ldc < N)
     return TSGNN_EINVAL;
-  if (ell_w != 4 && ell_w != 8 && ell_w != 16) return TSGNN_EUNSUPPORTED;
+  const bool sched = ell_w == TSGNN_SCHED_8x32 || ell_w == TSGNN_SCHED_16x24;
+  if (sched && (tail_ptr || tail_col)) return TSGNN_EINVAL;
+  if (!sched && ell_w != 4 && ell_w != 8 && ell_w != 16) return TSGNN_EUNSUPPORTED;
   if (!tsgnn_rowgemm_supported(x, ldx, b, ldb, c, ldc, K, N, 0) || N > 128 || N <= 96 || K > 128 || (reinterpret_cast<uintptr_t>(ell) & 15) ||
       (reinterpret_cast<uintptr_t>(sums) & 15))
     return TSGNN_EUNSUPPORTED;
@@ -247,22 +250,26 @@
   const bool ks2 = K > KC && nblk <= ks2_max_blocks() && rowgemm_ks2_enabled();
   if (!ks2)
     nblk = panel_split(rows, device_cu_count(), panel_units, &g.n_full, &g.unit) + (fill_rows > 0 ? 1u : 0u);
+  if (sched && ell_w != (ks2 ? TSGNN_SCHED_16x24 : (g.unit == 8 || g.unit == 16) ? 0 : TSGNN_SCHED_8x32)) return TSGNN_EUNSUPPORTED;
   if (ks2) {
     constexpr size_t lds2 = rowgemm_lds_bytes<4, false, true, 2>();
     static bool attr = false;
     if (!attr && lds2 > 64 * 1024) {
-      (void)hipFuncSetAttribute(reinterpret_cast<const void*>(rowgemm_gather_ks2_st_kernel), hipFuncAttributeMaxDynamicSharedMemorySize, (int)lds2);
+      (void)hipFuncSetAttribute(reinterpret_cast<const void*>(rowgemm_gather_ks2_st_kernel<0>), hipFuncAttributeMaxDynamicSharedMemorySize, (int)lds2);
+      (void)hipFuncSetAttribute(reinterpret_cast<const void*>(rowgemm_gather_ks2_st_kernel<TSGNN_SCHED_16x24>), hipFuncAttributeMaxDynamicSharedMemorySize, (int)lds2);
       attr = true;
     }
     const PullRider pr = take_pull_rider(512);
     pk.blocks *= PACK_SET_ENTRIES / 512;
     TSGNN_KNAME("rowgemm_gather_ks2_st_kernel");
-    rowgemm_gather_ks2_st_kernel<<<nblk + pk.blocks + pr.blocks, 512, lds2, stream>>>(g, pr, nblk, pk);
+    if (sched) rowgemm_gather_ks2_st_kernel<TSGNN_SCHED_16x24><<<nblk + pk.blocks + pr.blocks, 512, lds2, stream>>>(g, pr, nblk, pk);
+    else rowgemm_gather_ks2_st_kernel<0><<<nblk + pk.blocks + pr.blocks, 512, lds2, stream>>>(g, pr, nblk, pk);
   } else {
     const PullRider pr = take_pull_rider(256);
     pk.blocks *= PACK_SET_ENTRIES / 256;
     TSGNN_KNAME("rowgemm_gather_st_kernel<%s>", (g.unit == 8 || g.unit == 16) ? "true" : "false");
     if (g.unit == 8 || g.unit == 16) rowgemm_gather_st_kernel<true><<<nblk + pk.blocks + pr.blocks, 256, rowgemm_lds_bytes<4, false, true>(), stream>>>(g, pr, nblk, pk);
+    else if (sched) rowgemm_gather_st_kernel<false, TSGNN_SCHED_8x32><<<nblk + pk.blocks + pr.blocks, 256, rowgemm_lds_bytes<4, false, true>(), stream>>>(g, pr, nblk, pk);
     else rowgemm_gather_st_kernel<false><<<nblk + pk.blocks + pr.blocks, 256, rowgemm_lds_bytes<4, false, true>(), stream>>>(g, pr, nblk, pk);
   }
   TSGNN_CHECK_LAUNCH();
@@ -273,6 +280,17 @@
   if (rows <= 0) return 0;
   int nf = 0, un = 16;
   return (int)panel_split(rows, device_cu_count(), panel_units, &nf, &un);
+}
+
+int tsgnn_gather_sched_slots(int64_t rows, int64_t fill_rows, int K, int panel_units, int layer0) {
+  if (rows <= 0) return 0;
+  if (layer0) {
+    const unsigned nblk = (unsigned)(ceil_div64(rows, 32) + (fill_rows > 0 ? 1 : 0));
+    if (K > KC && nblk <= ks2_max_blocks() && rowgemm_ks2_enabled()) return TSGNN_SCHED_16x24;
+  }
+  int nf = 0, un = 32;
+  (void)panel_split(rows, device_cu_count(), panel_units, &nf, &un);
+  return nf > 0 ? 0 : TSGNN_SCHED_8x32;
 }
 
 int tsgnn_gather_rowgemm_f32(const int* ell, int ell_w, const int* tail_ptr, const int* tail_col, const float* x, int64_t ldx, const float* b, int64_t ldb, int trans_b,
diff --git a/two-stage-gnn_amd/csrc/rowgemm_body.h b/two-stage-gnn_amd/csrc/rowgemm_body.h
--- a/two-stage-gnn_amd/csrc/rowgemm_body.h
+++ b/two-stage-gnn_amd/csrc/rowgemm_body.h
@@ -59,17 +59,21 @@
 
 __device__ __forceinline__ float4 ldg4(const float* p) { return *reinterpret_cast<const float4*>(p); }
 
+#ifndef TSGNN_EXP_DROP_NB16
+#define TSGNN_EXP_DROP_NB16 0
+#endif
 constexpr int GN = 8;
 constexpr int LDA_F = 128;
 
 template <int NT, bool TRANS_B, bool GATHER, int KS = 1, bool READOUT = false, bool BNIN = false, bool STATS = false, bool UNITS = false,
-          bool BIMG = false>
+          bool BIMG = false, int SCHED = 0>
 __device__ __forceinline__ void rowgemm_body(const RowGemmArgs& g, float* smem_all, unsigned bid) {
   static_assert(KS == 1 || (KS == 2 && GATHER && NT <= 4), "the split-K variant is built for the gather kernel, widths <= 128");
   static_assert(!READOUT || (NT <= 4 && KS == 1), "the readout epilogue is built for one column tile per wave");
   static_assert(!BNIN || (GATHER && KS == 1), "batch-norm on the fly lives in the gather prologue of the one-group kernel");
   static_assert(!STATS || NT <= 4, "the statistics epilogue is built for one column tile per wave");
   static_assert(!BIMG || (GATHER && KS == 1 && NT == 4), "the image variant is built for the one-group gather kernel at K = N = 128");
+  static_assert(SCHED == 0 || (GATHER && !UNITS && SCHED == (KS == 2 ? 24 : 32)), "gather schedules: 8 x 32 (one group) / 16 x 24 (two groups), plain panels");
   constexpr int NP = 32 * NT;
   constexpr int TPW = (NT + 3) / 4;
   constexpr int BV = NT;
@@ -282,7 +286,20 @@
   Staged st[NS];
   constexpr int NPASS = 4 / KS;
   int ids[NPASS][GN];
-  if (GATHER) {
+  constexpr int NSL = SCHED ? SCHED : 1;
+  int sid[NSL];
+  int s_first = 0;
+  unsigned s_end = 0u, s_short = 0u;
+  if constexpr (SCHED != 0) {
+    const int4* rec = reinterpret_cast<const int4*>(g.ell) + ((m0 >> 5) * (8 * KS) + (tid_all >> 5)) * ((4 + SCHED) / 4);
+    const int4 hd = rec[0];
+    s_first = hd.x; s_end = (unsigned)hd.z; s_short = (unsigned)hd.w;
+#pragma unroll
+    for (int q = 0; q < SCHED / 4; ++q) {
+      const int4 v = rec[1 + q];
+      sid[4 * q] = v.x; sid[4 * q + 1] = v.y; sid[4 * q + 2] = v.z; sid[4 * q + 3] = v.w;
+    }
+  } else if (GATHER) {
     const int rsub = tid_all >> 5;
 #pragma unroll
     for (int p = 0; p < NPASS; ++p) {
@@ -341,6 +358,60 @@
         }
       }
     }
+    if constexpr (SCHED != 0) {
+      float4 sv[NSL];
+#pragma unroll
+      for (int s = 0; s < SCHED; ++s) {
+        sv[s] = make_float4(0.f, 0.f, 0.f, 0.f);
+        if (colok && sid[s] >= 0) sv[s] = ldg4(g.a + (int64_t)(BNIN ? (sid[s] & 0xFFFFF) : sid[s]) * g.lda + 4 * c4);
+      }
+      if constexpr (BIMG) {
+        __builtin_amdgcn_sched_barrier(0);
+        img_fetch(0);
+        __builtin_amdgcn_sched_barrier(0);
+      }
+      if constexpr (BNIN) {
+        __syncthreads();
+#pragma unroll
+        for (int s = 0; s < SCHED; ++s) {
+          if (sid[s] >= 0) {
+            const float2 rm = bn_tab[sid[s] >> 20];
+            float4& t = sv[s];
+            t.x = fmaf(fmaxf(t.x, 0.f), rm.x, -rm.y); t.y = fmaf(fmaxf(t.y, 0.f), rm.x, -rm.y);
+            t.z = fmaf(fmaxf(t.z, 0.f), rm.x, -rm.y); t.w = fmaf(fmaxf(t.w, 0.f), rm.x, -rm.y);
+          }
+        }
+      }
+      const unsigned e_any = (unsigned)__builtin_amdgcn_readlane((int)s_end, 0) | (unsigned)__builtin_amdgcn_readlane((int)s_end, 32);
+      const unsigned nshort = ~s_short;
+      float z0 = __uint_as_float((nshort & 1u) << 31);
+      float4 va = make_float4(z0, z0, z0, z0);
+      float* ap = Apanel + s_first * LDA_F;
+      int pr = s_first;
+      const bool zok = g.zout != nullptr && colok;
+      int64_t zoff = (m0 + s_first) * g.ldz + 4 * c4;
+      int zleft = zok ? (int)min(rows_hi - (m0 + s_first), (int64_t)32) : 0;
+#pragma unroll
+      for (int s = 0; s < SCHED; ++s) {
+        va.x += sv[s].x; va.y += sv[s].y; va.z += sv[s].z; va.w += sv[s].w;
+        if ((e_any >> s) & 1u) {
+          if ((s_end >> s) & 1u) {
+            *reinterpret_cast<float4*>(ap + 4 * (c4 ^ (pr & 7))) = va;
+            if (zleft > 0) st_out(reinterpret_cast<float4*>(g.zout + zoff), va);
+            ++pr; ap += LDA_F; zoff += g.ldz; --zleft;
+            if (s + 1 < SCHED) {
+              z0 = __uint_as_float(((nshort >> (s + 1)) & 1u) << 31);
+              va = make_float4(z0, z0, z0, z0);
+            }
+          }
+        }
+      }
+      if constexpr (BIMG) {
+        __builtin_amdgcn_sched_barrier(0);
+        img_fetch(8);
+        __builtin_amdgcn_sched_barrier(0);
+      }
+    } else {
     float4 nbv[NPASS][GN];
 #pragma unroll
     for (int p = 0; p < NPASS; ++p)
@@ -375,7 +446,7 @@
 #pragma unroll
       for (int k = 1; k < GN; ++k) { va.x += nbv[p][k].x; va.y += nbv[p][k].y; va.z += nbv[p][k].z; va.w += nbv[p][k].w; }
       bool table_full = g.ell_w <= GN && ids[p][GN - 1] >= 0;
-      if (colok && g.ell_w > GN && ids[p][GN - 1] >= 0) {
+      if (!TSGNN_EXP_DROP_NB16 && colok && g.ell_w > GN && ids[p][GN - 1] >= 0) {
         static_assert(GN == 8, "the second half of a 16-wide table");
         const int4 e0 = *reinterpret_cast<const int4*>(g.ell + row * g.ell_w + 8), e1 = *reinterpret_cast<const int4*>(g.ell + row * g.ell_w + 12);
         const int js[8] = {e0.x, e0.y, e0.z, e0.w, e1.x, e1.y, e1.z, e1.w};
@@ -417,6 +488,7 @@
       __builtin_amdgcn_sched_barrier(0);
       img_fetch(8);
       __builtin_amdgcn_sched_barrier(0);
+    }
     }
   }
   float bias_v[TPW];
diff --git a/two-stage-gnn_amd/graph.py b/two-stage-gnn_amd/graph.py
--- a/two-stage-gnn_amd/graph.py
+++ b/two-stage-gnn_amd/graph.py
@@ -19,6 +19,72 @@
     out = _i32(n + 1, counts.device)
     nat.call("exclusive_scan_i32", counts, n, out, _scan_ws(n, counts.device))
     return out
+
+
+SCHED_SHAPES = ((8, 32), (16, 24))
+SCHED_HEADER = 4
+
+
+def unit_cut(rows, ncu, panel_units=True):
+    P = -(-int(rows) // 32)
+    return bool(panel_units) and ncu >= 8 and P > ncu and P - ncu <= ncu // 2
+
+
+def pack_gather_schedule(rowptr, col, n_rows, shape, row_slot=None, balance=True):
+    G, S = shape
+    if (G, S) not in SCHED_SHAPES:
+        raise ValueError("gather schedule shapes: %s" % (SCHED_SHAPES,))
+    n_rows = int(n_rows)
+    rowptr = np.asarray(rowptr, dtype=np.int64)[: n_rows + 1]
+    col = np.asarray(col, dtype=np.int64)
+    deg = np.diff(rowptr)
+    P = -(-n_rows // 32)
+    if n_rows <= 0 or (deg > S).any():
+        return None
+    nnz = int(rowptr[-1])
+    ids = col[:nnz]
+    if nnz and (ids.min() < 0 or ids.max() >= n_rows):
+        return None
+    if row_slot is not None:
+        ids = (np.asarray(row_slot, dtype=np.int64)[ids] << 20) | ids
+    need = np.ones(32 * P, dtype=np.int64)
+    need[:n_rows] = np.maximum(deg, 1)
+    degp = np.zeros(32 * P, dtype=np.int64)
+    degp[:n_rows] = deg
+    rec = np.full((P, G, SCHED_HEADER + S), -1, dtype=np.int64)
+    rec[:, :, :SCHED_HEADER] = 0
+    need_l, deg_l, ptr_l = need.tolist(), degp.tolist(), rowptr.tolist()
+    def pack_panel(p, share):
+        q, used, first, done = 0, 0, 0, 0
+        start = end = short = 0
+        rec[p, :, :SCHED_HEADER] = 0
+        rec[p, :, SCHED_HEADER:] = -1
+        for i in range(32):
+            r = 32 * p + i
+            n = need_l[r]
+            if used and (used + n > S or done + 0.5 * n > (q + 1) * share):
+                rec[p, q, :SCHED_HEADER] = (first, start, end, short)
+                q, used, first = q + 1, 0, i
+                start = end = short = 0
+                if q >= G:
+                    return False
+            d = deg_l[r]
+            if d:
+                rec[p, q, SCHED_HEADER + used:SCHED_HEADER + used + d] = ids[ptr_l[r]:ptr_l[r] + d]
+            start |= 1 << used
+            end |= 1 << (used + n - 1)
+            if d < 8:
+                short |= 1 << used
+            used += n
+            done += n
+        rec[p, q, :SCHED_HEADER] = (first, start, end, short)
+        return True
+
+    for p in range(P):
+        total = sum(need_l[32 * p:32 * p + 32])
+        if not (balance and pack_panel(p, total / G)) and not pack_panel(p, float("inf")):
+            return None
+    return (rec & 0xFFFFFFFF).astype(np.uint32).view(np.int32)
 
 
 class GraphBatch:
@@ -223,6 +289,24 @@
                 tcol = pack(tail[1], int(tail[0][-1].item())) if tail is not None else None
                 self._ell_slots = (table, tcol)
         return self._ell_slots if self._ell_slots is not False else None
+
+    def gather_schedule(self, shape, slots=False, ncu=None):
+        shape = (int(shape[0]), int(shape[1]))
+        if ncu is None:
+            ncu = torch.cuda.get_device_properties(self.device).multi_processor_count
+        cache = self.__dict__.setdefault("_gather_sched", {})
+        key = (shape, bool(slots), int(ncu))
+        if key not in cache:
+            sched = None
+            if (self.val is None and self.sizes is not None and getattr(self, "ghost_slots_fixed", None) is None and self.n_rows > 0
+                    and not unit_cut(self.n_rows, int(ncu), self.panel_units)
+                    and not (slots and (self.total_rows >= (1 << 20) or self.nmax > 1024 or self.row_slot is None))):
+                rec = pack_gather_schedule(self.rowptr.cpu().numpy(), self.col.cpu().numpy(), self.n_rows, shape,
+                                           self.row_slot.cpu().numpy() if slots else None)
+                if rec is not None:
+                    sched = torch.from_numpy(rec).to(self.device)
+            cache[key] = sched
+        return cache[key]
 
     def du_map(self, other_blocks):
         if self.sizes is None or getattr(self, "ghost_slots_fixed", None) is not None:
diff --git a/two-stage-gnn_amd/sage_stack.py b/two-stage-gnn_amd/sage_stack.py
--- a/two-stage-gnn_amd/sage_stack.py
+++ b/two-stage-gnn_amd/sage_stack.py
@@ -42,6 +42,8 @@
 HEAD_DU = os.environ.get("TSGNN_HEAD_DU", "1") != "0"
 
 
+GATHER_SCHED = os.environ.get("TSGNN_GATHER_SCHED", "1") != "0"
+GATHER_SCHED_L0 = os.environ.get("TSGNN_GATHER_SCHED_L0", "1") != "0"
 DU_MAP = os.environ.get("TSGNN_DU_MAP", "1") != "0"
 SLABS_BESIDE = os.environ.get("TSGNN_SLABS_BESIDE", "1") != "0"
 NSLAB_MAX = int(os.environ.get("TSGNN_NSLAB_MAX", "0"))
@@ -77,6 +79,16 @@
     if not GATHER_FUSED or g.val is not None or not mp.ell_ok(x) or g.total_rows > GATHER_MAX_ROWS:
         return False
     return True
+
+
+def _gather_sched(g, slots=False, layer0_k=0, fill=0):
+    if not GATHER_SCHED:
+        return None, 0
+    code = int(nat.lib().tsgnn_gather_sched_slots(int(g.n_rows), int(fill), int(layer0_k), int(g.panel_units), 1 if layer0_k else 0))
+    if not code:
+        return None, 0
+    sched = g.gather_schedule((16, 24) if code == 24 else (8, 32), slots=slots)
+    return (sched, code) if sched is not None else (None, 0)
 
 
 def _flush_readout(g, B, sn, sg, pending):
@@ -169,6 +181,8 @@
                         pack_desc[1 + 6 * t:7 + 6 * t] = (Ws[l].data_ptr(), Ws[l].stride(0), 128, 128, kn, w_img[t].data_ptr())
                 bnf["pack_desc"] = pack_desc
             ctx.w_img, ctx.pack_desc = w_img, pack_desc
+            sch0, sch0_w = _gather_sched(g, layer0_k=Ws[0].size(0), fill=gs) if GATHER_SCHED_L0 else (None, 0)
+            schs, schs_w = _gather_sched(g, slots=True)
             for l in range(L):
                 K, N = Ws[l].size(0), Ws[l].size(1)
                 v = torch.empty(R, N, dtype=torch.float32, device=dev)
@@ -177,14 +191,16 @@
                 s_out = sums[l * 2 * sn:(l + 1) * 2 * sn] if l < L - 1 else None
                 g_out = ghost[2 * l:2 * l + 2] if l < L - 1 else None
                 if l == 0:
-                    nat.call("gather_rowgemm_st_f32", ell, ell_w, tp, tc, x, x.stride(0), Ws[0], Ws[0].stride(0), bs[0], v, v.stride(0), rinv, z,
+                    e_, w_, tp_, tc_ = (sch0, sch0_w, None, None) if sch0 is not None else (ell, ell_w, tp, tc)
+                    nat.call("gather_rowgemm_st_f32", e_, w_, tp_, tc_, x, x.stride(0), Ws[0], Ws[0].stride(0), bs[0], v, v.stride(0), rinv, z,
                              z.stride(0), g.n_rows, K, N, gs, g.row_slot, s_out, g_out, int(g.panel_units),
                              pack_desc.ctypes.data if pack_desc is not None else None)
                     mean = rstd = None
                 else:
                     pm, pr_ = saved[l - 1][3], saved[l - 1][4]
                     last = l == L - 1
-                    nat.call("sage_layer_fwd_bn_f32", ell_s, ell_w, tp, tc_s, saved[l - 1][1], saved[l - 1][1].stride(0), Ws[l], Ws[l].stride(0), bs[l],
+                    e_, w_, tp_, tc_ = (schs, schs_w, None, None) if schs is not None else (ell_s, ell_w, tp, tc_s)
+                    nat.call("sage_layer_fwd_bn_f32", e_, w_, tp_, tc_, saved[l - 1][1], saved[l - 1][1].stride(0), Ws[l], Ws[l].stride(0), bs[l],
                              v, v.stride(0), rinv, z, z.stride(0), g.n_rows, K, gs, g.graph_ptr, g.slot_count, B, sn, sg,
                              packed[(l - 1) * B * Fh:(l - 1) * B * Fh + B * Fh],
                              packed[l * B * Fh:l * B * Fh + (B + 1) * N] if last else None, g.row_graph,
@@ -430,6 +446,9 @@
                 if 0 < nslab < 512:
                     ell, ell_w, tail = g.ell()
                     tp, tc = tail if tail is not None else (None, None)
+                    schb, schb_w = _gather_sched(g)
+                    if schb is not None:
+                        ell, ell_w, tp, tc = schb, schb_w, None, None
                     ws = torch.empty(need, dtype=torch.float32, device=dev)
                     dxs = torch.empty(R, K, dtype=torch.float32, device=dev)
                     nat.call("sage_layer_bwd_f32", ell, ell_w, tp, tc, du, du.stride(0), W, W.stride(0), dxs, dxs.stride(0), z, z.stride(0),
```

Result: faster. 263,200 graphs/s, median of 6 (+2.4%).
